# paolomandica/HALO

Measured on AMD Instinct MI355X. Metric: acquisition-scored images/sec (1024x2048, C=256, 19 cls), higher is better.
Workload: dtype f64

## Files before the change

### halo_amd/_lib.py

```python
import ctypes as C
import os
import threading

from . import _build

F32, F64 = 0, 1
I64, I32, U8 = 2, 3, 4
UNC = {"entropy": 0, "pixel_entropy": 1, "oracle_acc": 2}
UNC_ZEROS = 3
PUR = {"ripu": 0, "oracle_ripu": 1, "hyper": 2, "none": 3, "radius": 4, "euc_norm": 5}
E_UNSUPPORTED = -2
SELECT = {"auto": 0, "serial": 1, "binned": 2}
LOSS_CE, LOSS_NL = 1, 2
SWEEP_REASONS = ("done", "bad_values", "bin_overflow", "survivors", "exhausted", "not_run")
PAD = {"zeros": 0, "reflect": 1, "replicate": 2, "circular": 3}
FLAG_NORMALIZE = 1


def score_flags(normalize, padding_mode="zeros"):
    return (FLAG_NORMALIZE if normalize else 0) | (PAD[padding_mode] << 8)

_i64, _dbl, _int, _vp, _sz = C.c_int64, C.c_double, C.c_int, C.c_void_p, C.c_size_t

SIGNATURES = {
    "halo_version": (_int, []),
    "halo_last_error": (C.c_char_p, []),
    "halo_expmap0_project": (_int, [_vp, _int, _vp, _i64, _i64, _i64, _dbl, _vp]),
    "halo_logmap0_project": (_int, [_vp, _vp, _i64, _i64, _i64, _dbl, _vp]),
    "halo_dist0": (_int, [_vp, _int, _vp, _i64, _i64, _i64, _dbl, _vp]),
    "halo_pdist": (_int, [_vp, _vp, _vp, _i64, _i64, _dbl, _vp]),
    "halo_hypermlr_workspace_bytes": (_sz, [_i64, _i64]),
    "halo_hypermlr_logits": (_int, [_vp, _vp, _vp, _vp, _int, _i64, _i64, _i64, _i64, _dbl, _vp, _sz, _vp]),
    "halo_head_tail": (_int, [_vp, _vp, _vp, _vp, _vp, _int, _i64, _i64, _i64, _i64, _dbl, _vp, _sz, _vp]),
    "halo_expmap0_project_bwd": (_int, [_vp, _int, _vp, _vp, _i64, _i64, _i64, _dbl, _vp]),
    "halo_hypermlr_bwd_terms": (_int, [_vp, _vp, _vp, _vp, _i64, _i64, _i64, _i64, _dbl, _vp, _vp, _vp, _vp, _vp, _vp, _vp,
                                       _sz, _vp]),
    "halo_hypermlr_backward_workspace_bytes": (_sz, [_i64, _i64, _i64, _i64]),
    "halo_hypermlr_backward": (_int, [_vp, _vp, _vp, _vp, _int, _i64, _i64, _i64, _i64, _dbl, _vp, _vp, _vp, _vp, _sz, _vp]),
    "halo_bilinear_upsample": (_int, [_vp, _vp, _int, _i64, _i64, _i64, _i64, _i64, _vp]),
    "halo_bilinear_upsample_bwd": (_int, [_vp, _vp, _int, _i64, _i64, _i64, _i64, _i64, _vp]),
    "halo_score_workspace_bytes": (_sz, [_i64, _i64, _i64]),
    "halo_score_maps": (_int, [_vp, _i64, _vp, _int, _i64, _vp, _vp, _i64, _i64, _i64, _i64, _i64, _int, _int,
                               _int, _int, _int, _i64, _dbl, _vp, _vp, _vp, _vp, _sz, _vp]),
    "halo_score_maps_timed": (_int, [_vp, _i64, _vp, _int, _i64, _vp, _vp, _i64, _i64, _i64, _i64, _i64, _int, _int,
                                     _int, _int, _int, _i64, _dbl, _vp, _vp, _vp, _vp, _sz, _vp, _vp, _vp, _vp]),
    "halo_score_maps_split": (_int, [_vp, _i64, _vp, _int, _i64, _vp, _vp, _i64, _i64, _i64, _i64, _i64, _int, _int,
                                     _int, _int, _int, _i64, _dbl, _vp, _vp, _vp, _vp, _sz, _vp, _vp, _vp, _vp, _vp]),
    "halo_score_lr_workspace_bytes": (_sz, [_i64, _i64, _i64, _i64]),
    "halo_score_maps_lr": (_int, [_vp, _i64, _i64, _i64, _vp, _int, _i64, _i64, _i64, _vp, _vp, _i64, _i64, _i64, _i64, _i64,
                                  _int, _int, _int, _int, _int, _i64, _dbl, _vp, _vp, _vp, _vp, _sz, _vp]),
    "halo_score_lr_gram_workspace_bytes": (_sz, [_i64, _i64, _i64, _i64, _i64, _i64]),
    "halo_score_maps_lr_gram": (_int, [_vp, _i64, _i64, _i64, _vp, _int, _i64, _i64, _i64, _vp, _vp, _i64, _i64, _i64, _i64, _i64,
                                       _int, _int, _int, _int, _int, _i64, _dbl, _vp, _vp, _vp, _vp, _sz, _vp]),
    "halo_score_maps_lr_timed": (_int, [_vp, _i64, _i64, _i64, _vp, _int, _i64, _i64, _i64, _vp, _vp, _i64, _i64, _i64, _i64, _i64,
                                        _int, _int, _int, _int, _int, _i64, _dbl, _vp, _vp, _vp, _vp, _sz, _vp, _int, _vp, _vp, _vp, _vp, _vp, _vp, _vp]),
    "halo_region_uncertainty": (_int, [_vp, _i64, _int, _vp, _i64, _i64, _i64, _i64, _int, _int, _int, _vp, _vp, _sz, _vp]),
    "halo_region_impurity": (_int, [_vp, _i64, _i64, _i64, _int, _i64, _vp, _vp, _int, _vp]),
    "halo_quantize_radius": (_int, [_vp, _int, _i64, _i64, _i64, _i64, _i64, _i64, _dbl, _vp, _vp, _sz, _vp]),
    "halo_loss_workspace_bytes": (_sz, [_i64]),
    "halo_negative_learning_fwd": (_int, [_vp, _i64, _dbl, _vp, _vp, _sz, _vp]),
    "halo_negative_learning_bwd": (_int, [_vp, _i64, _dbl, _vp, _vp, _vp, _vp]),
    "halo_local_consistent_fwd": (_int, [_vp, _vp, _i64, _i64, _i64, _i64, _int, _vp, _vp, _vp, _vp, _vp, _vp, _sz, _vp]),
    "halo_local_consistent_bwd": (_int, [_vp, _vp, _vp, _vp, _i64, _i64, _i64, _i64, _vp, _vp, _vp, _vp]),
    "halo_eval_workspace_bytes": (_sz, [_i64, _i64, _i64, _i64]),
    "halo_eval_confusion": (_int, [_vp, _i64, _int, _i64, _i64, _i64, _vp, _int, _i64, _i64, _i64, _i64, _vp, _vp, _vp, _sz, _vp]),
    "halo_confusion_from_pred": (_int, [_vp, _int, _vp, _int, _i64, _i64, _i64, _i64, _i64, _vp, _vp, _sz, _vp]),
    "halo_upsampled_loss_workspace_bytes": (_sz, [_i64, _i64, _i64, _i64]),
    "halo_upsampled_loss_fwd": (_int, [_vp, _i64, _i64, _i64, _i64, _i64, _vp, _int, _i64, _i64, _i64, _dbl, _int, _vp, _vp, _sz, _vp]),
    "halo_upsampled_loss_bwd": (_int, [_vp, _i64, _i64, _i64, _i64, _i64, _vp, _int, _i64, _i64, _i64, _dbl, _int, _vp, _vp, _vp, _vp, _vp]),
    "halo_hfr_workspace_bytes": (_sz, [_i64, _i64, _i64]),
    "halo_hfr_fwd_stats": (_int, [_vp, _i64, _i64, _i64, _vp, _vp, _vp, _vp, _sz, _vp]),
    "halo_hfr_fwd_apply": (_int, [_vp, _i64, _i64, _i64, _vp, _vp, _vp, _vp, _vp, _dbl, _dbl, _vp, _vp, _vp, _vp, _vp, _vp, _sz, _vp]),
    "halo_hfr_bwd_reduce": (_int, [_vp, _i64, _i64, _i64, _vp, _vp, _vp, _vp, _vp, _vp, _vp, _vp, _sz, _vp]),
    "halo_hfr_bwd_apply": (_int, [_vp, _i64, _i64, _i64, _vp, _vp, _vp, _vp, _vp, _vp, _vp, _vp, _vp, _sz, _vp]),
    "halo_dwconv_workspace_bytes": (_sz, [_i64, _i64, _i64, _i64, _i64]),
    "halo_dwconv3x3_affine_relu_fwd": (_int, [_vp, _vp, _vp, _vp, _vp, _i64, _i64, _i64, _i64, _i64, _vp]),
    "halo_dwconv3x3_affine_relu_bwd_data": (_int, [_vp, _vp, _vp, _vp, _vp, _i64, _i64, _i64, _i64, _i64, _vp]),
    "halo_dwconv3x3_affine_relu_bwd_weight": (_int, [_vp, _vp, _vp, _vp, _vp, _i64, _i64, _i64, _i64, _i64, _vp, _sz, _vp]),
    "halo_event_create": (_vp, []),
    "halo_event_record": (_int, [_vp, _vp]),
    "halo_event_elapsed_ms": (_int, [_vp, _vp, C.POINTER(C.c_float)]),
    "halo_event_destroy": (_int, [_vp]),
    "halo_pack_pick_tables": (_int, [_vp, _vp, _i64, _i64, _vp, _i64, _vp]),
    "halo_reset_round_state": (_int, [_vp, _vp, _vp, _i64, _vp]),
    "halo_undo_picks": (_int, [_vp, _vp, _i64, _i64, _i64, _i64, _i64, _i64, _vp, _vp, _vp, _vp]),
    "halo_device_identity": (_int, [_int, C.c_char_p, _sz]),
    "halo_select_workspace_bytes": (_sz, [_i64, _i64, _i64, _i64, _i64]),
    "halo_score_range_bytes": (_sz, [_i64]),
    "halo_score_range": (_int, [_vp, _int, _i64, _i64, _i64, _vp, _vp]),
    "halo_greedy_select_ranged": (_int, [_vp, _int, _i64, _i64, _i64, _i64, _i64, _i64, _vp, _vp, _vp, _vp, _vp, _vp,
                                         _vp, _sz, _int, _vp, _vp]),
    "halo_greedy_select_ex": (_int, [_vp, _int, _i64, _i64, _i64, _i64, _i64, _i64, _vp, _vp, _vp, _vp, _vp, _vp,
                                     _vp, _sz, _int, _vp, _vp, _vp]),
    "halo_greedy_select": (_int, [_vp, _int, _i64, _i64, _i64, _i64, _i64, _i64, _vp, _vp, _vp, _vp, _vp, _vp,
                                  _vp, _sz, _int, _vp]),
}

ABI_VERSION = 10

_lock = threading.Lock()
_handle = None


class HaloHipError(RuntimeError):
    pass


class HaloUnsupported(HaloHipError):
    """The kernel declined this configuration (HALO_E_UNSUPPORTED); the caller may take another HIP route."""


def library_path():
    return _build.SO


def _preload_torch_hip_runtime():
    import torch
    libdir = os.path.join(os.path.dirname(torch.__file__), "lib")
    for name in ("libamdhip64.so",):
        cand = os.path.join(libdir, name)
        if os.path.exists(cand):
            C.CDLL(cand, mode=C.RTLD_GLOBAL)


def hip_runtime():
    import torch
    cand = os.path.join(os.path.dirname(torch.__file__), "lib", "libamdhip64.so")
    return C.CDLL(cand if os.path.exists(cand) else "libamdhip64.so", mode=C.RTLD_GLOBAL)


def lib():
    global _handle
    if _handle is not None:
        return _handle
    with _lock:
        if _handle is not None:
            return _handle
        try:
            path = os.environ.get("HALO_LIB_PATH") or _build.build()
        except Exception as exc:
            if not os.path.exists(_build.SO):
                raise HaloHipError("libhalo_hip.so is missing and could not be built: %s" % exc) from exc
            if _build.is_stale() and not os.environ.get("HALO_ALLOW_STALE_LIB"):
                raise HaloHipError("libhalo_hip.so is older than its sources and could not be rebuilt (%s); "
                                   "set HALO_ALLOW_STALE_LIB=1 to load it anyway" % exc) from exc
            path = _build.SO
        _preload_torch_hip_runtime()
        h = C.CDLL(path)
        ns = _Library()
        for name, (res, args) in SIGNATURES.items():
            fn = getattr(h, name, None)
            if fn is None:
                raise HaloHipError("%s does not export %s" % (path, name))
            fn.restype = res
            fn.argtypes = args
            setattr(ns, name, _on_stream_device(fn) if res is _int and args and _vp in args else fn)
        got = h.halo_version()
        if got != ABI_VERSION:
            raise HaloHipError("%s has ABI version %d, this package binds version %d: rebuild it "
                               "(python -m halo_amd._build --force)" % (path, got, ABI_VERSION))
        ns._cdll = h
        _handle = ns
    return _handle


class _Library(object):
    """Typed entry points of libhalo_hip.so (attributes named like the C functions)."""


class StreamPtr(C.c_void_p):
    device_index = None


def _on_stream_device(fn):
    def call(*args):
        import torch
        for a in reversed(args):
            if isinstance(a, StreamPtr):
                idx = a.device_index
                if idx is not None and idx != torch.cuda.current_device():
                    with torch.cuda.device(idx):
                        return fn(*args)
                break
        return fn(*args)
    call.__name__ = getattr(fn, "__name__", "halo_call")
    return call


def check(rc, what=""):
    if rc == 0:
        return
    msg = lib().halo_last_error().decode("utf-8", "replace")
    if rc == E_UNSUPPORTED and "not implemented" in msg:
        raise NotImplementedError(msg)
    if rc == E_UNSUPPORTED:
        raise HaloUnsupported("%s: %s" % (what or "halo call", msg))
    raise HaloHipError("%s failed (%d): %s" % (what or "halo call", rc, msg))


def dtype_code(t):
    import torch
    if t.dtype == torch.float32:
        return F32
    if t.dtype == torch.float64:
        return F64
    raise TypeError("halo_amd: expected float32/float64 tensor, got %s" % t.dtype)


def int_code(t):
    import torch
    code = {torch.int64: I64, torch.int32: I32, torch.uint8: U8}.get(t.dtype)
    if code is None:
        raise HaloUnsupported("halo_amd: expected an int64/int32/uint8 map, got %s" % t.dtype)
    return code


def require_device(*tensors):
    dev = None
    for t in tensors:
        if t is None:
            continue
        if not t.is_cuda:
            raise HaloHipError(
                "halo_amd runs on ROCm devices only (got a %s tensor); there is no CPU fallback" % t.device)
        if dev is None:
            dev = t.device
        elif t.device != dev:
            raise HaloHipError("halo_amd: tensors on different devices (%s vs %s)" % (dev, t.device))
    return dev


def stream_ptr(device=None):
    import torch
    st = torch.cuda.current_stream(device)
    p = StreamPtr(st.cuda_stream)
    p.device_index = st.device.index
    return p


def ptr(t):
    return C.c_void_p(0 if t is None else t.data_ptr())
```

### halo_amd/core/active/floating_region.py

```python
import os

import torch
import torch.nn as nn

from ... import _lib
from ..configs import cfg
from ..utils.hyperbolic import HyperMapper

_WS = {}


import threading as _threading

_ws_tls = _threading.local()


class private_workspaces(object):

    def __enter__(self):
        self.held = []
        self._prev = getattr(_ws_tls, "held", None)
        _ws_tls.held = self.held
        return self

    def __exit__(self, *exc):
        _ws_tls.held = self._prev
        return False


def _workspace(dev, nbytes, tag):
    held = getattr(_ws_tls, "held", None)
    if held is not None:
        buf = torch.empty(int(nbytes), dtype=torch.uint8, device=dev)
        held.append(buf)
        return buf
    key = (dev.index, torch.cuda.current_stream(dev).cuda_stream, tag)
    buf = _WS.get(key)
    if buf is None or buf.numel() < nbytes:
        buf = torch.empty(int(nbytes), dtype=torch.uint8, device=dev)
        _WS[key] = buf
    return buf


def score_workspace(B, H, W, dev):
    return torch.empty(int(_lib.lib().halo_score_workspace_bytes(int(B), int(H), int(W))), dtype=torch.uint8, device=dev)


def score_dtype(pur_type, decoder_out):
    if pur_type in ("radius", "euc_norm") and decoder_out is not None and decoder_out.dtype == torch.float64:
        return torch.float64
    return torch.float32


def new_score_range(B, dev):
    n = _lib.lib().halo_score_range_bytes(1)
    return torch.empty((int(B), int(n)), dtype=torch.uint8, device=dev)


def score_maps(logit, decoder_out=None, unc_type=None, pur_type=None, normalize=False, ground_truth=None,
               size=3, purity_size=None, K=100, c=1.0, active=None, want_maps=True, out=None, events=None, score_range=None,
               tail_stream=None, workspace=None, maps=None, padding_mode="zeros"):
    if pur_type not in _lib.PUR:
        raise NotImplementedError("Error: purity type '{}' not implemented".format(pur_type))
    if padding_mode not in _lib.PAD:
        raise ValueError("padding_mode must be one of %s, got %r" % (sorted(_lib.PAD), padding_mode))
    dev = _lib.require_device(logit, decoder_out, ground_truth, active)
    assert logit.dim() == 4, "logit must be (B,O,H,W)"
    if logit.dtype != torch.float32:
        logit = logit.float()
    B, O, H, W = logit.shape
    if logit.stride()[1:] != (H * W, W, 1):
        logit = logit.contiguous()
    need_feat = pur_type in ("hyper", "radius", "euc_norm")
    feat = None
    Cc, fdt, fbs = 0, _lib.F64, 0
    if need_feat:
        if decoder_out is None:
            raise ValueError("decoder_out is required for purity type '%s'" % pur_type)
        feat = decoder_out
        if feat.dtype not in (torch.float32, torch.float64):
            feat = feat.float()
        Cc = feat.shape[1]
        assert feat.shape[0] == B and feat.shape[2:] == (H, W), "decoder_out shape mismatch"
        if feat.stride()[1:] != (H * W, W, 1):
            feat = feat.contiguous()
        fdt, fbs = _lib.dtype_code(feat), feat.stride(0)
    need_gt = unc_type == "oracle_acc" or pur_type == "oracle_ripu"
    gt = None
    if need_gt:
        if ground_truth is None:
            raise ValueError("ground_truth is required for '%s'/'%s'" % (unc_type, pur_type))
        gt = ground_truth.reshape(B, H, W).to(torch.int64).contiguous()
    act = None
    if active is not None:
        act = active.reshape(B, H, W).contiguous()
        act = act.view(torch.uint8) if act.dtype == torch.bool else act.to(torch.uint8)
    odt = score_dtype(pur_type, feat)
    if B == 0 or H == 0 or W == 0:
        e = torch.empty((B, H, W), dtype=odt, device=dev)
        return (e, e.clone(), torch.empty((B, H, W), dtype=torch.float32, device=dev)) if want_maps else (e, None, None)
    if out is not None:
        assert out.shape == (B, H, W) and out.dtype == odt and out.is_contiguous() and out.device == dev
        score = out
    else:
        score = torch.empty((B, H, W), dtype=odt, device=dev)
    if maps is not None:
        imp, unc = maps
        assert imp.shape == (B, H, W) and imp.dtype == odt and imp.is_contiguous() and unc.shape == (B, H, W) and unc.dtype == torch.float32
    else:
        imp = torch.empty((B, H, W), dtype=odt, device=dev) if want_maps else None
        unc = torch.empty((B, H, W), dtype=torch.float32, device=dev) if want_maps else None
    L = _lib.lib()
    nws = L.halo_score_workspace_bytes(B, H, W)
    if workspace is not None:
        assert workspace.dtype == torch.uint8 and workspace.numel() >= nws and workspace.device == dev
        ws = workspace
    else:
        ws = _workspace(dev, nws, "score")
    psize = size if purity_size is None else purity_size
    ev0, ev1 = events if events is not None else (None, None)
    if score_range is not None:
        assert score_range.is_contiguous() and score_range.device == dev and score_range.numel() >= L.halo_score_range_bytes(B)
    if tail_stream is not None:
        assert events is not None and workspace is not None and (maps is not None or not want_maps), \
            "tail_stream needs events, a workspace of the call's own and preallocated maps"
        rc = L.halo_score_maps_split(_lib.ptr(logit), logit.stride(0), _lib.ptr(feat), fdt, fbs, _lib.ptr(gt),
                                     _lib.ptr(act), B, O, Cc, H, W, _lib.UNC.get(unc_type, _lib.UNC_ZEROS),
                                     _lib.PUR[pur_type], _lib.score_flags(normalize, padding_mode), int(size), int(psize), int(K), float(c),
                                     _lib.ptr(score), _lib.ptr(imp), _lib.ptr(unc), _lib.ptr(ws), ws.numel(),
                                     _lib.stream_ptr(dev), _lib.C.c_void_p(tail_stream.cuda_stream), ev0, ev1, _lib.ptr(score_range))
        _lib.check(rc, "halo_score_maps_split")
        return score, imp, unc
    rc = L.halo_score_maps_timed(_lib.ptr(logit), logit.stride(0), _lib.ptr(feat), fdt, fbs, _lib.ptr(gt),
                                 _lib.ptr(act), B, O, Cc, H, W, _lib.UNC.get(unc_type, _lib.UNC_ZEROS),
                                 _lib.PUR[pur_type], _lib.score_flags(normalize, padding_mode), int(size), int(psize), int(K), float(c),
                                 _lib.ptr(score), _lib.ptr(imp), _lib.ptr(unc), _lib.ptr(ws), ws.numel(),
                                 _lib.stream_ptr(dev), ev0, ev1, _lib.ptr(score_range))
    _lib.check(rc, "halo_score_maps")
    return score, imp, unc


LOWRES_MODES = ("exact", "gram")


def lowres_mode(mode=None):
    mode = os.environ.get("HALO_LOWRES", "exact") if mode is None else mode
    if mode not in LOWRES_MODES:
        raise ValueError("low-res mode must be one of %s, got %r" % (LOWRES_MODES, mode))
    return mode


def score_maps_lowres(logit_lr, decoder_lr, size, unc_type=None, pur_type=None, normalize=False, ground_truth=None,
                      ksize=3, purity_size=None, K=100, c=1.0, active=None, want_maps=True, mode=None, events=None,
                      score_range=None, padding_mode="zeros"):
    if pur_type not in _lib.PUR:
        raise NotImplementedError("Error: purity type '{}' not implemented".format(pur_type))
    mode = lowres_mode(mode)
    dev = _lib.require_device(logit_lr, decoder_lr, ground_truth, active)
    H, W = int(size[0]), int(size[1])
    logit_lr = logit_lr.float().contiguous()
    B, O, hl, wl = logit_lr.shape
    need_feat = pur_type in ("hyper", "radius", "euc_norm")
    feat, Cc, fdt, fbs, hf, wf = None, 0, _lib.F64, 0, 0, 0
    if need_feat:
        if decoder_lr is None:
            raise ValueError("decoder_out is required for purity type '%s'" % pur_type)
        feat = decoder_lr if decoder_lr.dtype in (torch.float32, torch.float64) else decoder_lr.float()
        feat = feat.contiguous()
        assert feat.shape[0] == B
        Cc, hf, wf = feat.shape[1:]
        fdt, fbs = _lib.dtype_code(feat), feat.stride(0)
    need_gt = unc_type == "oracle_acc" or pur_type == "oracle_ripu"
    if need_gt and ground_truth is None:
        raise ValueError("ground_truth is required for '%s'/'%s'" % (unc_type, pur_type))
    gt = ground_truth.reshape(B, H, W).to(torch.int64).contiguous() if need_gt else None
    act = None
    if active is not None:
        act = active.reshape(B, H, W).contiguous()
        act = act.view(torch.uint8) if act.dtype == torch.bool else act.to(torch.uint8)
    odt = score_dtype(pur_type, feat)
    score = torch.empty((B, H, W), dtype=odt, device=dev)
    imp = torch.empty((B, H, W), dtype=odt, device=dev) if want_maps else None
    unc = torch.empty((B, H, W), dtype=torch.float32, device=dev) if want_maps else None
    L = _lib.lib()
    gram = mode == "gram" and need_feat and fdt == _lib.F64
    nws = L.halo_score_lr_gram_workspace_bytes(B, O, H, W, hf, wf) if gram else L.halo_score_lr_workspace_bytes(B, O, H, W)
    ws = _workspace(dev, nws, "score")
    psize = ksize if purity_size is None else purity_size
    fn, name = (L.halo_score_maps_lr_gram, "halo_score_maps_lr_gram") if gram else (L.halo_score_maps_lr, "halo_score_maps_lr")
    args = (_lib.ptr(logit_lr), logit_lr.stride(0), hl, wl, _lib.ptr(feat), fdt, fbs, hf, wf,
            _lib.ptr(gt), _lib.ptr(act), B, O, Cc, H, W, _lib.UNC.get(unc_type, _lib.UNC_ZEROS),
            _lib.PUR[pur_type], _lib.score_flags(normalize, padding_mode), int(ksize), int(psize), int(K), float(c),
            _lib.ptr(score), _lib.ptr(imp), _lib.ptr(unc), _lib.ptr(ws), ws.numel(),
            _lib.stream_ptr(dev))
    if events is not None or score_range is not None:
        if score_range is not None:
            assert score_range.is_contiguous() and score_range.device == dev and score_range.numel() >= L.halo_score_range_bytes(B)
        name = "halo_score_maps_lr_timed"
        ev = tuple(events or ()) + (None,) * 6
        rc = L.halo_score_maps_lr_timed(*(args + (1 if gram else 0,) + ev[:4] + (_lib.ptr(score_range),) + ev[4:6]))
    else:
        rc = fn(*args)
    _lib.check(rc, name)
    return score, imp, unc


class FloatingRegionScore(nn.Module):
    def __init__(self, in_channels=19, padding_mode="zeros", size=33, purity_type=None, K=100):
        super(FloatingRegionScore, self).__init__()
        self.in_channels = in_channels
        assert size % 2 == 1, "error size"
        if padding_mode not in _lib.PAD:
            raise ValueError("padding_mode must be one of ['zeros', 'reflect', 'replicate', 'circular'], but got padding_mode='{}'"
                             .format(padding_mode))
        self.padding_mode = padding_mode
        if purity_type is None:
            purity_type = cfg.ACTIVE.PURITY
        self.size = size
        self.purity_size = size
        self.purity_channels = in_channels
        if purity_type == "hyper":
            self.K, self.purity_size, self.purity_channels = K, 3, K
        self.mapper = HyperMapper(c=cfg.MODEL.CURVATURE)

    def _check_purity_channels(self, pur_type):
        if pur_type in ("ripu", "oracle_ripu") and self.purity_channels != self.in_channels:
            raise RuntimeError("purity window was built for %d bins ('hyper'), got a %d-class prediction"
                               % (self.purity_channels, self.in_channels))
        if pur_type == "hyper" and not hasattr(self, "K"):
            raise AttributeError("'FloatingRegionScore' object has no attribute 'K'")
        if pur_type == "hyper" and self.purity_channels != self.K:
            raise RuntimeError("purity window channel mismatch")

    def _uncertainty(self, x, is_prob, unc_type, ground_truth, do_box):
        dev = _lib.require_device(x, ground_truth)
        x = x.float().contiguous()
        O, H, W = x.shape
        out = torch.empty((1, 1, H, W), dtype=torch.float32, device=dev)
        gt = None if ground_truth is None else ground_truth.to(torch.int64).contiguous()
        ws = _workspace(dev, H * W * 4 + 256, "unc")
        rc = _lib.lib().halo_region_uncertainty(_lib.ptr(x), x.numel(), 1 if is_prob else 0, _lib.ptr(gt), 1, O, H, W,
                                                _lib.UNC.get(unc_type, _lib.UNC_ZEROS), int(self.size),
                                                (1 if do_box else 0) | (_lib.PAD[self.padding_mode] << 8), _lib.ptr(out), _lib.ptr(ws), ws.numel(),
                                                _lib.stream_ptr(dev))
        _lib.check(rc, "halo_region_uncertainty")
        return out

    def compute_region_uncertainty(self, unc_type, logit, p, ground_truth=None):
        return self._uncertainty(p, True, unc_type, ground_truth, do_box=(unc_type != "none"))

    def compute_pixel_entropy(self, p):
        return self._uncertainty(p, True, "pixel_entropy", None, do_box=False)

    def quantize_uncert_map(self, decoder_out):
        dev = _lib.require_device(decoder_out)
        feat = decoder_out if decoder_out.dtype in (torch.float32, torch.float64) else decoder_out.float()
        feat = feat.contiguous()
        B, Cc, H, W = feat.shape
        assert B == 1
        pred = torch.empty((H, W), dtype=torch.int64, device=dev)
        L = _lib.lib()
        nws = L.halo_score_workspace_bytes(1, H, W)
        ws = _workspace(dev, nws, "score")
        rc = L.halo_quantize_radius(_lib.ptr(feat), _lib.dtype_code(feat), feat.stride(0), 1, Cc, H, W, int(self.K),
                                    float(self.mapper.c), _lib.ptr(pred), _lib.ptr(ws), ws.numel(), _lib.stream_ptr(dev))
        _lib.check(rc, "halo_quantize_radius")
        return pred

    def compute_region_impurity(self, predict, K):
        dev = _lib.require_device(predict)
        if K != self.purity_channels:
            raise RuntimeError("purity window was built for %d channels, got K=%d" % (self.purity_channels, K))
        pred = predict.to(torch.int64).contiguous()
        H, W = pred.shape
        imp = torch.empty((1, 1, H, W), dtype=torch.float32, device=dev)
        cnt = torch.empty((1, 1, H, W), dtype=torch.float32, device=dev)
        rc = _lib.lib().halo_region_impurity(_lib.ptr(pred), 1, H, W, int(self.purity_size), int(K), _lib.ptr(imp),
                                             _lib.ptr(cnt), _lib.PAD[self.padding_mode], _lib.stream_ptr(dev))
        _lib.check(rc, "halo_region_impurity")
        return imp, cnt

    def forward(self, logit: torch.Tensor, decoder_out: torch.Tensor = None, unc_type: str = None,
                pur_type: str = None, normalize: bool = False, ground_truth=None):
        if pur_type not in _lib.PUR:
            raise NotImplementedError("Error: purity type '{}' not implemented".format(pur_type))
        self._check_purity_channels(pur_type)
        if logit.dim() == 3:
            logit = logit.unsqueeze(0)
        if logit.shape[0] != 1:
            raise ValueError("FloatingRegionScore.forward scores one image (as the reference); "
                             "use score_maps() for a batch")
        if decoder_out is not None and decoder_out.dim() == 3:
            decoder_out = decoder_out.unsqueeze(0)
        gt = None if ground_truth is None else ground_truth.unsqueeze(0)
        score, imp, unc = score_maps(logit, decoder_out, unc_type, pur_type, normalize, gt, size=self.size,
                                     purity_size=self.purity_size, K=getattr(self, "K", 100), c=self.mapper.c,
                                     padding_mode=self.padding_mode)
        return score[0], imp[0], unc[0]
```

### halo_amd/csrc/halo_score.hip

```cpp
#include "halo_common.hpp"
#include "halo_devmath.hpp"
#include "halo_select_plan.hpp"
#include "halo_softmax.hpp"
#include <stdlib.h>

namespace halo {

constexpr int TPB = 256;
#ifndef HALO_FTPB
#define HALO_FTPB 128
#endif
#ifndef HALO_FEAT_WAVES
#define HALO_FEAT_WAVES 4
#endif
#ifndef HALO_FEAT_UNROLL
#define HALO_FEAT_UNROLL 8
#endif
constexpr int FTPB = HALO_FTPB;

__device__ __forceinline__ double nan_min(double a, double b) { return (a != a) ? a : ((b != b) ? b : (b < a ? b : a)); }
__device__ __forceinline__ double nan_max(double a, double b) { return (a != a) ? a : ((b != b) ? b : (b > a ? b : a)); }

template <int NT = TPB>
__device__ __forceinline__ void block_minmax(double mn, double mx, double *out2)
{
    __shared__ double smn[NT / 64], smx[NT / 64];
#pragma unroll
    for (int off = 32; off > 0; off >>= 1) {
        mn = nan_min(mn, __shfl_xor(mn, off));
        mx = nan_max(mx, __shfl_xor(mx, off));
    }
    const int wave = threadIdx.x >> 6;
    if ((threadIdx.x & 63) == 0) { smn[wave] = mn; smx[wave] = mx; }
    __syncthreads();
    if (threadIdx.x == 0) {
#pragma unroll
        for (int i = 1; i < NT / 64; ++i) { mn = nan_min(mn, smn[i]); mx = nan_max(mx, smx[i]); }
        out2[0] = mn;
        out2[1] = mx;
    }
}

__global__ void __launch_bounds__(TPB) k_minmax_finalize(const double *__restrict__ partials, int nblk,
                                                          double *__restrict__ stats, int slot)
{
    const int b = blockIdx.x;
    const double *p = partials + (size_t)b * nblk * 2;
    double mn = p[0], mx = p[1];
    for (int i = threadIdx.x; i < nblk; i += TPB) { mn = nan_min(mn, p[2 * i]); mx = nan_max(mx, p[2 * i + 1]); }
    block_minmax<TPB>(mn, mx, stats + b * 4 + slot * 2);
}

constexpr int FIN_TPB = 1024;
__global__ void __launch_bounds__(FIN_TPB) k_minmax_finalize2(const double *__restrict__ part0, int nblk0, const double *__restrict__ part1,
                                                               int nblk1, double *__restrict__ stats)
{
    const int b = blockIdx.x, slot = blockIdx.y;
    const int nblk = slot ? nblk1 : nblk0;
    const double2 *p = reinterpret_cast<const double2 *>((slot ? part1 : part0) + (size_t)b * nblk * 2);
    const double2 p0 = p[0];
    double mn = p0.x, mx = p0.y;
    for (int i = threadIdx.x; i < nblk; i += FIN_TPB) { const double2 q = p[i]; mn = nan_min(mn, q.x); mx = nan_max(mx, q.y); }
    block_minmax<FIN_TPB>(mn, mx, stats + b * 4 + slot * 2);
}


#ifndef HALO_LOGF_LDS
#define HALO_LOGF_LDS 1
#endif

struct ClassSum {
    float a0 = 0.0f, a1 = 0.0f, a2 = 0.0f, a3 = 0.0f;
    int prev = 0;
    __device__ __forceinline__ void add(int c, float t)
    {
        const int x = c ^ prev;
        if (x >> 4) {
            a1 = a1 + a0; a0 = 0.0f;
            if (x >> 8) {
                a2 = a2 + a1; a1 = 0.0f;
                if (x >> 12) { a3 = a3 + a2; a2 = 0.0f; }
            }
        }
        a0 = a0 + t;
        prev = c;
    }
    __device__ __forceinline__ float result() const { return ((a0 + a1) + a2) + a3; }
};

__device__ __forceinline__ void px_general(const float *__restrict__ lp, int O, long long hw, int is_prob, int unc_type,
                                           int pur_type, long long g, float &ent, int &pred)
{
    float m = 0.0f, s = 1.0f;
    if (!is_prob) {
        m = lp[0];
#pragma unroll 1
        for (int c = 1; c < O; ++c) { float x = lp[(size_t)c * hw]; m = x > m ? x : m; }
        s = 0.0f;
#pragma unroll 1
        for (int c = 0; c < O; ++c) s = s + det_expf(lp[(size_t)c * hw] - m);
    }
    float best = 0.0f, pg = 0.0f;
    ClassSum acc;
    int am = 0;
#pragma unroll 1
    for (int c = 0; c < O; ++c) {
        const float p = is_prob ? lp[(size_t)c * hw] : det_expf(lp[(size_t)c * hw] - m) / s;
        if (c == 0 || p > best) { best = p; am = c; }
        if (c == (int)g) pg = p;
        acc.add(c, (-p) * det_logf(p + 1e-6f));
    }
    const float a = acc.result();
    if (unc_type == HALO_UNC_ENTROPY || unc_type == HALO_UNC_PIXEL_ENTROPY) ent = a / (float)2.9444389791664403;
    else if (unc_type == HALO_UNC_ORACLE_ACC) ent = 1.0f - (g == 255 ? best : pg);
    else ent = 0.0f;
    pred = pur_type == HALO_PUR_ORACLE_RIPU ? (g == 255 ? am : (int)g) : am;
}


template <int O_T, int NP, bool LEAN>
__device__ __forceinline__ void finish_px(float (&p)[NP][O_T], int unc_type, int pur_type, const long long (&g)[NP],
                                          float (&ent)[NP], int (&pred)[NP], bool want_pred = true, const double (*ltab)[2] = logf_tab_)
{
    int am[NP];
    float best[NP];
#pragma unroll
    for (int j = 0; j < NP; ++j) { am[j] = 0; best[j] = p[j][0]; }
    if (want_pred || unc_type == HALO_UNC_ORACLE_ACC) {
#pragma unroll
        for (int c = 1; c < O_T; ++c)
#pragma unroll
            for (int j = 0; j < NP; ++j) { const bool gtb = p[j][c] > best[j]; am[j] = gtb ? c : am[j]; best[j] = gtb ? p[j][c] : best[j]; }
    }
    if (unc_type == HALO_UNC_ENTROPY || unc_type == HALO_UNC_PIXEL_ENTROPY) {
        static_assert(O_T <= 256, "class count of the unrolled statement");
        float a0[NP], a1[NP];
#pragma unroll
        for (int j = 0; j < NP; ++j) a0[j] = a1[j] = 0.0f;
#pragma unroll
        for (int c = 0; c < O_T; ++c) {
#pragma unroll
            for (int j = 0; j < NP; ++j) {
                const float q = p[j][c] + 1e-6f;
                a0[j] = a0[j] + (-p[j][c]) * (LEAN ? det_logf_core(q, ltab) : det_logf(q));
            }
            if ((c & 15) == 15 && c + 1 < O_T) {
#pragma unroll
                for (int j = 0; j < NP; ++j) { a1[j] = a1[j] + a0[j]; a0[j] = 0.0f; }
            }
        }
#pragma unroll
        for (int j = 0; j < NP; ++j) ent[j] = (a0[j] + a1[j]) / (float)2.9444389791664403;
    } else if (unc_type == HALO_UNC_ORACLE_ACC) {
#pragma unroll
        for (int j = 0; j < NP; ++j) {
            const int gi = g[j] == 255 ? am[j] : (int)g[j];
            float pg = 0.0f;
#pragma unroll
            for (int c = 0; c < O_T; ++c) pg = c == gi ? p[j][c] : pg;
            ent[j] = 1.0f - pg;
        }
    } else {
#pragma unroll
        for (int j = 0; j < NP; ++j) ent[j] = 0.0f;
    }
#pragma unroll
    for (int j = 0; j < NP; ++j) pred[j] = pur_type == HALO_PUR_ORACLE_RIPU ? (g[j] == 255 ? am[j] : (int)g[j]) : am[j];
}

template <int O_T, int VEC>
__global__ void __launch_bounds__(TPB) k_logit_maps(const float *__restrict__ logit, long long bstride,
                                                    const long long *__restrict__ gt, long long hw,
                                                    int unc_type, int pur_type, float *__restrict__ ent,
                                                    short *__restrict__ pred)
{
    const int b = blockIdx.y;
    const long long i0 = ((long long)blockIdx.x * TPB + threadIdx.x) * VEC;
#if HALO_LOGF_LDS
    __shared__ double s_ltab[128][2];
    stage_logf_table<TPB>(s_ltab);
    const double (*ltab)[2] = s_ltab;
#else
    const double (*ltab)[2] = logf_tab_;
#endif
    if (i0 >= hw) return;
    const float *lp = logit + (size_t)b * bstride + i0;
    const bool need_gt = unc_type == HALO_UNC_ORACLE_ACC || pur_type == HALO_PUR_ORACLE_RIPU;
    float v[VEC][O_T];
    if constexpr (VEC == 4) {
#pragma unroll
        for (int c = 0; c < O_T; ++c) {
            const float4 q = *reinterpret_cast<const float4 *>(lp + (size_t)c * hw);
            v[0][c] = q.x; v[1][c] = q.y; v[2][c] = q.z; v[3][c] = q.w;
        }
    } else {
#pragma unroll
        for (int c = 0; c < O_T; ++c) v[0][c] = lp[(size_t)c * hw];
    }
    float e[VEC];
    int pr[VEC];
    long long g[VEC];
#pragma unroll
    for (int j = 0; j < VEC; ++j) g[j] = need_gt ? gt[(size_t)b * hw + i0 + j] : 0;
    if (softmax_lean<O_T, VEC>(v)) {
        finish_px<O_T, VEC, true>(v, unc_type, pur_type, g, e, pr, pred != nullptr, ltab);
    } else {
#pragma unroll 1
        for (int j = 0; j < VEC; ++j) px_general(lp + j, O_T, hw, 0, unc_type, pur_type, g[j], e[j], pr[j]);
    }
    float *ep = ent + (size_t)b * hw + i0;
    if constexpr (VEC == 4) {
        *reinterpret_cast<float4 *>(ep) = make_float4(e[0], e[1], e[2], e[3]);
    } else {
        ep[0] = e[0];
    }
    if (pred) {
#pragma unroll
        for (int j = 0; j < VEC; ++j) pred[(size_t)b * hw + i0 + j] = (short)pr[j];
    }
}

__global__ void __launch_bounds__(TPB) k_logit_maps_generic(const float *__restrict__ logit, long long bstride,
                                                            const long long *__restrict__ gt, int O, long long hw,
                                                            int unc_type, int pur_type, int is_prob,
                                                            float *__restrict__ ent, short *__restrict__ pred)
{
    const int b = blockIdx.y;
    const long long i = (long long)blockIdx.x * TPB + threadIdx.x;
    if (i >= hw) return;
    const bool need_gt = unc_type == HALO_UNC_ORACLE_ACC || pur_type == HALO_PUR_ORACLE_RIPU;
    const long long g = need_gt ? gt[(size_t)b * hw + i] : 0;
    float e;
    int pr;
    px_general(logit + (size_t)b * bstride + i, O, hw, is_prob, unc_type, pur_type, g, e, pr);
    ent[(size_t)b * hw + i] = e;
    if (pred) pred[(size_t)b * hw + i] = (short)pr;
}

__device__ __forceinline__ double fma_t(double a, double b, double c) { return __builtin_fma(a, b, c); }
__device__ __forceinline__ float fma_t(float a, float b, float c) { return __builtin_fmaf(a, b, c); }

template <typename T, int VEC> struct VecLoad;
typedef double d2_t __attribute__((ext_vector_type(2)));
typedef float f4_t __attribute__((ext_vector_type(4)));
template <> struct VecLoad<double, 2> {
    static __device__ __forceinline__ void ld(const double *p, double (&v)[2])
    {
        const d2_t q = __builtin_nontemporal_load(reinterpret_cast<const d2_t *>(p));
        v[0] = q.x; v[1] = q.y;
    }
};
template <> struct VecLoad<float, 4> {
    static __device__ __forceinline__ void ld(const float *p, float (&v)[4])
    {
        const f4_t q = __builtin_nontemporal_load(reinterpret_cast<const f4_t *>(p));
        v[0] = q.x; v[1] = q.y; v[2] = q.z; v[3] = q.w;
    }
};
template <typename T> struct VecLoad<T, 1> {
    static __device__ __forceinline__ void ld(const T *p, T (&v)[1]) { v[0] = *p; }
};

template <typename T, int VEC, int MODE, int UNROLL, int FO>
__global__ void __launch_bounds__(FTPB) __attribute__((amdgpu_waves_per_eu(1, HALO_FEAT_WAVES))) k_feat_reduce(const T *__restrict__ feat, long long bstride, int C,
                                                     long long hw, double ks, double rks, T *__restrict__ out,
                                                     double *__restrict__ partials, const float *__restrict__ logit,
                                                     long long lbstride, int unc_type, float *__restrict__ ent, unsigned xcd_g)
{
    const int b = blockIdx.y;
    unsigned bx = blockIdx.x;
    const unsigned xj = blockIdx.x >> 3;
    if (xcd_g != 0 && blockIdx.x < (gridDim.x / (8 * xcd_g)) * (8 * xcd_g))
        bx = (xj / xcd_g) * 8 * xcd_g + (blockIdx.x & 7) * xcd_g + xj % xcd_g;
    const long long blk0 = (long long)bx * (FTPB * VEC);
    const unsigned lane0 = threadIdx.x * VEC;
    const long long i0 = blk0 + lane0;
    const bool live = i0 < hw;
#if HALO_LOGF_LDS
    __shared__ double s_ltab[FO > 0 ? 128 : 1][2];
    if constexpr (FO > 0) stage_logf_table<FTPB>(s_ltab);
    const double (*ltab)[2] = s_ltab;
#else
    const double (*ltab)[2] = logf_tab_;
#endif
    T acc[VEC];
#pragma unroll
    for (int j = 0; j < VEC; ++j) acc[j] = (T)0;
    auto entropy_part = [&]() {
        if constexpr (FO > 0) {
            const float *lp = logit + (size_t)b * lbstride + blk0;
            float *eb = ent + (size_t)b * hw + blk0;
            constexpr int NP = VEC >= 2 ? 2 : 1;
#pragma unroll
            for (int part = 0; part < VEC / NP; ++part) {
                const unsigned off = part * (FTPB * NP) + threadIdx.x * NP;
                if (blk0 + off < hw) {
                    float lv[NP][FO];
                    const float *plane = lp;
#pragma unroll
                    for (int c2 = 0; c2 < FO; ++c2, plane += hw) {
                        if constexpr (NP == 2) {
                            const float2 q = *reinterpret_cast<const float2 *>(plane + off);
                            lv[0][c2] = q.x; lv[1][c2] = q.y;
                        } else {
                            lv[0][c2] = plane[off];
                        }
                    }
                    float e[NP];
                    int pr[NP];
                    long long gz[NP];
#pragma unroll
                    for (int j = 0; j < NP; ++j) gz[j] = 0;
                    if (softmax_lean<FO, NP>(lv)) {
                        finish_px<FO, NP, true>(lv, unc_type, HALO_PUR_NONE, gz, e, pr, false, ltab);
                    } else {
#pragma unroll 1
                        for (int j = 0; j < NP; ++j) px_general(lp + off + j, FO, hw, 0, unc_type, HALO_PUR_NONE, 0, e[j], pr[j]);
                    }
                    if constexpr (NP == 2) *reinterpret_cast<float2 *>(eb + off) = make_float2(e[0], e[1]);
                    else eb[off] = e[0];
                }
                __builtin_amdgcn_sched_barrier(0);
            }
        }
    };
    const bool ent_first = ((xcd_g != 0 ? xj / xcd_g : blockIdx.x) & 1) != 0;
    double mn = 0.0, mx = 0.0;
    const T *p = feat + (size_t)b * bstride + blk0;
    auto walk_to = [&](int c, const int c_end) {
        for (; c + UNROLL <= c_end; c += UNROLL) {
            T v[UNROLL][VEC];
#pragma unroll
            for (int u = 0; u < UNROLL; ++u, p += hw) VecLoad<T, VEC>::ld(p + lane0, v[u]);
#pragma unroll
            for (int u = 0; u < UNROLL; ++u)
#pragma unroll
                for (int j = 0; j < VEC; ++j) acc[j] = fma_t(v[u][j], v[u][j], acc[j]);
        }
        for (; c < c_end; ++c, p += hw) {
            T v[VEC];
            VecLoad<T, VEC>::ld(p + lane0, v);
#pragma unroll
            for (int j = 0; j < VEC; ++j) acc[j] = fma_t(v[j], v[j], acc[j]);
        }
    };
    auto finish = [&]() {
        T r[VEC];
#pragma unroll
        for (int j = 0; j < VEC; ++j) {
            if constexpr (MODE == 0) r[j] = dist0_from_ssq(acc[j], ks, rks);
            else if constexpr (sizeof(T) == 8) r[j] = __builtin_sqrt(acc[j]);
            else r[j] = __builtin_sqrtf(acc[j]);
        }
        T *op = (out + (size_t)b * hw + blk0) + lane0;
        if constexpr (VEC == 2) *reinterpret_cast<double2 *>(op) = make_double2(r[0], r[1]);
        else if constexpr (VEC == 4) *reinterpret_cast<float4 *>(op) = make_float4(r[0], r[1], r[2], r[3]);
        else op[0] = r[0];
        mn = mx = (double)r[0];
#pragma unroll
        for (int j = 1; j < VEC; ++j) { mn = nan_min(mn, (double)r[j]); mx = nan_max(mx, (double)r[j]); }
    };
    if constexpr (FO > 0) {
        if (live && !ent_first) { walk_to(0, C); finish(); }
        entropy_part();
        if (live && ent_first) { walk_to(0, C); finish(); }
    } else {
        if (live) { walk_to(0, C); finish(); }
    }
    __shared__ double seed[2];
    if (threadIdx.x == 0) { seed[0] = mn; seed[1] = mx; }
    __syncthreads();
    if (!live) { mn = seed[0]; mx = seed[1]; }
    block_minmax<FTPB>(mn, mx, partials + ((size_t)b * gridDim.x + bx) * 2);
}

template <typename T, typename TO>
__global__ void __launch_bounds__(TPB) k_quantize(const T *__restrict__ r, const double *__restrict__ stats,
                                                  long long hw, int K, TO *__restrict__ pred)
{
    const int b = blockIdx.y;
    const long long i = (long long)blockIdx.x * TPB + threadIdx.x;
    if (i >= hw) return;
    const T mn = (T)stats[b * 4 + 0], mx = (T)stats[b * 4 + 1];
    T x;
    if constexpr (sizeof(T) == 8) {
        x = (r[(size_t)b * hw + i] - mn) / (mx - mn);
        x = 1.0 - x;
        double p = x * (double)K - 0.5;
        const double lo = -0.5 + 1e-5, hi = (double)K - 0.5 - 1e-5;
        p = p < lo ? lo : p;
        p = p > hi ? hi : p;
        pred[(size_t)b * hw + i] = (TO)__builtin_rint(p);
    } else {
        const float den = (float)((double)mx - (double)mn);
        x = (r[(size_t)b * hw + i] - mn) / den;
        x = 1.0f - x;
        float p = x * (float)K - 0.5f;
        const float lo = (float)(-0.5 + 1e-5), hi = (float)((double)K - 0.5 - 1e-5);
        p = p < lo ? lo : p;
        p = p > hi ? hi : p;
        const float q = __builtin_rintf(p);
        pred[(size_t)b * hw + i] = (TO)(q > (float)(K - 1) ? (float)(K - 1) : q);
    }
}

__device__ __forceinline__ int pad_index(int t, int n, int mode)
{
    if (t >= 0 && t < n) return t;
    if (mode == HALO_PAD_ZEROS) return -1;
    if (mode == HALO_PAD_REPLICATE) return t < 0 ? 0 : n - 1;
    if (mode == HALO_PAD_REFLECT) return t < 0 ? -t : 2 * (n - 1) - t;
    return t < 0 ? t + n : t - n;
}

template <typename TL>
__global__ void __launch_bounds__(TPB) k_region_impurity(const TL *__restrict__ pred, int H, int W, int k,
                                                         float logK, float *__restrict__ imp, float *__restrict__ count, int pad)
{
    const int b = blockIdx.y;
    const long long hw = (long long)H * W;
    const long long i = (long long)blockIdx.x * TPB + threadIdx.x;
    if (i >= hw) return;
    const int y = (int)(i / W), x = (int)(i % W), r = k / 2;
    const int y0 = pad ? y - r : (y - r < 0 ? 0 : y - r), y1 = pad ? y + r : (y + r >= H ? H - 1 : y + r);
    const int x0 = pad ? x - r : (x - r < 0 ? 0 : x - r), x1 = pad ? x + r : (x + r >= W ? W - 1 : x + r);
    const TL *pp = pred + (size_t)b * hw;
    const float cnt = (float)((y1 - y0 + 1) * (x1 - x0 + 1));
    ClassSum acc;
    int cur = -1;
    while (true) {
        int nxt = 0x7fffffff, n = 0;
        for (int yy = y0; yy <= y1; ++yy)
            for (int xx = x0; xx <= x1; ++xx) {
                const int v = (int)pp[(size_t)pad_index(yy, H, pad) * W + pad_index(xx, W, pad)];
                if (v > cur) {
                    if (v < nxt) { nxt = v; n = 1; }
                    else if (v == nxt) ++n;
                }
            }
        if (n == 0) break;
        const float d = (float)n / cnt;
        acc.add(nxt, (-d) * det_logf(d + 1e-6f));
        cur = nxt;
    }
    imp[(size_t)b * hw + i] = acc.result() / logK;
    if (count) count[(size_t)b * hw + i] = cnt;
}

constexpr int RI_TW = 64, RI_TH = 16;

template <typename TL>
__global__ void __launch_bounds__(TPB) k_region_impurity3(const TL *__restrict__ pred, int H, int W, float logK,
                                                          float *__restrict__ imp, float *__restrict__ count,
                                                          double *__restrict__ partials)
{
    __shared__ int lab[RI_TH + 2][RI_TW + 2 + 2];
    __shared__ float term[10][10];
    const int b = blockIdx.z, tid = threadIdx.x;
    if (tid < 100) {
        const int c = tid / 10, n = tid % 10;
        float tv = 0.0f;
        if (c > 0 && n > 0 && n <= c) { const float d = (float)n / (float)c; tv = (-d) * det_logf(d + 1e-6f); }
        term[c][n] = tv;
    }
    const int X0 = blockIdx.x * RI_TW, Y0 = blockIdx.y * RI_TH;
    const long long hw = (long long)H * W;
    const TL *pp = pred + (size_t)b * hw;
    for (int e = tid; e < (RI_TH + 2) * (RI_TW + 2); e += TPB) {
        const int ty = e / (RI_TW + 2), tx = e % (RI_TW + 2);
        const int y = Y0 + ty - 1, x = X0 + tx - 1;
        lab[ty][tx] = (y >= 0 && y < H && x >= 0 && x < W) ? (int)pp[(size_t)y * W + x] : -1;
    }
    __syncthreads();
    const int ly = tid >> 4, lx = (tid & 15) * 4;
    const int y = Y0 + ly, xb = X0 + lx;
    const bool live = y < H && xb < W;
    double mn = 0.0, mx = 0.0;
    int v[3][6];
#pragma unroll
    for (int dy = 0; dy < 3; ++dy)
#pragma unroll
        for (int dx = 0; dx < 6; ++dx) v[dy][dx] = lab[ly + dy][lx + dx];
    const int ny = (y > 0 ? 1 : 0) + 1 + (y < H - 1 ? 1 : 0);
#pragma unroll
    for (int j = 0; j < 4; ++j) {
        const int x = xb + j;
        if (!live || x >= W) break;
        const int cnti = ny * ((x > 0 ? 1 : 0) + 1 + (x < W - 1 ? 1 : 0));
        const float cnt = (float)cnti;
        const float *tc = term[cnti];
        ClassSum acc;
        int cur = -1;
        while (true) {
            int nxt = 0x7fffffff;
#pragma unroll
            for (int dy = 0; dy < 3; ++dy)
#pragma unroll
                for (int dx = 0; dx < 3; ++dx) { const int q = v[dy][j + dx]; nxt = (q > cur && q < nxt) ? q : nxt; }
            if (nxt == 0x7fffffff) break;
            int n = 0;
#pragma unroll
            for (int dy = 0; dy < 3; ++dy)
#pragma unroll
                for (int dx = 0; dx < 3; ++dx) n += v[dy][j + dx] == nxt ? 1 : 0;
            acc.add(nxt, tc[n]);
            cur = nxt;
        }
        const float res = acc.result() / logK;
        imp[(size_t)b * hw + (size_t)y * W + x] = res;
        if (count) count[(size_t)b * hw + (size_t)y * W + x] = cnt;
        if (j == 0) mn = mx = (double)res;
        else { mn = nan_min(mn, (double)res); mx = nan_max(mx, (double)res); }
    }
    if (!partials) return;
    __shared__ double seed[2];
    if (tid == 0) { seed[0] = mn; seed[1] = mx; }
    __syncthreads();
    if (!live) { mn = seed[0]; mx = seed[1]; }
    block_minmax<TPB>(mn, mx, partials + (((size_t)b * gridDim.y + blockIdx.y) * gridDim.x + blockIdx.x) * 2);
}

template <typename TL>
static int launch_region_impurity(const TL *pred, int64_t B, int64_t H, int64_t W, int k, float logK, float *imp, float *count,
                                  hipStream_t st, double *partials = nullptr, int pad = HALO_PAD_ZEROS)
{
    if (pad == HALO_PAD_ZEROS && k == 3 && cdiv(H, RI_TH) <= 65535 && B <= 65535) {
        const dim3 grid((unsigned)cdiv(W, RI_TW), (unsigned)cdiv(H, RI_TH), (unsigned)B);
        hipLaunchKernelGGL((k_region_impurity3<TL>), grid, dim3(TPB), 0, st, pred, (int)H, (int)W, logK, imp, count, partials);
        return partials ? (int)(grid.x * grid.y) : 0;
    }
    hipLaunchKernelGGL((k_region_impurity<TL>), dim3((unsigned)cdiv(H * W, TPB), (unsigned)B), dim3(TPB), 0, st, pred, (int)H, (int)W, k,
                       logK, imp, count, pad);
    return 0;
}

__global__ void __launch_bounds__(TPB) k_box_unc(const float *__restrict__ ent, int H, int W, int k, int do_box,
                                                 int pk, float *__restrict__ unc, double *__restrict__ partials, int pad)
{
    const int b = blockIdx.y;
    const long long hw = (long long)H * W;
    const long long i = (long long)blockIdx.x * TPB + threadIdx.x;
    const bool live = i < hw;
    double mn = 0.0, mx = 0.0;
    if (live) {
        const int y = (int)(i / W), x = (int)(i % W);
        const float *ep = ent + (size_t)b * hw;
        float a;
        if (do_box) {
            const int r = k / 2;
            a = 0.0f;
            for (int dy = -r; dy <= r; ++dy)
                for (int dx = -r; dx <= r; ++dx) {
                    const int yy = pad_index(y + dy, H, pad), xx = pad_index(x + dx, W, pad);
                    const float v = (yy >= 0 && xx >= 0) ? ep[(size_t)yy * W + xx] : 0.0f;
                    a = a + v;
                }
        } else {
            a = ep[i];
        }
        float cnt = 1.0f;
        if (pk > 0 && pad) {
            cnt = (float)(pk * pk);
        } else if (pk > 0) {
            const int r = pk / 2;
            const int y0 = y - r < 0 ? 0 : y - r, y1 = y + r >= H ? H - 1 : y + r;
            const int x0 = x - r < 0 ? 0 : x - r, x1 = x + r >= W ? W - 1 : x + r;
            cnt = (float)((y1 - y0 + 1) * (x1 - x0 + 1));
        }
        a = a / cnt;
        unc[(size_t)b * hw + i] = a;
        mn = mx = (double)a;
    }
    if (!partials) return;
    __shared__ double seed[2];
    if (threadIdx.x == 0) { seed[0] = mn; seed[1] = mx; }
    __syncthreads();
    if (!live) { mn = seed[0]; mx = seed[1]; }
    block_minmax<TPB>(mn, mx, partials + ((size_t)b * gridDim.x + blockIdx.x) * 2);
}

__device__ __forceinline__ float lane_prev(float v)
{
    return __int_as_float(__builtin_amdgcn_update_dpp(0, __float_as_int(v), 0x138 , 0xf, 0xf, false));
}
__device__ __forceinline__ float lane_next(float v)
{
    return __int_as_float(__builtin_amdgcn_update_dpp(0, __float_as_int(v), 0x130 , 0xf, 0xf, false));
}

__device__ __forceinline__ float box3_over_count(float a, int H, int W, int y, int xx, int pk)
{
    if (pk <= 0) return a;
    const int rr = pk / 2;
    const int y0 = y - rr < 0 ? 0 : y - rr, y1 = y + rr >= H ? H - 1 : y + rr;
    const int x0 = xx - rr < 0 ? 0 : xx - rr, x1 = xx + rr >= W ? W - 1 : xx + rr;
    return a / (float)((y1 - y0 + 1) * (x1 - x0 + 1));
}

__device__ __forceinline__ void box3_row4(const float *__restrict__ ep, int H, int W, int y, int x, bool live, int pk, float (&o)[4])
{
    const int lane = threadIdx.x & 63;
    float r[3][6];
#pragma unroll
    for (int dy = 0; dy < 3; ++dy) {
        const int yy = y + dy - 1;
        const bool in = live && yy >= 0 && yy < H;
        const float *row = ep + (size_t)(in ? yy : 0) * W;
        float4 q = make_float4(0.0f, 0.0f, 0.0f, 0.0f);
        if (in) q = *reinterpret_cast<const float4 *>(row + x);
        float left = lane_prev(q.w), right = lane_next(q.x);
        if (lane == 0) left = (in && x > 0) ? row[x - 1] : 0.0f;
        if (lane == 63) right = (in && x + 4 < W) ? row[x + 4] : 0.0f;
        r[dy][0] = (in && x > 0) ? left : 0.0f;
        r[dy][1] = q.x; r[dy][2] = q.y; r[dy][3] = q.z; r[dy][4] = q.w;
        r[dy][5] = (in && x + 4 < W) ? right : 0.0f;
    }
#pragma unroll
    for (int j = 0; j < 4; ++j) {
        float a = 0.0f;
#pragma unroll
        for (int dy = 0; dy < 3; ++dy)
#pragma unroll
            for (int dx = 0; dx < 3; ++dx) a = a + r[dy][j + dx];
        o[j] = box3_over_count(a, H, W, y, x + j, pk);
    }
}

__global__ void __launch_bounds__(TPB) k_box3_unc(const float *__restrict__ ent, int H, int W, int pk,
                                                  float *__restrict__ unc, double *__restrict__ partials)
{
    const int b = blockIdx.y;
    const long long hw = (long long)H * W;
    const long long i0 = ((long long)blockIdx.x * TPB + threadIdx.x) * 4;
    const bool live = i0 < hw;
    double mn = 0.0, mx = 0.0;
    const int y = live ? (int)(i0 / W) : 0, x = live ? (int)(i0 % W) : 0;
    float o[4];
    box3_row4(ent + (size_t)b * hw, H, W, y, x, live, pk, o);
    if (live) {
        if (unc) *reinterpret_cast<float4 *>(unc + (size_t)b * hw + i0) = make_float4(o[0], o[1], o[2], o[3]);
        mn = mx = (double)o[0];
#pragma unroll
        for (int j = 1; j < 4; ++j) { mn = nan_min(mn, (double)o[j]); mx = nan_max(mx, (double)o[j]); }
    }
    if (!partials) return;
    __shared__ double seed[2];
    if (threadIdx.x == 0) { seed[0] = mn; seed[1] = mx; }
    __syncthreads();
    if (!live) { mn = seed[0]; mx = seed[1]; }
    block_minmax<TPB>(mn, mx, partials + ((size_t)b * gridDim.x + blockIdx.x) * 2);
}

constexpr int BM_RPT = 4, BM_TW = 256, BM_TH = BM_RPT * (TPB / 64);

__device__ __forceinline__ float nan_minf(float a, float b) { return (a != a) ? a : ((b != b) ? b : (b < a ? b : a)); }
__device__ __forceinline__ float nan_maxf(float a, float b) { return (a != a) ? a : ((b != b) ? b : (b > a ? b : a)); }

__global__ void __launch_bounds__(TPB) k_box3_minmax(const float *__restrict__ ent, int H, int W, int pk, double *__restrict__ partials,
                                                     unsigned *__restrict__ hist_zero)
{
    const int b = blockIdx.z, lane = threadIdx.x & 63, wv = threadIdx.x >> 6;
    if (hist_zero) {
        const unsigned nb = gridDim.x * gridDim.y;
        for (unsigned l = blockIdx.y * gridDim.x + blockIdx.x; l < NB1 / TPB; l += nb) hist_zero[(size_t)b * NB1 + l * TPB + threadIdx.x] = 0u;
    }
    const int x = blockIdx.x * BM_TW + lane * 4, y0 = blockIdx.y * BM_TH + wv * BM_RPT;
    const float *ep = ent + (size_t)b * H * W;
    const bool xin = x < W;
    auto load_row = [&](int yy, float (&r)[6]) {
        const bool in = xin && yy >= 0 && yy < H;
        const float *row = ep + (size_t)(in ? yy : 0) * W;
        float4 q = make_float4(0.0f, 0.0f, 0.0f, 0.0f);
        if (in) q = *reinterpret_cast<const float4 *>(row + x);
        float left = lane_prev(q.w), right = lane_next(q.x);
        if (lane == 0) left = (in && x > 0) ? row[x - 1] : 0.0f;
        if (lane == 63) right = (in && x + 4 < W) ? row[x + 4] : 0.0f;
        r[0] = (in && x > 0) ? left : 0.0f;
        r[1] = q.x; r[2] = q.y; r[3] = q.z; r[4] = q.w;
        r[5] = (in && x + 4 < W) ? right : 0.0f;
    };
    float r0[6], r1[6], r2[6];
    load_row(y0 - 1, r0);
    load_row(y0, r1);
    float mn = 0.0f, mx = 0.0f;
    bool have = false;
#pragma unroll
    for (int k = 0; k < BM_RPT; ++k) {
        const int y = y0 + k;
        load_row(y + 1, r2);
        if (xin && y < H) {
#pragma unroll
            for (int j = 0; j < 4; ++j) {
                float a = 0.0f;
#pragma unroll
                for (int dx = 0; dx < 3; ++dx) a = a + r0[j + dx];
#pragma unroll
                for (int dx = 0; dx < 3; ++dx) a = a + r1[j + dx];
#pragma unroll
                for (int dx = 0; dx < 3; ++dx) a = a + r2[j + dx];
                const float o = box3_over_count(a, H, W, y, x + j, pk);
                if (!have) { mn = mx = o; have = true; }
                else { mn = nan_minf(mn, o); mx = nan_maxf(mx, o); }
            }
        }
#pragma unroll
        for (int q = 0; q < 6; ++q) { r0[q] = r1[q]; r1[q] = r2[q]; }
    }
    __shared__ float seedf[2];
    __shared__ float smn[TPB / 64], smx[TPB / 64];
    if (threadIdx.x == 0) { seedf[0] = mn; seedf[1] = mx; }
    __syncthreads();
    if (!have) { mn = seedf[0]; mx = seedf[1]; }
#pragma unroll
    for (int off = 32; off > 0; off >>= 1) {
        mn = nan_minf(mn, __shfl_xor(mn, off));
        mx = nan_maxf(mx, __shfl_xor(mx, off));
    }
    if (lane == 0) { smn[wv] = mn; smx[wv] = mx; }
    __syncthreads();
    if (threadIdx.x == 0) {
#pragma unroll
        for (int i = 1; i < TPB / 64; ++i) { mn = nan_minf(mn, smn[i]); mx = nan_maxf(mx, smx[i]); }
        double *out2 = partials + (((size_t)b * gridDim.y + blockIdx.y) * gridDim.x + blockIdx.x) * 2;
        out2[0] = (double)mn;
        out2[1] = (double)mx;
    }
}

__global__ void __launch_bounds__(TPB) k_minmax_f32(const float *__restrict__ x, long long hw,
                                                    double *__restrict__ partials)
{
    const int b = blockIdx.y;
    const long long i = (long long)blockIdx.x * TPB + threadIdx.x;
    const bool live = i < hw;
    double mn = 0.0, mx = 0.0;
    if (live) mn = mx = (double)x[(size_t)b * hw + i];
    __shared__ double seed[2];
    if (threadIdx.x == 0) { seed[0] = mn; seed[1] = mx; }
    __syncthreads();
    if (!live) { mn = seed[0]; mx = seed[1]; }
    block_minmax<TPB>(mn, mx, partials + ((size_t)b * gridDim.x + blockIdx.x) * 2);
}

__global__ void __launch_bounds__(TPB) k_fill_f32(float *__restrict__ x, long long n, float v)
{
    const long long i = (long long)blockIdx.x * TPB + threadIdx.x;
    if (i < n) x[i] = v;
}

template <typename TI>
__global__ void __launch_bounds__(TPB) k_combine(const TI *__restrict__ imp_raw, const float *__restrict__ unc_raw,
                                                 const double *__restrict__ stats, const unsigned char *__restrict__ active,
                                                 long long hw, int normalize, TI *__restrict__ score,
                                                 TI *__restrict__ imp_out, float *__restrict__ unc_out)
{
    const int b = blockIdx.y;
    const long long i = (long long)blockIdx.x * TPB + threadIdx.x;
    if (i >= hw) return;
    const size_t o = (size_t)b * hw + i;
    TI im = imp_raw[o];
    float un = unc_raw[o];
    if (normalize) {
        const float umn = (float)stats[b * 4 + 2], umx = (float)stats[b * 4 + 3];
        un = (un - umn) / (float)((double)umx - (double)umn);
        const TI imn = (TI)stats[b * 4 + 0], imx = (TI)stats[b * 4 + 1];
        if constexpr (sizeof(TI) == 8) im = (im - imn) / (imx - imn);
        else im = (im - imn) / (float)((double)imx - (double)imn);
    }
    TI s = im * (TI)un;
    if (active && active[o]) {
        if constexpr (sizeof(TI) == 8) s = __longlong_as_double(0xfff0000000000000ll);
        else s = __uint_as_float(0xff800000u);
    }
    score[o] = s;
    if (imp_out) imp_out[o] = im;
    if (unc_out) unc_out[o] = un;
}


constexpr int CB_ROWS = 16;

template <typename TI>
__global__ void __launch_bounds__(TPB) k_combine_box3(const TI *__restrict__ imp_raw, const float *__restrict__ ent,
                                                      const double *__restrict__ stats, const unsigned char *__restrict__ active,
                                                      int H, int W, int pk, int normalize, TI *__restrict__ score,
                                                      TI *__restrict__ imp_out, float *__restrict__ unc_out, SelHdr *__restrict__ rng,
                                                      unsigned *__restrict__ hist, int rows)
{
    __shared__ unsigned hl[NB1];
    const int b = blockIdx.z;
    const long long hw = (long long)H * W;
    const int x = (blockIdx.x * TPB + threadIdx.x) * 4;
    const bool live = x < W;
    float umn = 0.0f, uden = 1.0f;
    TI imn = (TI)0, iden = (TI)1;
    bool fin = false;
    if (normalize) {
        umn = (float)stats[b * 4 + 2];
        const float umx = (float)stats[b * 4 + 3];
        uden = (float)((double)umx - (double)umn);
        imn = (TI)stats[b * 4 + 0];
        const TI imx = (TI)stats[b * 4 + 1];
        if constexpr (sizeof(TI) == 8) iden = imx - imn;
        else iden = (float)((double)imx - (double)imn);
        fin = uden > 0.0f && uden < __builtin_inff() && iden > (TI)0 && iden < (TI)__builtin_inf();
        if (rng && blockIdx.x == 0 && blockIdx.y == 0 && threadIdx.x == 0) {
            SelHdr h;
            memset(&h, 0, sizeof(h));
            h.kmin_inv = ~order_key(0.0);
            h.kmax = order_key(1.0);
            h.nvalid = 1u;
            h.flags = fin ? (hist ? (unsigned)SEL_F_HIST : 0u) : (unsigned)SEL_F_BAD;
            rng[b] = h;
        }
    }
    const bool count = hist != nullptr && fin;
    if (count) {
        for (int j = threadIdx.x; j < NB1; j += TPB) hl[j] = 0u;
        __syncthreads();
    }
    ValRange vr;
    vr.lo = 0.0; vr.scale = (double)NB1; vr.ok = true;
    const int ybeg = blockIdx.y * rows, yend = ybeg + rows < H ? ybeg + rows : H;
    const float *ep = ent + (size_t)b * hw;
    const int lane = threadIdx.x & 63;
    struct RowRaw { float4 q; float el, er; bool in; };
    auto row_issue = [&](int yy) {
        RowRaw t;
        t.in = live && yy >= 0 && yy < H;
        const float *row = ep + (size_t)(t.in ? yy : 0) * W;
        t.q = make_float4(0.0f, 0.0f, 0.0f, 0.0f);
        t.el = 0.0f; t.er = 0.0f;
        if (t.in) t.q = *reinterpret_cast<const float4 *>(row + x);
        if (lane == 0 && t.in && x > 0) t.el = row[x - 1];
        if (lane == 63 && t.in && x + 4 < W) t.er = row[x + 4];
        return t;
    };
    auto row_finish = [&](const RowRaw &t, float (&r)[6]) {
        float left = lane_prev(t.q.w), right = lane_next(t.q.x);
        if (lane == 0) left = t.el;
        if (lane == 63) right = t.er;
        r[0] = (t.in && x > 0) ? left : 0.0f;
        r[1] = t.q.x; r[2] = t.q.y; r[3] = t.q.z; r[4] = t.q.w;
        r[5] = (t.in && x + 4 < W) ? right : 0.0f;
    };
    typedef double cb_d2 __attribute__((ext_vector_type(2)));
    typedef float cb_f4 __attribute__((ext_vector_type(4)));
    struct PixRaw { cb_d2 d0, d1; cb_f4 f; unsigned am; };
    auto pix_issue = [&](int yy) {
        PixRaw t;
        t.d0 = (cb_d2){0.0, 0.0}; t.d1 = t.d0; t.f = (cb_f4){0.f, 0.f, 0.f, 0.f}; t.am = 0u;
        if (!live || yy >= yend) return t;
        const size_t o = (size_t)b * hw + (size_t)yy * W + x;
        if constexpr (sizeof(TI) == 8) {
            t.d0 = *reinterpret_cast<const cb_d2 *>(imp_raw + o);
            t.d1 = *reinterpret_cast<const cb_d2 *>(imp_raw + o + 2);
        } else {
            t.f = *reinterpret_cast<const cb_f4 *>(imp_raw + o);
        }
        if (active) t.am = *reinterpret_cast<const unsigned *>(active + o);
        return t;
    };
    float r0[6], r1[6], r2[6];
    {
        const RowRaw a0 = row_issue(ybeg - 1), a1 = row_issue(ybeg);
        row_finish(a0, r0);
        row_finish(a1, r1);
    }
    RowRaw nrow = row_issue(ybeg + 1);
    PixRaw npix = pix_issue(ybeg);
    for (int y = ybeg; y < yend; ++y) {
        row_finish(nrow, r2);
        const PixRaw cpix = npix;
        nrow = row_issue(y + 2);
        npix = pix_issue(y + 1);
        float un[4];
#pragma unroll
        for (int j = 0; j < 4; ++j) {
            float a = 0.0f;
#pragma unroll
            for (int dx = 0; dx < 3; ++dx) a = a + r0[j + dx];
#pragma unroll
            for (int dx = 0; dx < 3; ++dx) a = a + r1[j + dx];
#pragma unroll
            for (int dx = 0; dx < 3; ++dx) a = a + r2[j + dx];
            un[j] = box3_over_count(a, H, W, y, x + j, pk);
        }
#pragma unroll
        for (int q = 0; q < 6; ++q) { r0[q] = r1[q]; r1[q] = r2[q]; }
        if (!live) continue;
        const size_t o = (size_t)b * hw + (size_t)y * W + x;
        TI im[4];
        if constexpr (sizeof(TI) == 8) { im[0] = cpix.d0.x; im[1] = cpix.d0.y; im[2] = cpix.d1.x; im[3] = cpix.d1.y; }
        else { im[0] = cpix.f.x; im[1] = cpix.f.y; im[2] = cpix.f.z; im[3] = cpix.f.w; }
        if (normalize) {
#pragma unroll
            for (int j = 0; j < 4; ++j) { un[j] = (un[j] - umn) / uden; im[j] = (im[j] - imn) / iden; }
        }
        const unsigned am = cpix.am;
        TI sc[4];
#pragma unroll
        for (int j = 0; j < 4; ++j) {
            sc[j] = im[j] * (TI)un[j];
            if ((am >> (8 * j)) & 0xffu) {
                if constexpr (sizeof(TI) == 8) sc[j] = __longlong_as_double(0xfff0000000000000ll);
                else sc[j] = __uint_as_float(0xff800000u);
            }
        }
        if (count) {
#pragma unroll
            for (int j = 0; j < 4; ++j) {
                const double v = (double)sc[j];
                const unsigned long long k = order_key(v);
                if (k < KEY_POS_INF && k != KEY_NEG_INF) {
                    double t;
                    atomicAdd(&hl[coarse_bin(v, vr, t)], 1u);
                }
            }
        }
        if constexpr (sizeof(TI) == 8) {
            *reinterpret_cast<double2 *>(score + o) = make_double2(sc[0], sc[1]);
            *reinterpret_cast<double2 *>(score + o + 2) = make_double2(sc[2], sc[3]);
            if (imp_out) {
                *reinterpret_cast<double2 *>(imp_out + o) = make_double2(im[0], im[1]);
                *reinterpret_cast<double2 *>(imp_out + o + 2) = make_double2(im[2], im[3]);
            }
        } else {
            *reinterpret_cast<float4 *>(score + o) = make_float4(sc[0], sc[1], sc[2], sc[3]);
            if (imp_out) *reinterpret_cast<float4 *>(imp_out + o) = make_float4(im[0], im[1], im[2], im[3]);
        }
        if (unc_out) *reinterpret_cast<float4 *>(unc_out + o) = make_float4(un[0], un[1], un[2], un[3]);
    }
    if (count) {
        __syncthreads();
        unsigned *g = hist + (size_t)b * NB1;
        for (int j = threadIdx.x; j < NB1; j += TPB)
            if (hl[j]) atomicAdd(&g[j], hl[j]);
    }
}



constexpr int LR_STAGE_IT = 3, LR_STAGE_G = 4;
constexpr int LR_TW = 64, LR_TH = 16, LR_PPT = 4;

template <typename T, int NPX = LR_PPT> struct LrW { T lx0, lx1, ly0[NPX], ly1[NPX]; };


template <typename T, int PAT> struct LrRows {
    T v[3][2];
    __device__ __forceinline__ void load(const T *__restrict__ tp, int stride)
    {
        if constexpr (sizeof(T) == 8) {
            typedef __attribute__((address_space(3))) const T *lds_ptr;
            const unsigned a0 = (unsigned)(uintptr_t)(lds_ptr)tp, a1 = a0 + (unsigned)stride * 8u;
            if constexpr (PAT != 0) {
                const unsigned a2 = a1 + (unsigned)stride * 8u;
                asm volatile("ds_read_b64 %0, %6\n\tds_read_b64 %1, %6 offset:8\n\tds_read_b64 %2, %7\n\tds_read_b64 %3, %7 offset:8\n\t"
                             "ds_read_b64 %4, %8\n\tds_read_b64 %5, %8 offset:8\n\ts_waitcnt lgkmcnt(0)"
                             : "=&v"(v[0][0]), "=&v"(v[0][1]), "=&v"(v[1][0]), "=&v"(v[1][1]), "=&v"(v[2][0]), "=&v"(v[2][1])
                             : "v"(a0), "v"(a1), "v"(a2)
                             : "memory");
            } else {
                asm volatile("ds_read_b64 %0, %4\n\tds_read_b64 %1, %4 offset:8\n\tds_read_b64 %2, %5\n\tds_read_b64 %3, %5 offset:8\n\t"
                             "s_waitcnt lgkmcnt(0)"
                             : "=&v"(v[0][0]), "=&v"(v[0][1]), "=&v"(v[1][0]), "=&v"(v[1][1])
                             : "v"(a0), "v"(a1)
                             : "memory");
            }
        } else {
            v[0][0] = tp[0]; v[0][1] = tp[1];
            v[1][0] = tp[stride]; v[1][1] = tp[stride + 1];
            if constexpr (PAT != 0) { v[2][0] = tp[2 * stride]; v[2][1] = tp[2 * stride + 1]; }
        }
    }
    __device__ __forceinline__ void accumulate(const LrW<T> &wt, T (&acc)[LR_PPT]) const
    {
        T t[3];
        t[0] = col_lerp(wt.lx0, wt.lx1, v[0][0], v[0][1]);
        t[1] = col_lerp(wt.lx0, wt.lx1, v[1][0], v[1][1]);
        if constexpr (PAT != 0) t[2] = col_lerp(wt.lx0, wt.lx1, v[2][0], v[2][1]);
#pragma unroll
        for (int j = 0; j < LR_PPT; ++j) {
            const int a = j == 0 ? 0 : (PAT >> (j - 1)) & 1;
            const T x = col_lerp(wt.ly0[j], wt.ly1[j], t[a], t[a + 1]);
            acc[j] = fma_t(x, x, acc[j]);
        }
    }
};
template <typename T, int PAT>
__device__ __forceinline__ void lr_rows_chunk(const T *__restrict__ tp, int cc, int plane, int stride, const LrW<T> &wt, T (&acc)[LR_PPT])
{
#pragma unroll 1
    for (int ch = 0; ch < cc; ++ch, tp += plane) {
        LrRows<T, PAT> A;
        A.load(tp, stride);
        A.accumulate(wt, acc);
    }
}

template <typename T, int MODE>
__global__ void __launch_bounds__(TPB) k_feat_reduce_lr(const T *__restrict__ feat, long long bstride, int C, int h, int w,
                                                        int H, int W, T sh, T sw, int max_rows, int max_cols, int CC,
                                                        double ks, double rks, T *__restrict__ out,
                                                        double *__restrict__ partials)
{
    extern __shared__ __attribute__((aligned(16))) unsigned char lr_smem[];
    T *tile = reinterpret_cast<T *>(lr_smem);
    const unsigned ntx = gridDim.x, nty = gridDim.y, ntiles = ntx * nty * gridDim.z;
    const unsigned lin = blockIdx.x + ntx * (blockIdx.y + nty * blockIdx.z);
    const unsigned xq = ntiles / 8, xr = ntiles % 8, xk = lin % 8;
    const unsigned tile_id = (xk < xr ? xk * (xq + 1) : xr * (xq + 1) + (xk - xr) * xq) + lin / 8;
    const int bx = (int)(tile_id % ntx), by = (int)((tile_id / ntx) % nty);
    const int b = (int)(tile_id / (ntx * nty));
    const int X0 = bx * LR_TW, Y0 = by * LR_TH;
    const int lx = threadIdx.x & (LR_TW - 1), ly = threadIdx.x / LR_TW;
    const int x = X0 + lx;
    const int ylast = (Y0 + LR_TH - 1 < H ? Y0 + LR_TH - 1 : H - 1), xlast = (X0 + LR_TW - 1 < W ? X0 + LR_TW - 1 : W - 1);
    const int ty_lo = make_taps<T>(Y0, sh, h).i0, ty_hi = make_taps<T>(ylast, sh, h).i1;
    const int tx_lo = make_taps<T>(X0, sw, w).i0, tx_hi = make_taps<T>(xlast, sw, w).i1;
    const int rows = ty_hi - ty_lo + 2, cols = tx_hi - tx_lo + 2;
    const bool xin = x < W;
    const Taps<T> tx = make_taps<T>(xin ? x : W - 1, sw, w);
    T acc[LR_PPT];
    LrW<T> wt;
    wt.lx0 = tx.l0; wt.lx1 = tx.l1;
    int o00[LR_PPT], o10[LR_PPT];
    bool live[LR_PPT];
    int a0 = 0, pat = 0;
    bool regular = true;
#pragma unroll
    for (int j = 0; j < LR_PPT; ++j) {
        const int y = Y0 + ly * LR_PPT + j;
        live[j] = xin && y < H;
        const Taps<T> ty = make_taps<T>(y < H ? y : H - 1, sh, h);
        wt.ly0[j] = ty.l0; wt.ly1[j] = ty.l1;
        o00[j] = (ty.i0 - ty_lo) * max_cols + (tx.i0 - tx_lo);
        o10[j] = (ty.i1 - ty_lo) * max_cols + (tx.i0 - tx_lo);
        acc[j] = (T)0;
        if (j == 0) a0 = ty.i0;
        const int d = ty.i0 - a0;
        regular = regular && (d == 0 || d == 1);
        if (j > 0) pat |= (d & 1) << (j - 1);
    }
    const int dx1 = tx.i1 - tx.i0;
    const T *fb = feat + (size_t)b * bstride;
    const int plane = max_rows * max_cols;
    int st_src[LR_STAGE_IT], st_dst[LR_STAGE_IT];
    bool st_ok[LR_STAGE_IT];
#pragma unroll
    for (int it = 0; it < LR_STAGE_IT; ++it) {
        const int e = (threadIdx.x & 63) + 64 * it;
        const int r = e / cols, q = e % cols;
        const int sr = ty_lo + r < h - 1 ? ty_lo + r : h - 1, sq = tx_lo + q < w - 1 ? tx_lo + q : w - 1;
        st_ok[it] = e < rows * cols;
        st_src[it] = sr * w + sq;
        st_dst[it] = r * max_cols + q;
    }
    const int upat = __builtin_amdgcn_readfirstlane(regular ? pat : -1);
    const int wv = threadIdx.x >> 6;
    for (int c0 = 0; c0 < C; c0 += CC) {
        const int cc = C - c0 < CC ? C - c0 : CC;
        __syncthreads();
        {
            T pre[LR_STAGE_G][LR_STAGE_IT];
#pragma unroll
            for (int gI = 0; gI < LR_STAGE_G; ++gI) {
                const int ch = wv + gI * (TPB / 64);
                const T *src = fb + (size_t)(c0 + (ch < cc ? ch : 0)) * h * w;
#pragma unroll
                for (int it = 0; it < LR_STAGE_IT; ++it) pre[gI][it] = (st_ok[it] && ch < cc) ? src[st_src[it]] : (T)0;
            }
#pragma unroll
            for (int gI = 0; gI < LR_STAGE_G; ++gI) {
                const int ch = wv + gI * (TPB / 64);
                if (ch < cc) {
                    T *dst = tile + ch * plane;
#pragma unroll
                    for (int it = 0; it < LR_STAGE_IT; ++it)
                        if (st_ok[it]) dst[st_dst[it]] = pre[gI][it];
                    for (int e = (threadIdx.x & 63) + 64 * LR_STAGE_IT; e < rows * cols; e += 64) {
                        const int r = e / cols, q = e % cols;
                        const int sr = ty_lo + r < h - 1 ? ty_lo + r : h - 1, sq = tx_lo + q < w - 1 ? tx_lo + q : w - 1;
                        dst[r * max_cols + q] = fb[(size_t)(c0 + ch) * h * w + (size_t)sr * w + sq];
                    }
                }
            }
        }
        __syncthreads();
        const T *t0 = tile + o00[0];
        if (upat == 0) lr_rows_chunk<T, 0>(t0, cc, plane, max_cols, wt, acc);
        else if (upat == 4) lr_rows_chunk<T, 4>(t0, cc, plane, max_cols, wt, acc);
        else if (upat == 6) lr_rows_chunk<T, 6>(t0, cc, plane, max_cols, wt, acc);
        else if (upat == 7) lr_rows_chunk<T, 7>(t0, cc, plane, max_cols, wt, acc);
        else {
#pragma unroll 1
            for (int ch = 0; ch < cc; ++ch) {
                const T *tp = tile + ch * plane;
#pragma unroll
                for (int j = 0; j < LR_PPT; ++j) {
                    const T v = bilerp<T>(tp[o00[j]], tp[o00[j] + dx1], tp[o10[j]], tp[o10[j] + dx1], wt.lx0, wt.lx1, wt.ly0[j], wt.ly1[j]);
                    acc[j] = fma_t(v, v, acc[j]);
                }
            }
        }
    }
    double mn = 0.0, mx = 0.0;
    bool have = false;
#pragma unroll
    for (int j = 0; j < LR_PPT; ++j) {
        if (!live[j]) continue;
        const int y = Y0 + ly * LR_PPT + j;
        T r;
        if constexpr (MODE == 0) r = dist0_from_ssq(acc[j], ks, rks);
        else if constexpr (sizeof(T) == 8) r = __builtin_sqrt(acc[j]);
        else r = __builtin_sqrtf(acc[j]);
        out[(size_t)b * H * W + (size_t)y * W + x] = r;
        if (!have) { mn = mx = (double)r; have = true; }
        else { mn = nan_min(mn, (double)r); mx = nan_max(mx, (double)r); }
    }
    __shared__ double seed[2];
    if (threadIdx.x == 0) { seed[0] = mn; seed[1] = mx; }
    __syncthreads();
    if (!have) { mn = seed[0]; mx = seed[1]; }
    block_minmax<TPB>(mn, mx, partials + (size_t)tile_id * 2);
}

constexpr int DMA_PER_WAVE = 4, DMA_UNITS = DMA_PER_WAVE * TPB;

__device__ __forceinline__ void glds16(const void *gsrc, unsigned lds_dst)
{
    unsigned keep;
    asm volatile("s_mov_b32 %0, m0\n\ts_mov_b32 m0, %2\n\ts_nop 0\n\tglobal_load_lds_dwordx4 %1, off\n\ts_mov_b32 m0, %0"
                 : "=&s"(keep) : "v"(gsrc), "s"(lds_dst) : "memory");
}

template <int MODE>
__global__ void __launch_bounds__(TPB) k_feat_reduce_lr_dma(const double *__restrict__ feat, long long bstride, int C, int h, int w,
                                                            int H, int W, double sh, double sw, int CC, double ks, double rks,
                                                            double *__restrict__ out, double *__restrict__ partials)
{
    typedef double T;
    extern __shared__ __attribute__((aligned(16))) unsigned char lr_smem[];
    T *img = reinterpret_cast<T *>(lr_smem);
    typedef __attribute__((address_space(3))) unsigned char *lds_bytes;
    const unsigned lds0 = (unsigned)(uintptr_t)(lds_bytes)lr_smem;
    const unsigned ntx = gridDim.x, nty = gridDim.y, ntiles = ntx * nty * gridDim.z;
    const unsigned lin = blockIdx.x + ntx * (blockIdx.y + nty * blockIdx.z);
    const unsigned xq = ntiles / 8, xr = ntiles % 8, xk = lin % 8;
    const unsigned tile_id = (xk < xr ? xk * (xq + 1) : xr * (xq + 1) + (xk - xr) * xq) + lin / 8;
    const int bx = (int)(tile_id % ntx), by = (int)((tile_id / ntx) % nty);
    const int b = (int)(tile_id / (ntx * nty));
    const int X0 = bx * LR_TW, Y0 = by * LR_TH;
    const int lx = threadIdx.x & (LR_TW - 1), ly = threadIdx.x / LR_TW;
    const int lane = threadIdx.x & 63, wv = threadIdx.x >> 6;
    const int x = X0 + lx;
    const int ylast = (Y0 + LR_TH - 1 < H ? Y0 + LR_TH - 1 : H - 1), xlast = (X0 + LR_TW - 1 < W ? X0 + LR_TW - 1 : W - 1);
    const int ty_lo = make_taps<T>(Y0, sh, h).i0, ty_hi = make_taps<T>(ylast, sh, h).i1;
    const int tx_lo = make_taps<T>(X0, sw, w).i0 & ~1, tx_hi = make_taps<T>(xlast, sw, w).i1;
    const int rows = ty_hi - ty_lo + 2;
    const int U = (tx_hi - tx_lo + 2 + 1) >> 1;
    const int per = rows * U, stride = 2 * U, plane = 2 * per;
    const bool xin = x < W;
    const Taps<T> tx = make_taps<T>(xin ? x : W - 1, sw, w);
    T acc[LR_PPT];
    LrW<T> wt;
    wt.lx0 = tx.l0; wt.lx1 = tx.l1;
    int o00[LR_PPT], o10[LR_PPT];
    bool live[LR_PPT];
    int a0 = 0, pat = 0;
    bool regular = true;
#pragma unroll
    for (int j = 0; j < LR_PPT; ++j) {
        const int y = Y0 + ly * LR_PPT + j;
        live[j] = xin && y < H;
        const Taps<T> ty = make_taps<T>(y < H ? y : H - 1, sh, h);
        wt.ly0[j] = ty.l0; wt.ly1[j] = ty.l1;
        o00[j] = (ty.i0 - ty_lo) * stride + (tx.i0 - tx_lo);
        o10[j] = (ty.i1 - ty_lo) * stride + (tx.i0 - tx_lo);
        acc[j] = (T)0;
        if (j == 0) a0 = ty.i0;
        const int d = ty.i0 - a0;
        regular = regular && (d == 0 || d == 1);
        if (j > 0) pat |= (d & 1) << (j - 1);
    }
    const int dx1 = tx.i1 - tx.i0;
    const int upat = __builtin_amdgcn_readfirstlane(regular ? pat : -1);
    const long long hwl = (long long)h * w;
    unsigned soff[DMA_PER_WAVE], sch[DMA_PER_WAVE];
#pragma unroll
    for (int i = 0; i < DMA_PER_WAVE; ++i) {
        const int u = (i * (TPB / 64) + wv) * 64 + lane;
        const int ch = u / per, rem = u - ch * per, r = rem / U, pp = rem - r * U;
        const int sr = ty_lo + r < h - 1 ? ty_lo + r : h - 1;
        int q0 = tx_lo + 2 * pp;
        q0 = q0 + 1 > w - 1 ? w - 2 : q0;
        sch[i] = (unsigned)ch;
        soff[i] = (unsigned)(sr * w + q0);
    }
    const T *fb = feat + (size_t)b * bstride;
    auto issue = [&](int c0, int buf) {
        const int cc = C - c0 < CC ? C - c0 : CC;
#pragma unroll
        for (int i = 0; i < DMA_PER_WAVE; ++i) {
            const unsigned ch = sch[i] < (unsigned)cc ? sch[i] : (unsigned)(cc - 1);
            const T *src = fb + (size_t)(c0 + ch) * hwl + soff[i];
            const unsigned dst = lds0 + (unsigned)buf * (DMA_UNITS * 16) + (unsigned)((i * (TPB / 64) + wv) * 64) * 16u;
            glds16(src, (unsigned)__builtin_amdgcn_readfirstlane((int)dst));
        }
    };
    const bool patch = tx_lo + 2 * U > w;
    const int nchunks = (C + CC - 1) / CC;
    issue(0, 0);
    for (int n = 0; n < nchunks; ++n) {
        const int c0 = n * CC, cc = C - c0 < CC ? C - c0 : CC;
        if (n + 1 < nchunks) {
            issue(c0 + CC, (n + 1) & 1);
            asm volatile("s_waitcnt vmcnt(%0)" ::"n"(DMA_PER_WAVE) : "memory");
        } else {
            asm volatile("s_waitcnt vmcnt(0)" ::: "memory");
        }
        __builtin_amdgcn_s_barrier();
        T *tile = img + (size_t)(n & 1) * (DMA_UNITS * 2);
        if (patch) {
            const int pu = (w - tx_lo) >> 1;
            for (int e = threadIdx.x; e < cc * rows; e += TPB) {
                T *q = tile + (size_t)(e / rows) * plane + (size_t)(e % rows) * stride + 2 * pu;
                q[0] = q[1];
            }
            asm volatile("s_waitcnt lgkmcnt(0)" ::: "memory");
            __builtin_amdgcn_s_barrier();
        }
        const T *t0 = tile + o00[0];
        if (upat == 0) lr_rows_chunk<T, 0>(t0, cc, plane, stride, wt, acc);
        else if (upat == 4) lr_rows_chunk<T, 4>(t0, cc, plane, stride, wt, acc);
        else if (upat == 6) lr_rows_chunk<T, 6>(t0, cc, plane, stride, wt, acc);
        else if (upat == 7) lr_rows_chunk<T, 7>(t0, cc, plane, stride, wt, acc);
        else {
#pragma unroll 1
            for (int ch = 0; ch < cc; ++ch) {
                const T *tp = tile + (size_t)ch * plane;
#pragma unroll
                for (int j = 0; j < LR_PPT; ++j) {
                    const T v = bilerp<T>(tp[o00[j]], tp[o00[j] + dx1], tp[o10[j]], tp[o10[j] + dx1], wt.lx0, wt.lx1, wt.ly0[j], wt.ly1[j]);
                    acc[j] = fma_t(v, v, acc[j]);
                }
            }
        }
        asm volatile("s_waitcnt lgkmcnt(0)" ::: "memory");
        __builtin_amdgcn_s_barrier();
    }
    double mn = 0.0, mx = 0.0;
    bool have = false;
#pragma unroll
    for (int j = 0; j < LR_PPT; ++j) {
        if (!live[j]) continue;
        const int y = Y0 + ly * LR_PPT + j;
        T r;
        if constexpr (MODE == 0) r = dist0_from_ssq(acc[j], ks, rks);
        else r = __builtin_sqrt(acc[j]);
        out[(size_t)b * H * W + (size_t)y * W + x] = r;
        if (!have) { mn = mx = (double)r; have = true; }
        else { mn = nan_min(mn, (double)r); mx = nan_max(mx, (double)r); }
    }
    __shared__ double seed[2];
    if (threadIdx.x == 0) { seed[0] = mn; seed[1] = mx; }
    __syncthreads();
    if (!have) { mn = seed[0]; mx = seed[1]; }
    block_minmax<TPB>(mn, mx, partials + (size_t)tile_id * 2);
}

template <int PAT, int OFF, int STRIDE_B> struct LrRowsImm {
    double v[3][2];
    __device__ __forceinline__ void issue(unsigned base)
    {
        if constexpr (PAT != 0) {
            asm volatile("ds_read_b64 %0, %6 offset:%7\n\tds_read_b64 %1, %6 offset:%8\n\tds_read_b64 %2, %6 offset:%9\n\t"
                         "ds_read_b64 %3, %6 offset:%10\n\tds_read_b64 %4, %6 offset:%11\n\tds_read_b64 %5, %6 offset:%12"
                         : "=&v"(v[0][0]), "=&v"(v[0][1]), "=&v"(v[1][0]), "=&v"(v[1][1]), "=&v"(v[2][0]), "=&v"(v[2][1])
                         : "v"(base), "n"(OFF), "n"(OFF + 8), "n"(OFF + STRIDE_B), "n"(OFF + STRIDE_B + 8), "n"(OFF + 2 * STRIDE_B),
                           "n"(OFF + 2 * STRIDE_B + 8)
                         : "memory");
        } else {
            asm volatile("ds_read_b64 %0, %4 offset:%5\n\tds_read_b64 %1, %4 offset:%6\n\tds_read_b64 %2, %4 offset:%7\n\t"
                         "ds_read_b64 %3, %4 offset:%8"
                         : "=&v"(v[0][0]), "=&v"(v[0][1]), "=&v"(v[1][0]), "=&v"(v[1][1])
                         : "v"(base), "n"(OFF), "n"(OFF + 8), "n"(OFF + STRIDE_B), "n"(OFF + STRIDE_B + 8)
                         : "memory");
        }
    }
    template <int N> __device__ __forceinline__ void wait()
    {
        if constexpr (PAT != 0)
            asm volatile("s_waitcnt lgkmcnt(%6)" : "+v"(v[0][0]), "+v"(v[0][1]), "+v"(v[1][0]), "+v"(v[1][1]), "+v"(v[2][0]), "+v"(v[2][1]) : "n"(N) : "memory");
        else
            asm volatile("s_waitcnt lgkmcnt(%4)" : "+v"(v[0][0]), "+v"(v[0][1]), "+v"(v[1][0]), "+v"(v[1][1]) : "n"(N) : "memory");
    }
    __device__ __forceinline__ void accumulate(const LrW<double> &wt, double (&acc)[LR_PPT]) const
    {
        double t[3];
        t[0] = col_lerp(wt.lx0, wt.lx1, v[0][0], v[0][1]);
        t[1] = col_lerp(wt.lx0, wt.lx1, v[1][0], v[1][1]);
        if constexpr (PAT != 0) t[2] = col_lerp(wt.lx0, wt.lx1, v[2][0], v[2][1]);
#pragma unroll
        for (int j = 0; j < LR_PPT; ++j) {
            const int a = j == 0 ? 0 : (PAT >> (j - 1)) & 1;
            const double x = col_lerp(wt.ly0[j], wt.ly1[j], t[a], t[a + 1]);
            acc[j] = fma_t(x, x, acc[j]);
        }
    }
};

template <int PAT, int ROWS, int UU, int CH, int CCF, bool FULL>
__device__ __forceinline__ void lr_imm_steps(unsigned base, int cc, LrRowsImm<PAT, (CH % CCF) * ROWS * UU * 16, UU * 16> &cur,
                                             const LrW<double> &wt, double (&acc)[LR_PPT])
{
    constexpr int NREAD = PAT != 0 ? 6 : 4;
    if constexpr (CH + 1 < CCF) {
        LrRowsImm<PAT, ((CH + 1) % CCF) * ROWS * UU * 16, UU * 16> nxt;
        nxt.issue(base);
        cur.template wait<NREAD>();
        if (FULL || CH < cc) cur.accumulate(wt, acc);
        lr_imm_steps<PAT, ROWS, UU, CH + 1, CCF, FULL>(base, cc, nxt, wt, acc);
    } else {
        cur.template wait<0>();
        if (FULL || CH < cc) cur.accumulate(wt, acc);
    }
}

template <int PAT, int ROWS, int UU, int CCF>
__device__ __forceinline__ void lr_imm_chunk(unsigned base, int cc, const LrW<double> &wt, double (&acc)[LR_PPT])
{
    if (cc == CCF) {
        LrRowsImm<PAT, 0, UU * 16> first;
        first.issue(base);
        lr_imm_steps<PAT, ROWS, UU, 0, CCF, true>(base, cc, first, wt, acc);
    } else {
        LrRowsImm<PAT, 0, UU * 16> first;
        first.issue(base);
        lr_imm_steps<PAT, ROWS, UU, 0, CCF, false>(base, cc, first, wt, acc);
    }
}

template <int NPX, unsigned CODE, int OFF, int STRIDE_B> struct LrRowsImmN {
    static constexpr int row(int j) { return (int)((CODE >> (2 * j)) & 3u); }
    static constexpr int NR = row(NPX - 1) + 2;
    double v[NR][2];
    template <int R> __device__ __forceinline__ void issue_rows(unsigned base)
    {
        if constexpr (R < NR) {
            asm volatile("ds_read_b64 %0, %2 offset:%3\n\tds_read_b64 %1, %2 offset:%4"
                         : "=&v"(v[R][0]), "=&v"(v[R][1]) : "v"(base), "n"(OFF + R * STRIDE_B), "n"(OFF + R * STRIDE_B + 8) : "memory");
            issue_rows<R + 1>(base);
        }
    }
    __device__ __forceinline__ void issue(unsigned base) { issue_rows<0>(base); }
    template <int N> __device__ __forceinline__ void wait()
    {
        asm volatile("s_waitcnt lgkmcnt(%0)" ::"n"(N) : "memory");
#pragma unroll
        for (int r = 0; r < NR; ++r) { asm volatile("" : "+v"(v[r][0])); asm volatile("" : "+v"(v[r][1])); }
    }
    __device__ __forceinline__ void accumulate(const LrW<double, NPX> &wt, double (&acc)[NPX]) const
    {
        double t[NR];
#pragma unroll
        for (int r = 0; r < NR; ++r) t[r] = col_lerp(wt.lx0, wt.lx1, v[r][0], v[r][1]);
#pragma unroll
        for (int j = 0; j < NPX; ++j) {
            const int a = row(j);
            const double x = col_lerp(wt.ly0[j], wt.ly1[j], t[a], t[a + 1]);
            acc[j] = fma_t(x, x, acc[j]);
        }
    }
};

template <int NPX, unsigned CODE, int ROWS, int UU, int CH, int CCF, bool FULL>
__device__ __forceinline__ void lr_immn_steps(unsigned base, int cc, LrRowsImmN<NPX, CODE, (CH % CCF) * ROWS * UU * 16, UU * 16> &cur,
                                              const LrW<double, NPX> &wt, double (&acc)[NPX])
{
    constexpr int NREAD = 2 * LrRowsImmN<NPX, CODE, 0, UU * 16>::NR;
    if constexpr (CH + 1 < CCF) {
        LrRowsImmN<NPX, CODE, ((CH + 1) % CCF) * ROWS * UU * 16, UU * 16> nxt;
        nxt.issue(base);
        cur.template wait<NREAD>();
        if (FULL || CH < cc) cur.accumulate(wt, acc);
        lr_immn_steps<NPX, CODE, ROWS, UU, CH + 1, CCF, FULL>(base, cc, nxt, wt, acc);
    } else {
        cur.template wait<0>();
        if (FULL || CH < cc) cur.accumulate(wt, acc);
    }
}
template <int NPX, unsigned CODE, int ROWS, int UU, int CCF>
__device__ __forceinline__ void lr_immn_chunk(unsigned base, int cc, const LrW<double, NPX> &wt, double (&acc)[NPX])
{
    if (cc == CCF) {
        LrRowsImmN<NPX, CODE, 0, UU * 16> first;
        first.issue(base);
        lr_immn_steps<NPX, CODE, ROWS, UU, 0, CCF, true>(base, cc, first, wt, acc);
    } else {
        LrRowsImmN<NPX, CODE, 0, UU * 16> first;
        first.issue(base);
        lr_immn_steps<NPX, CODE, ROWS, UU, 0, CCF, false>(base, cc, first, wt, acc);
    }
}

#ifndef HALO_LR8_WAVES
#define HALO_LR8_WAVES 3
#endif
#define HALO_LR_CODES8(X) \
    X(0x0000u) \
    X(0x5554u) X(0x5550u) X(0x5540u) X(0x5500u) X(0x5400u) X(0x5000u) X(0x4000u) \
    X(0xa954u) X(0xa554u) X(0x9554u) X(0xa550u) X(0x9550u) X(0x9540u) \
    X(0xaa54u) X(0xa950u) X(0xa540u) X(0x9500u)

template <int MODE, int ROWS, int UU, int PPT = LR_PPT>
__global__ void __launch_bounds__(TPB, (PPT > LR_PPT ? HALO_LR8_WAVES : 1)) k_feat_reduce_lr_dmaf(const double *__restrict__ feat, long long bstride, int C, int h, int w,
                                                             int H, int W, double sh, double sw, double ks, double rks,
                                                             double *__restrict__ out, double *__restrict__ partials)
{
    typedef double T;
    constexpr int PER = ROWS * UU, CCF = DMA_UNITS / PER, STRIDE = 2 * UU, PLANE = 2 * PER;
    constexpr int TH = PPT * (TPB / 64);
    extern __shared__ __attribute__((aligned(16))) unsigned char lr_smem[];
    T *img = reinterpret_cast<T *>(lr_smem);
    typedef __attribute__((address_space(3))) unsigned char *lds_bytes;
    const unsigned lds0 = (unsigned)(uintptr_t)(lds_bytes)lr_smem;
    const unsigned ntx = gridDim.x, nty = gridDim.y, ntiles = ntx * nty * gridDim.z;
    const unsigned lin = blockIdx.x + ntx * (blockIdx.y + nty * blockIdx.z);
    const unsigned xq = ntiles / 8, xr = ntiles % 8, xk = lin % 8;
    const unsigned tile_id = (xk < xr ? xk * (xq + 1) : xr * (xq + 1) + (xk - xr) * xq) + lin / 8;
    const int bx = (int)(tile_id % ntx), by = (int)((tile_id / ntx) % nty);
    const int b = (int)(tile_id / (ntx * nty));
    const int X0 = bx * LR_TW, Y0 = by * TH;
    const int lx = threadIdx.x & (LR_TW - 1), ly = threadIdx.x / LR_TW;
    const int lane = threadIdx.x & 63, wv = threadIdx.x >> 6;
    const int x = X0 + lx;
    const int xlast = (X0 + LR_TW - 1 < W ? X0 + LR_TW - 1 : W - 1);
    const int ty_lo = make_taps<T>(Y0, sh, h).i0;
    const int tx_lo = make_taps<T>(X0, sw, w).i0 & ~1, tx_hi = make_taps<T>(xlast, sw, w).i1;
    const bool xin = x < W;
    const Taps<T> tx = make_taps<T>(xin ? x : W - 1, sw, w);
    T acc[PPT];
    LrW<T, PPT> wt;
    wt.lx0 = tx.l0; wt.lx1 = tx.l1;
    int o00[PPT], o10[PPT];
    bool live[PPT];
    int a0 = 0, pat = 0;
    bool regular = true;
#pragma unroll
    for (int j = 0; j < PPT; ++j) {
        const int y = Y0 + ly * PPT + j;
        live[j] = xin && y < H;
        const Taps<T> ty = make_taps<T>(y < H ? y : H - 1, sh, h);
        wt.ly0[j] = ty.l0; wt.ly1[j] = ty.l1;
        o00[j] = (ty.i0 - ty_lo) * STRIDE + (tx.i0 - tx_lo);
        o10[j] = (ty.i1 - ty_lo) * STRIDE + (tx.i0 - tx_lo);
        acc[j] = (T)0;
        if (j == 0) a0 = ty.i0;
        const int d = ty.i0 - a0;
        if constexpr (PPT == LR_PPT) {
            regular = regular && (d == 0 || d == 1);
            if (j > 0) pat |= (d & 1) << (j - 1);
        } else {
            regular = regular && d >= 0 && d <= 3;
            pat |= (d & 3) << (2 * j);
        }
    }
    const int dx1 = tx.i1 - tx.i0;
    const int upat = __builtin_amdgcn_readfirstlane(regular ? pat : -1);
    const long long hwl = (long long)h * w;
    unsigned soff[DMA_PER_WAVE], sch[DMA_PER_WAVE];
#pragma unroll
    for (int i = 0; i < DMA_PER_WAVE; ++i) {
        const int u = (i * (TPB / 64) + wv) * 64 + lane;
        const int ch = u / PER, rem = u - ch * PER, r = rem / UU, pp = rem - r * UU;
        const int sr = ty_lo + r < h - 1 ? ty_lo + r : h - 1;
        int q0 = tx_lo + 2 * pp;
        q0 = q0 + 1 > w - 1 ? w - 2 : q0;
        sch[i] = (unsigned)(ch < CCF ? ch : CCF - 1);
        soff[i] = (unsigned)(sr * w + q0);
    }
    const T *fb = feat + (size_t)b * bstride;
    const T *sp[DMA_PER_WAVE];
#pragma unroll
    for (int i = 0; i < DMA_PER_WAVE; ++i) sp[i] = fb + (size_t)sch[i] * hwl + soff[i];
    const unsigned dst0 = (unsigned)__builtin_amdgcn_readfirstlane((int)(lds0 + (unsigned)(wv * 64) * 16u));
    auto issue = [&](int c0, int buf) {
        const int cc = C - c0 < CCF ? C - c0 : CCF;
        long long back[DMA_PER_WAVE];
#pragma unroll
        for (int i = 0; i < DMA_PER_WAVE; ++i) back[i] = 0;
        if (cc != CCF) {
#pragma unroll
            for (int i = 0; i < DMA_PER_WAVE; ++i) {
                const int ex = (int)sch[i] - (cc - 1);
                back[i] = ex > 0 ? (long long)ex * hwl : 0ll;
            }
        }
#pragma unroll
        for (int i = 0; i < DMA_PER_WAVE; ++i) {
            glds16(sp[i] - back[i], dst0 + (unsigned)buf * (DMA_UNITS * 16) + (unsigned)(i * (TPB / 64) * 64) * 16u);
            sp[i] += (size_t)CCF * hwl;
        }
    };
    const int pu = (w - tx_lo) >> 1;
    const bool patch = tx_hi + 1 >= w && pu < UU;
    const int nchunks = (C + CCF - 1) / CCF;
    issue(0, 0);
    for (int n = 0; n < nchunks; ++n) {
        const int c0 = n * CCF, cc = C - c0 < CCF ? C - c0 : CCF;
        if (n + 1 < nchunks) {
            issue(c0 + CCF, (n + 1) & 1);
            asm volatile("s_waitcnt vmcnt(%0)" ::"n"(DMA_PER_WAVE) : "memory");
        } else {
            asm volatile("s_waitcnt vmcnt(0)" ::: "memory");
        }
        __builtin_amdgcn_s_barrier();
        T *tile = img + (size_t)(n & 1) * (DMA_UNITS * 2);
        if (patch) {
            for (int e = threadIdx.x; e < cc * ROWS; e += TPB) {
                T *q = tile + (size_t)(e / ROWS) * PLANE + (size_t)(e % ROWS) * STRIDE + 2 * pu;
                q[0] = q[1];
            }
            asm volatile("s_waitcnt lgkmcnt(0)" ::: "memory");
            __builtin_amdgcn_s_barrier();
        }
        const unsigned base = lds0 + (unsigned)(n & 1) * (DMA_UNITS * 16) + (unsigned)o00[0] * 8u;
        bool done = false;
        if constexpr (PPT == LR_PPT) {
            done = true;
            if (upat == 0) lr_imm_chunk<0, ROWS, UU, CCF>(base, cc, wt, acc);
            else if (upat == 4) lr_imm_chunk<4, ROWS, UU, CCF>(base, cc, wt, acc);
            else if (upat == 6) lr_imm_chunk<6, ROWS, UU, CCF>(base, cc, wt, acc);
            else if (upat == 7) lr_imm_chunk<7, ROWS, UU, CCF>(base, cc, wt, acc);
            else done = false;
        } else {
            switch (upat) {
#define HALO_LR_CASE(CODE_) case (int)CODE_: lr_immn_chunk<PPT, CODE_, ROWS, UU, CCF>(base, cc, wt, acc); done = true; break;
                HALO_LR_CODES8(HALO_LR_CASE)
#undef HALO_LR_CASE
                default: break;
            }
        }
        if (!done) {
#pragma unroll 1
            for (int ch = 0; ch < cc; ++ch) {
                const T *tp = tile + (size_t)ch * PLANE;
#pragma unroll
                for (int j = 0; j < PPT; ++j) {
                    const T v = bilerp<T>(tp[o00[j]], tp[o00[j] + dx1], tp[o10[j]], tp[o10[j] + dx1], wt.lx0, wt.lx1, wt.ly0[j], wt.ly1[j]);
                    acc[j] = fma_t(v, v, acc[j]);
                }
            }
        }
        asm volatile("s_waitcnt lgkmcnt(0)" ::: "memory");
        __builtin_amdgcn_s_barrier();
    }
    double mn = 0.0, mx = 0.0;
    bool have = false;
#pragma unroll
    for (int j = 0; j < PPT; ++j) {
        if (!live[j]) continue;
        const int y = Y0 + ly * PPT + j;
        T r;
        if constexpr (MODE == 0) r = dist0_from_ssq(acc[j], ks, rks);
        else r = __builtin_sqrt(acc[j]);
        out[(size_t)b * H * W + (size_t)y * W + x] = r;
        if (!have) { mn = mx = (double)r; have = true; }
        else { mn = nan_min(mn, (double)r); mx = nan_max(mx, (double)r); }
    }
    __shared__ double seed[2];
    if (threadIdx.x == 0) { seed[0] = mn; seed[1] = mx; }
    __syncthreads();
    if (!have) { mn = seed[0]; mx = seed[1]; }
    block_minmax<TPB>(mn, mx, partials + (size_t)tile_id * 2);
}

constexpr int GRAM_MAPS = 5;
constexpr int GRAM_COLS = 63;

__device__ __forceinline__ double next_lane(double v)
{
    const long long u = __double_as_longlong(v);
    const int lo = __builtin_amdgcn_update_dpp(0, (int)(u & 0xffffffffll), 0x130 , 0xf, 0xf, false);
    const int hi = __builtin_amdgcn_update_dpp(0, (int)(u >> 32), 0x130, 0xf, 0xf, false);
    return __longlong_as_double(((long long)hi << 32) | (unsigned)lo);
}

__global__ void __launch_bounds__(TPB) k_gram_lr(const double *__restrict__ feat, long long bstride, int C, int h, int w,
                                                 double *__restrict__ gram)
{
    const int b = blockIdx.y, lane = threadIdx.x & 63;
    const unsigned per = gridDim.x / 8;
    const unsigned wid = ((blockIdx.x % 8) * per + blockIdx.x / 8) * (TPB / 64) + (threadIdx.x >> 6);
    const unsigned nwx = (unsigned)((w + GRAM_COLS - 1) / GRAM_COLS);
    const int y = 2 * (int)(wid / nwx);
    if (y >= h) return;
    const int xu = (int)(wid % nwx) * GRAM_COLS + lane, x = xu < w - 1 ? xu : w - 1;
    const int y1 = y + 1 < h - 1 ? y + 1 : h - 1, y2 = y + 2 < h - 1 ? y + 2 : h - 1;
    const unsigned a0 = (unsigned)(y * w + x), a1 = (unsigned)(y1 * w + x), a2 = (unsigned)(y2 * w + x);
    const int hwl = h * w;
    const double *p = feat + (size_t)b * bstride;
    double g0[GRAM_MAPS], g1[GRAM_MAPS];
#pragma unroll
    for (int k = 0; k < GRAM_MAPS; ++k) g0[k] = g1[k] = 0.0;
    auto accumulate = [&](double v0, double v1, double v2) {
        const double r0 = next_lane(v0), r1 = next_lane(v1), r2 = next_lane(v2);
        g0[0] = __builtin_fma(v0, v0, g0[0]); g0[1] = __builtin_fma(v0, r0, g0[1]); g0[2] = __builtin_fma(v0, v1, g0[2]);
        g0[3] = __builtin_fma(v0, r1, g0[3]); g0[4] = __builtin_fma(r0, v1, g0[4]);
        g1[0] = __builtin_fma(v1, v1, g1[0]); g1[1] = __builtin_fma(v1, r1, g1[1]); g1[2] = __builtin_fma(v1, v2, g1[2]);
        g1[3] = __builtin_fma(v1, r2, g1[3]); g1[4] = __builtin_fma(r1, v2, g1[4]);
    };
    int c = 0;
    for (; c + 4 <= C; c += 4) {
        double v[4][3];
#pragma unroll
        for (int u = 0; u < 4; ++u, p += hwl) { v[u][0] = p[a0]; v[u][1] = p[a1]; v[u][2] = p[a2]; }
#pragma unroll
        for (int u = 0; u < 4; ++u) accumulate(v[u][0], v[u][1], v[u][2]);
    }
    for (; c < C; ++c, p += hwl) accumulate(p[a0], p[a1], p[a2]);
    if (lane < GRAM_COLS && xu < w) {
        double *gb = gram + (size_t)b * GRAM_MAPS * hwl;
#pragma unroll
        for (int k = 0; k < GRAM_MAPS; ++k) gb[(size_t)k * hwl + a0] = g0[k];
        if (y + 1 < h) {
#pragma unroll
            for (int k = 0; k < GRAM_MAPS; ++k) gb[(size_t)k * hwl + a1] = g1[k];
        }
    }
}

template <int UCH, int R>
__global__ void __launch_bounds__(TPB) k_gram_lr2(const double *__restrict__ feat, long long bstride, int C, int h, int w,
                                                  double *__restrict__ gram)
{
    const int b = blockIdx.y, lane = threadIdx.x & 63;
    const unsigned per = gridDim.x / 8;
    const unsigned wid = ((blockIdx.x % 8) * per + blockIdx.x / 8) * (TPB / 64) + (threadIdx.x >> 6);
    const unsigned nwx = (unsigned)((w + 127) / 128);
    const int y = R * (int)(wid / nwx);
    if (y >= h) return;
    const int xu = (int)(wid % nwx) * 128 + 2 * lane;
    const int x = xu < w - 2 ? xu : w - 2;
    const int xr = xu + 2 < w - 1 ? xu + 2 : w - 1;
    unsigned a[R + 1], e[R + 1];
#pragma unroll
    for (int r = 0; r <= R; ++r) {
        const int yr = y + r < h - 1 ? y + r : h - 1;
        a[r] = (unsigned)(yr * w + x);
        e[r] = (unsigned)(yr * w + xr);
    }
    const int hwl = h * w;
    const double *p = feat + (size_t)b * bstride;
    double g[R][2][GRAM_MAPS];
#pragma unroll
    for (int r = 0; r < R; ++r)
#pragma unroll
        for (int q = 0; q < 2; ++q)
#pragma unroll
            for (int k = 0; k < GRAM_MAPS; ++k) g[r][q][k] = 0.0;
    const bool last = lane == 63, edge = xu + 2 >= w;
    auto accumulate = [&](const d2_t (&v)[R + 1], const double (&xx)[R + 1]) {
        double cc[R + 1][2], rr[R + 1][2];
#pragma unroll
        for (int r = 0; r <= R; ++r) {
            const double sh = next_lane(v[r].x);
            const double nb = edge ? v[r].y : (last ? xx[r] : sh);
            cc[r][0] = v[r].x; cc[r][1] = v[r].y; rr[r][0] = v[r].y; rr[r][1] = nb;
        }
#pragma unroll
        for (int r = 0; r < R; ++r)
#pragma unroll
            for (int q = 0; q < 2; ++q) {
                g[r][q][0] = __builtin_fma(cc[r][q], cc[r][q], g[r][q][0]); g[r][q][1] = __builtin_fma(cc[r][q], rr[r][q], g[r][q][1]);
                g[r][q][2] = __builtin_fma(cc[r][q], cc[r + 1][q], g[r][q][2]); g[r][q][3] = __builtin_fma(cc[r][q], rr[r + 1][q], g[r][q][3]);
                g[r][q][4] = __builtin_fma(rr[r][q], cc[r + 1][q], g[r][q][4]);
            }
    };
    auto ld2 = [](const double *q) -> d2_t { return *reinterpret_cast<const d2_t *>(q); };
    int c = 0;
    for (; c + UCH <= C; c += UCH) {
        d2_t v[UCH][R + 1];
        double xe[UCH][R + 1];
#pragma unroll
        for (int u = 0; u < UCH; ++u, p += hwl) {
#pragma unroll
            for (int r = 0; r <= R; ++r) { v[u][r] = ld2(p + a[r]); xe[u][r] = 0.0; }
            if (last) {
#pragma unroll
                for (int r = 0; r <= R; ++r) xe[u][r] = p[e[r]];
            }
        }
#pragma unroll
        for (int u = 0; u < UCH; ++u) accumulate(v[u], xe[u]);
    }
    for (; c < C; ++c, p += hwl) {
        d2_t v[R + 1];
        double xx[R + 1];
#pragma unroll
        for (int r = 0; r <= R; ++r) { v[r] = *reinterpret_cast<const d2_t *>(p + a[r]); xx[r] = last ? p[e[r]] : 0.0; }
        accumulate(v, xx);
    }
    if (xu < w) {
        double *gb = gram + (size_t)b * GRAM_MAPS * hwl;
#pragma unroll
        for (int r = 0; r < R; ++r)
            if (y + r < h) {
#pragma unroll
                for (int k = 0; k < GRAM_MAPS; ++k) *reinterpret_cast<d2_t *>(gb + (size_t)k * hwl + a[r]) = (d2_t){g[r][0][k], g[r][1][k]};
            }
    }
}

constexpr double GRAM_GUARD = 0x1p-10;

template <int MODE>
__global__ void __launch_bounds__(TPB) k_radius_gram(const double *__restrict__ gram, const double *__restrict__ feat, long long bstride,
                                                     int C, int h, int w, int H, int W, double sh, double sw,
                                                     double ks, double rks, double *__restrict__ out, double *__restrict__ partials)
{
    const int b = blockIdx.y;
    const long long hw = (long long)H * W;
    const long long i = (long long)blockIdx.x * TPB + threadIdx.x;
    const bool live = i < hw;
    double mn = 0.0, mx = 0.0;
    if (live) {
        int y, x;
        if (hw <= 0x7fffffffll) { const unsigned iu = (unsigned)i; y = (int)(iu / (unsigned)W); x = (int)(iu - (unsigned)y * (unsigned)W); }
        else { y = (int)(i / W); x = (int)(i % W); }
        const Taps<double> ty = make_taps<double>(y, sh, h), tx = make_taps<double>(x, sw, w);
        const double wt[4] = {ty.l0 * tx.l0, ty.l0 * tx.l1, ty.l1 * tx.l0, ty.l1 * tx.l1};
        const size_t hwl = (size_t)h * w;
        const double *S = gram + (size_t)b * GRAM_MAPS * hwl, *Hh = S + hwl, *Vv = Hh + hwl, *D1 = Vv + hwl, *D2 = D1 + hwl;
        const unsigned c00 = (unsigned)(ty.i0 * w + tx.i0), c01 = (unsigned)(ty.i0 * w + tx.i1), c10 = (unsigned)(ty.i1 * w + tx.i0),
                       c11 = (unsigned)(ty.i1 * w + tx.i1);
        const double G[10] = {S[c00], Hh[c00], Vv[c00], D1[c00], S[c01], D2[c00], Vv[c01], S[c10], Hh[c10], S[c11]};
        double s = 0.0, t = 0.0;
        int k = 0;
#pragma unroll
        for (int a = 0; a < 4; ++a)
#pragma unroll
            for (int c2 = a; c2 < 4; ++c2, ++k) {
                double coef = wt[a] * wt[c2];
                if (c2 != a) coef = coef + coef;
                s = __builtin_fma(coef, G[k], s);
                t = __builtin_fma(coef, __builtin_fabs(G[k]), t);
            }
        if (s < t * GRAM_GUARD) {
            const double *pl = feat + (size_t)b * bstride;
            double acc = 0.0;
            for (int ch = 0; ch < C; ++ch, pl += hwl) {
                const double v = bilerp<double>(pl[c00], pl[c01], pl[c10], pl[c11], tx.l0, tx.l1, ty.l0, ty.l1);
                acc = __builtin_fma(v, v, acc);
            }
            s = acc;
        }
        double r;
        if constexpr (MODE == 0) r = dist0_from_ssq(s, ks, rks);
        else r = __builtin_sqrt(s);
        out[(size_t)b * hw + i] = r;
        mn = mx = r;
    }
    __shared__ double seed[2];
    if (threadIdx.x == 0) { seed[0] = mn; seed[1] = mx; }
    __syncthreads();
    if (!live) { mn = seed[0]; mx = seed[1]; }
    block_minmax<TPB>(mn, mx, partials + ((size_t)b * gridDim.x + blockIdx.x) * 2);
}

template <int O_T>
__global__ void __launch_bounds__(TPB) k_logit_maps_lr(const float *__restrict__ logit, long long bstride, int h, int w, int H, int W,
                                                       float sh, float sw, const long long *__restrict__ gt, int unc_type,
                                                       int pur_type, float *__restrict__ ent, short *__restrict__ pred)
{
    const int b = blockIdx.y;
    const long long hw = (long long)H * W;
    const long long i = (long long)blockIdx.x * TPB + threadIdx.x;
#if HALO_LOGF_LDS
    __shared__ double s_ltab[128][2];
    stage_logf_table<TPB>(s_ltab);
    const double (*ltab)[2] = s_ltab;
#else
    const double (*ltab)[2] = logf_tab_;
#endif
    if (i >= hw) return;
    const int y = (int)(i / W), x = (int)(i % W);
    const Taps<float> ty = make_taps<float>(y, sh, h), tx = make_taps<float>(x, sw, w);
    const char *pl = reinterpret_cast<const char *>(logit + (size_t)b * bstride);
    const unsigned a00 = (unsigned)(ty.i0 * w + tx.i0) * 4u, a01 = (unsigned)(ty.i0 * w + tx.i1) * 4u,
                   a10 = (unsigned)(ty.i1 * w + tx.i0) * 4u, a11 = (unsigned)(ty.i1 * w + tx.i1) * 4u;
    const size_t plane_bytes = (size_t)h * w * 4;
    auto at = [](const char *base, unsigned off) { return *reinterpret_cast<const float *>(base + off); };
    float p[1][O_T];
#pragma unroll
    for (int c = 0; c < O_T; ++c, pl += plane_bytes)
        p[0][c] = bilerp<float>(at(pl, a00), at(pl, a01), at(pl, a10), at(pl, a11), tx.l0, tx.l1, ty.l0, ty.l1);
    const bool need_gt = unc_type == HALO_UNC_ORACLE_ACC || pur_type == HALO_PUR_ORACLE_RIPU;
    const long long g[1] = {need_gt ? gt[(size_t)b * hw + i] : 0};
    float e[1];
    int pr[1];
    if (softmax_lean<O_T, 1>(p)) {
        finish_px<O_T, 1, true>(p, unc_type, pur_type, g, e, pr, pred != nullptr, ltab);
    } else {
        softmax_general<O_T, 1>(p);
        finish_px<O_T, 1, false>(p, unc_type, pur_type, g, e, pr, pred != nullptr);
    }
    ent[(size_t)b * hw + i] = e[0];
    if (pred) pred[(size_t)b * hw + i] = (short)pr[0];
}

__global__ void __launch_bounds__(TPB) k_logit_interp_lr(const float *__restrict__ logit, long long bstride, int O, int h, int w, int H,
                                                         int W, float sh, float sw, float *__restrict__ dst)
{
    const int b = blockIdx.y;
    const long long hw = (long long)H * W;
    const long long i = (long long)blockIdx.x * TPB + threadIdx.x;
    if (i >= hw) return;
    const int y = (int)(i / W), x = (int)(i % W);
    const Taps<float> ty = make_taps<float>(y, sh, h), tx = make_taps<float>(x, sw, w);
    const float *lb = logit + (size_t)b * bstride;
    for (int c = 0; c < O; ++c) {
        const float *pl = lb + (size_t)c * h * w;
        dst[((size_t)b * O + c) * hw + i] = bilerp<float>(pl[(size_t)ty.i0 * w + tx.i0], pl[(size_t)ty.i0 * w + tx.i1],
                                                          pl[(size_t)ty.i1 * w + tx.i0], pl[(size_t)ty.i1 * w + tx.i1], tx.l0, tx.l1, ty.l0, ty.l1);
    }
}

static inline bool aligned16(const void *p) { return ((uintptr_t)p & 15) == 0; }

struct FusedLogit { const float *logit; long long bstride; int O; int unc_type; float *ent; };

template <typename T, int VEC>
static void launch_feat(const T *feat, long long bstride, int C, long long hw, int B, int mode, double ks, double rks,
                        T *out, double *partials, int nblk, hipStream_t st, const FusedLogit *fl = nullptr)
{
    dim3 grid(nblk, B), block(FTPB);
    constexpr int UNROLL = HALO_FEAT_UNROLL;
    unsigned xcd_g = 256;
    while (xcd_g > 1 && 8 * xcd_g > (unsigned)nblk) xcd_g >>= 1;
    if (8 * xcd_g > (unsigned)nblk) xcd_g = 0;
#define HALO_FEAT(M, FO_)                                                                                               \
    hipLaunchKernelGGL((k_feat_reduce<T, VEC, M, UNROLL, FO_>), grid, block, 0, st, feat, bstride, C, hw, ks, rks, out, \
                       partials, fl ? fl->logit : nullptr, fl ? fl->bstride : 0ll, fl ? fl->unc_type : 0, fl ? fl->ent : nullptr, \
                       xcd_g)
    const int fo = fl ? fl->O : 0;
    if (mode == 0) {
        if (fo == 19) HALO_FEAT(0, 19); else if (fo == 16) HALO_FEAT(0, 16); else HALO_FEAT(0, 0);
    } else {
        if (fo == 19) HALO_FEAT(1, 19); else if (fo == 16) HALO_FEAT(1, 16); else HALO_FEAT(1, 0);
    }
#undef HALO_FEAT
}

}

using namespace halo;

static_assert(RI_TW == LR_TW && RI_TH == LR_TH, "k_region_impurity3 writes one min/max partial per tile of the same shape");
static size_t partial_slots(int64_t H, int64_t W)
{
    const size_t a = (size_t)cdiv(H * W, FTPB), b = (size_t)(cdiv(W, LR_TW) * cdiv(H, LR_TH));
    return a > b ? a : b;
}

extern "C" size_t halo_score_workspace_bytes(int64_t B, int64_t H, int64_t W)
{
    if (B <= 0 || H <= 0 || W <= 0) return 0;
    const size_t n = (size_t)B * H * W;
    const size_t nblk = partial_slots(H, W);
    size_t s = 0;
    s += align_up(n * 4, 256);
    s += align_up(n * 4, 256);
    s += align_up(n * 8, 256);
    s += align_up(n * 2, 256);
    s += 2 * align_up((size_t)B * nblk * 2 * 8, 256);
    s += align_up((size_t)B * 4 * 8, 256);
    return s + 1024;
}

extern "C" int halo_score_maps(const float *logit, int64_t logit_bstride, const void *feat, int feat_dtype,
                               int64_t feat_bstride, const int64_t *gt, const uint8_t *active, int64_t B, int64_t O,
                               int64_t C, int64_t H, int64_t W, int unc_type, int pur_type, int normalize, int ksize,
                               int pksize, int64_t K, double c, void *score, void *impurity, float *uncertainty,
                               void *workspace, size_t workspace_bytes, void *stream)
{
    return halo_score_maps_timed(logit, logit_bstride, feat, feat_dtype, feat_bstride, gt, active, B, O, C, H, W, unc_type,
                                 pur_type, normalize, ksize, pksize, K, c, score, impurity, uncertainty, workspace,
                                 workspace_bytes, stream, nullptr, nullptr, nullptr);
}

extern "C" size_t halo_score_lr_workspace_bytes(int64_t B, int64_t O, int64_t H, int64_t W)
{
    const size_t base = halo_score_workspace_bytes(B, H, W);
    if (base == 0 || O <= 0) return 0;
    return base + ((O == 19 || O == 16) ? 0 : (size_t)B * O * H * W * 4 + 512);
}

extern "C" size_t halo_score_lr_gram_workspace_bytes(int64_t B, int64_t O, int64_t H, int64_t W, int64_t hf, int64_t wf)
{
    const size_t base = halo_score_lr_workspace_bytes(B, O, H, W);
    if (base == 0 || hf <= 0 || wf <= 0) return 0;
    return base + (size_t)B * 5 * hf * wf * 8 + 512;
}

struct LrDims { int hl, wl, hf, wf; bool gram; };

template <typename T>
static void lr_window(int out_size, int in_size, int tile, int &max_span)
{
    const T sc = out_size > 1 ? (T)(in_size - 1) / (T)(out_size - 1) : (T)0;
    max_span = 1;
    for (int o0 = 0; o0 < out_size; o0 += tile) {
        const int ol = o0 + tile - 1 < out_size ? o0 + tile - 1 : out_size - 1;
        T f = sc * (T)o0; int lo = (int)f; lo = lo > in_size - 1 ? in_size - 1 : lo;
        f = sc * (T)ol; int hi = (int)f; hi = hi > in_size - 1 ? in_size - 1 : hi; hi = hi + (hi < in_size - 1 ? 1 : 0);
        if (hi - lo + 1 > max_span) max_span = hi - lo + 1;
    }
}

template <typename T>
static int launch_feat_lr(const T *feat, long long bstride, int C, const LrDims &lr, int H, int W, int B, int mode, double ks,
                          double rks, T *out, double *partials, int &nblk, hipStream_t st)
{
    int max_rows, max_cols;
    lr_window<T>(H, lr.hf, LR_TH, max_rows);
    lr_window<T>(W, lr.wf, LR_TW, max_cols);
    ++max_rows; ++max_cols;
    const T sh = H > 1 ? (T)(lr.hf - 1) / (T)(H - 1) : (T)0, sw = W > 1 ? (T)(lr.wf - 1) / (T)(W - 1) : (T)0;
    dim3 grid((unsigned)cdiv(W, LR_TW), (unsigned)cdiv(H, LR_TH), (unsigned)B), block(TPB);
    nblk = (int)(grid.x * grid.y);
    if constexpr (sizeof(T) == 8) {
        const int units_per_ch = max_rows * ((max_cols + 2) / 2 + 1);
        int CCd = DMA_UNITS / units_per_ch;
        CCd = CCd > C ? C : CCd;
        const bool dma_ok = lr.wf >= 2 && lr.wf % 2 == 0 && bstride % 2 == 0 && aligned16(feat) && CCd >= 4;
        if (dma_ok) {
            const size_t lds = 2 * (size_t)DMA_UNITS * 16;
            const int need_rows = max_rows, need_u = (max_cols + 2) / 2;
            if ((double)sh <= 1.0 / 3.0 && H >= 2 * LR_TH) {
                int max_rows8;
                lr_window<T>(H, lr.hf, 2 * LR_TH, max_rows8);
                ++max_rows8;
                dim3 grid8((unsigned)cdiv(W, LR_TW), (unsigned)cdiv(H, 2 * LR_TH), (unsigned)B);
#define HALO_LR_FIXED8(R_, U_)                                                                                                             \
                if (max_rows8 <= R_ && need_u <= U_) {                                                                                     \
                    nblk = (int)(grid8.x * grid8.y);                                                                                       \
                    if (mode == 0) hipLaunchKernelGGL((k_feat_reduce_lr_dmaf<0, R_, U_, 2 * LR_PPT>), grid8, block, lds, st, (const double *)feat, bstride, C, lr.hf, lr.wf, H, W, (double)sh, (double)sw, ks, rks, (double *)out, partials); \
                    else hipLaunchKernelGGL((k_feat_reduce_lr_dmaf<1, R_, U_, 2 * LR_PPT>), grid8, block, lds, st, (const double *)feat, bstride, C, lr.hf, lr.wf, H, W, (double)sh, (double)sw, ks, rks, (double *)out, partials);           \
                    return HALO_OK;                                                                                                        \
                }
                HALO_LR_FIXED8(8, 8)
                HALO_LR_FIXED8(11, 10)
#undef HALO_LR_FIXED8
            }
#define HALO_LR_FIXED(R_, U_)                                                                                                              \
            if (need_rows <= R_ && need_u <= U_) {                                                                                         \
                if (mode == 0) hipLaunchKernelGGL((k_feat_reduce_lr_dmaf<0, R_, U_>), grid, block, lds, st, (const double *)feat, bstride, C, lr.hf, lr.wf, H, W, (double)sh, (double)sw, ks, rks, (double *)out, partials); \
                else hipLaunchKernelGGL((k_feat_reduce_lr_dmaf<1, R_, U_>), grid, block, lds, st, (const double *)feat, bstride, C, lr.hf, lr.wf, H, W, (double)sh, (double)sw, ks, rks, (double *)out, partials);           \
                return HALO_OK;                                                                                                            \
            }
            HALO_LR_FIXED(6, 8)
            HALO_LR_FIXED(7, 10)
            HALO_LR_FIXED(8, 12)
#undef HALO_LR_FIXED
            if (mode == 0) hipLaunchKernelGGL((k_feat_reduce_lr_dma<0>), grid, block, lds, st, (const double *)feat, bstride, C, lr.hf, lr.wf, H, W, (double)sh, (double)sw, CCd, ks, rks, (double *)out, partials);
            else hipLaunchKernelGGL((k_feat_reduce_lr_dma<1>), grid, block, lds, st, (const double *)feat, bstride, C, lr.hf, lr.wf, H, W, (double)sh, (double)sw, CCd, ks, rks, (double *)out, partials);
            return HALO_OK;
        }
    }
    const size_t plane_bytes = (size_t)max_rows * max_cols * sizeof(T);
    if (plane_bytes > 48 * 1024) return fail(HALO_E_UNSUPPORTED, "halo_score_maps_lr: source window too large for LDS (downsampling?)");
    int CC = (int)((48 * 1024) / plane_bytes);
    CC = CC > (TPB / 64) * LR_STAGE_G ? (TPB / 64) * LR_STAGE_G : CC;
    CC = CC > C ? C : CC;
    const size_t lds = (size_t)CC * plane_bytes;
    if (mode == 0) hipLaunchKernelGGL((k_feat_reduce_lr<T, 0>), grid, block, lds, st, feat, bstride, C, lr.hf, lr.wf, H, W, sh, sw, max_rows, max_cols, CC, ks, rks, out, partials);
    else hipLaunchKernelGGL((k_feat_reduce_lr<T, 1>), grid, block, lds, st, feat, bstride, C, lr.hf, lr.wf, H, W, sh, sw, max_rows, max_cols, CC, ks, rks, out, partials);
    return HALO_OK;
}

static int check_padding(int pad, int k, int64_t H, int64_t W, const char *who)
{
    if (pad < HALO_PAD_ZEROS || pad > HALO_PAD_CIRCULAR) return fail(HALO_E_ARG, "%s: bad padding mode %d", who, pad);
    const int64_t r = k / 2, m = H < W ? H : W;
    if (pad == HALO_PAD_REFLECT && r >= m)
        return fail(HALO_E_ARG, "%s: padding_mode='reflect' needs the padding (%lld) to be smaller than the map (%lld x %lld)", who, (long long)r, (long long)H, (long long)W);
    if (pad == HALO_PAD_CIRCULAR && r > m)
        return fail(HALO_E_ARG, "%s: padding_mode='circular' needs the padding (%lld) to be at most the map size (%lld x %lld)", who, (long long)r, (long long)H, (long long)W);
    return HALO_OK;
}

static int score_impl(const float *logit, int64_t logit_bstride, const void *feat, int feat_dtype,
                      int64_t feat_bstride, const int64_t *gt, const uint8_t *active, int64_t B, int64_t O,
                      int64_t C, int64_t H, int64_t W, int unc_type, int pur_type, int normalize, int ksize,
                      int pksize, int64_t K, double c, void *score, void *impurity, float *uncertainty,
                      void *workspace, size_t workspace_bytes, void *stream, void *ev_feat_start,
                      void *ev_feat_stop, const LrDims *lr, void *ev_logit_start = nullptr, void *ev_logit_stop = nullptr,
                      void *score_range = nullptr, void *tail_stream = nullptr, void *ev_feat_mid = nullptr, void *ev_tail_stop = nullptr)
{
    hipStream_t st = (hipStream_t)stream;
    const int pad = (normalize >> 8) & 3;
    if (normalize & ~(HALO_FLAG_NORMALIZE | (3 << 8))) return fail(HALO_E_ARG, "halo_score_maps: unknown flag bits 0x%x", normalize);
    normalize &= HALO_FLAG_NORMALIZE;
    if (!logit || !score || B <= 0 || O <= 0 || H <= 0 || W <= 0) return fail(HALO_E_ARG, "halo_score_maps: null/empty argument");
    if (unc_type < 0 || unc_type > HALO_UNC_ZEROS) return fail(HALO_E_ARG, "halo_score_maps: bad unc_type %d", unc_type);
    if (pur_type < 0 || pur_type > HALO_PUR_EUC_NORM) return fail(HALO_E_UNSUPPORTED, "Error: purity type '%d' not implemented", pur_type);
    if (ksize < 1 || !(ksize & 1) || pksize < 1 || !(pksize & 1)) return fail(HALO_E_ARG, "halo_score_maps: window sizes must be odd");
    {
        const int rc = check_padding(pad, ksize > pksize ? ksize : pksize, H, W, "halo_score_maps");
        if (rc != HALO_OK) return rc;
    }
    const bool need_feat = pur_type == HALO_PUR_HYPER || pur_type == HALO_PUR_RADIUS || pur_type == HALO_PUR_EUC_NORM;
    if (need_feat && (!feat || C <= 0)) return fail(HALO_E_ARG, "halo_score_maps: decoder_out required for this purity type");
    if (need_feat && feat_dtype != HALO_F32 && feat_dtype != HALO_F64) return fail(HALO_E_ARG, "halo_score_maps: bad feat dtype");
    const bool need_gt = unc_type == HALO_UNC_ORACLE_ACC || pur_type == HALO_PUR_ORACLE_RIPU;
    if (need_gt && !gt) return fail(HALO_E_ARG, "halo_score_maps: ground_truth required");
    if (pur_type == HALO_PUR_HYPER && (K < 1 || K > 32767)) return fail(HALO_E_UNSUPPORTED, "halo_score_maps: K out of range");
    if (O > 32767) return fail(HALO_E_UNSUPPORTED, "halo_score_maps: too many classes");
    if (workspace_bytes < halo_score_workspace_bytes(B, H, W) || !workspace) return fail(HALO_E_WORKSPACE, "halo_score_maps: workspace too small");
    const bool lr_generic_O = lr && !(O == 19 || O == 16);
    if (lr_generic_O && workspace_bytes < halo_score_workspace_bytes(B, H, W) + (size_t)B * O * H * W * 4 + 256)
        return fail(HALO_E_WORKSPACE, "halo_score_maps_lr: workspace too small for %d classes", (int)O);

    const long long hw = (long long)H * W;
    const int nblk1 = (int)cdiv(hw, TPB);
    Arena ar(workspace, workspace_bytes);
    float *ent = ar.take<float>((size_t)B * hw);
    float *unc_raw = ar.take<float>((size_t)B * hw);
    double *imp_raw = ar.take<double>((size_t)B * hw);
    short *pred = ar.take<short>((size_t)B * hw);
    double *part_imp = ar.take<double>((size_t)B * partial_slots(H, W) * 2);
    double *part_unc = ar.take<double>((size_t)B * partial_slots(H, W) * 2);
    double *stats = ar.take<double>((size_t)B * 4);
    float *lr_logit_full = lr_generic_O ? ar.take<float>((size_t)B * O * hw) : nullptr;
    const bool gram_mode = lr && lr->gram && need_feat;
    if (gram_mode && feat_dtype != HALO_F64) return fail(HALO_E_UNSUPPORTED, "halo_score_maps_lr_gram: float64 embeddings only");
    double *gram = gram_mode ? ar.take<double>((size_t)B * GRAM_MAPS * lr->hf * lr->wf) : nullptr;
    if (!ar.ok()) return fail(HALO_E_WORKSPACE, "halo_score_maps: workspace too small");

    const bool f64out = (pur_type == HALO_PUR_RADIUS || pur_type == HALO_PUR_EUC_NORM) && feat_dtype == HALO_F64;
    const bool hist = pur_type == HALO_PUR_RIPU || pur_type == HALO_PUR_ORACLE_RIPU || pur_type == HALO_PUR_HYPER;
    const double ks = sqrt(fabs(-c) + 1e-15), rks = 1.0 / ks;
    dim3 block(TPB);

    const bool ent_only = (unc_type == HALO_UNC_ENTROPY || unc_type == HALO_UNC_PIXEL_ENTROPY) &&
                          pur_type != HALO_PUR_RIPU && pur_type != HALO_PUR_ORACLE_RIPU;
    const int fvec = !need_feat ? 0 : (feat_dtype == HALO_F64
        ? (((hw % 2 == 0) && (feat_bstride % 2 == 0) && aligned16(feat) && aligned16(imp_raw)) ? 2 : 1)
        : (((hw % 4 == 0) && (feat_bstride % 4 == 0) && aligned16(feat) && aligned16(imp_raw)) ? 4 : 1));
    const bool fuse = !lr && need_feat && ent_only && (O == 19 || O == 16) && fvec > 1 && (logit_bstride % fvec == 0) &&
                      (((uintptr_t)logit) % (4 * fvec) == 0);
    FusedLogit fl{logit, (long long)logit_bstride, (int)O, unc_type, ent};
    const FusedLogit *flp = fuse ? &fl : nullptr;
    const bool need_logit_pass = !fuse && ( unc_type != HALO_UNC_ZEROS || pur_type == HALO_PUR_RIPU || pur_type == HALO_PUR_ORACLE_RIPU);
    short *pred_from_logits = (pur_type == HALO_PUR_RIPU || pur_type == HALO_PUR_ORACLE_RIPU) ? pred : nullptr;
    if (ev_logit_start) (void)hipEventRecord((hipEvent_t)ev_logit_start, st);
    if (need_logit_pass && lr) {
        const float shl = H > 1 ? (float)(lr->hl - 1) / (float)(H - 1) : 0.0f, swl = W > 1 ? (float)(lr->wl - 1) / (float)(W - 1) : 0.0f;
        dim3 grid((unsigned)nblk1, (unsigned)B);
        if (O == 19)
            hipLaunchKernelGGL((k_logit_maps_lr<19>), grid, block, 0, st, logit, (long long)logit_bstride, lr->hl, lr->wl, (int)H, (int)W, shl, swl, (const long long *)gt, unc_type, pur_type, ent, pred_from_logits);
        else if (O == 16)
            hipLaunchKernelGGL((k_logit_maps_lr<16>), grid, block, 0, st, logit, (long long)logit_bstride, lr->hl, lr->wl, (int)H, (int)W, shl, swl, (const long long *)gt, unc_type, pur_type, ent, pred_from_logits);
        else {
            hipLaunchKernelGGL(k_logit_interp_lr, grid, block, 0, st, logit, (long long)logit_bstride, (int)O, lr->hl, lr->wl, (int)H, (int)W, shl, swl, lr_logit_full);
            hipLaunchKernelGGL(k_logit_maps_generic, grid, block, 0, st, (const float *)lr_logit_full, (long long)(O * hw), (const long long *)gt, (int)O, hw, unc_type, pur_type, 0, ent, pred_from_logits);
        }
    } else if (need_logit_pass) {
        const bool vec4 = (hw % 4 == 0) && (logit_bstride % 4 == 0) && aligned16(logit) && aligned16(ent);
        if (O == 19 && vec4) {
            dim3 grid((unsigned)cdiv(hw, TPB * 4), (unsigned)B);
            hipLaunchKernelGGL((k_logit_maps<19, 4>), grid, block, 0, st, logit, (long long)logit_bstride, (const long long *)gt, hw, unc_type, pur_type, ent, pred_from_logits);
        } else if (O == 16 && vec4) {
            dim3 grid((unsigned)cdiv(hw, TPB * 4), (unsigned)B);
            hipLaunchKernelGGL((k_logit_maps<16, 4>), grid, block, 0, st, logit, (long long)logit_bstride, (const long long *)gt, hw, unc_type, pur_type, ent, pred_from_logits);
        } else {
            dim3 grid((unsigned)nblk1, (unsigned)B);
            hipLaunchKernelGGL(k_logit_maps_generic, grid, block, 0, st, logit, (long long)logit_bstride, (const long long *)gt, (int)O, hw, unc_type, pur_type, 0, ent, pred_from_logits);
        }
    } else if (!fuse) {
        hipLaunchKernelGGL(k_fill_f32, dim3((unsigned)cdiv(B * hw, TPB)), block, 0, st, ent, (long long)(B * hw), 0.0f);
    }

    if (ev_logit_stop) (void)hipEventRecord((hipEvent_t)ev_logit_stop, st);

    int nblk_imp = nblk1;
    if (need_feat) {
        if (ev_feat_start) (void)hipEventRecord((hipEvent_t)ev_feat_start, st);
        const int mode = pur_type == HALO_PUR_EUC_NORM ? 1 : 0;
        if (gram_mode) {
            const bool wide = lr->wf >= 2 && lr->wf % 2 == 0 && feat_bstride % 2 == 0 && aligned16(feat) && aligned16(gram);
            if (wide) {
                const long long nwx = cdiv(lr->wf, 128);
                int rows = 2;
                for (int cand = 8; cand > 2; cand >>= 1)
                    if (B * nwx * cdiv(lr->hf, cand) >= 1024) { rows = cand; break; }
                const long long nwaves = nwx * cdiv(lr->hf, rows);
                const dim3 gg((unsigned)(cdiv(cdiv(nwaves, TPB / 64), 8) * 8), (unsigned)B);
#define HALO_GRAM2(U_, R_) hipLaunchKernelGGL((k_gram_lr2<U_, R_>), gg, block, 0, st, (const double *)feat, (long long)feat_bstride, (int)C, lr->hf, lr->wf, gram)
                if (rows == 8) HALO_GRAM2(1, 8);
                else if (rows == 4) HALO_GRAM2(2, 4);
                else HALO_GRAM2(2, 2);
#undef HALO_GRAM2
            } else {
                const long long nwaves = cdiv(lr->wf, GRAM_COLS) * cdiv(lr->hf, 2);
                hipLaunchKernelGGL(k_gram_lr, dim3((unsigned)(cdiv(cdiv(nwaves, TPB / 64), 8) * 8), (unsigned)B), block, 0, st, (const double *)feat,
                                   (long long)feat_bstride, (int)C, lr->hf, lr->wf, gram);
            }
            if (ev_feat_mid) (void)hipEventRecord((hipEvent_t)ev_feat_mid, st);
            const double shd = H > 1 ? (double)(lr->hf - 1) / (double)(H - 1) : 0.0, swd = W > 1 ? (double)(lr->wf - 1) / (double)(W - 1) : 0.0;
            nblk_imp = nblk1;
            if (mode == 0) hipLaunchKernelGGL(k_radius_gram<0>, dim3((unsigned)nblk1, (unsigned)B), block, 0, st, gram, (const double *)feat, (long long)feat_bstride, (int)C, lr->hf, lr->wf, (int)H, (int)W, shd, swd, ks, rks, imp_raw, part_imp);
            else hipLaunchKernelGGL(k_radius_gram<1>, dim3((unsigned)nblk1, (unsigned)B), block, 0, st, gram, (const double *)feat, (long long)feat_bstride, (int)C, lr->hf, lr->wf, (int)H, (int)W, shd, swd, ks, rks, imp_raw, part_imp);
        } else if (lr) {
            const int rc = feat_dtype == HALO_F64
                ? launch_feat_lr<double>((const double *)feat, feat_bstride, (int)C, *lr, (int)H, (int)W, (int)B, mode, ks, rks, imp_raw, part_imp, nblk_imp, st)
                : launch_feat_lr<float>((const float *)feat, feat_bstride, (int)C, *lr, (int)H, (int)W, (int)B, mode, ks, rks, (float *)imp_raw, part_imp, nblk_imp, st);
            if (rc != HALO_OK) return rc;
        } else if (feat_dtype == HALO_F64) {
            const bool v2 = (hw % 2 == 0) && (feat_bstride % 2 == 0) && aligned16(feat) && aligned16(imp_raw);
            if (v2) { nblk_imp = (int)cdiv(hw, FTPB * 2); launch_feat<double, 2>((const double *)feat, feat_bstride, (int)C, hw, (int)B, mode, ks, rks, imp_raw, part_imp, nblk_imp, st, flp); }
            else { nblk_imp = (int)cdiv(hw, FTPB); launch_feat<double, 1>((const double *)feat, feat_bstride, (int)C, hw, (int)B, mode, ks, rks, imp_raw, part_imp, nblk_imp, st); }
        } else {
            const bool v4 = (hw % 4 == 0) && (feat_bstride % 4 == 0) && aligned16(feat) && aligned16(imp_raw);
            if (v4) { nblk_imp = (int)cdiv(hw, FTPB * 4); launch_feat<float, 4>((const float *)feat, feat_bstride, (int)C, hw, (int)B, mode, ks, rks, (float *)imp_raw, part_imp, nblk_imp, st, flp); }
            else { nblk_imp = (int)cdiv(hw, FTPB); launch_feat<float, 1>((const float *)feat, feat_bstride, (int)C, hw, (int)B, mode, ks, rks, (float *)imp_raw, part_imp, nblk_imp, st); }
        }
        if (ev_feat_stop) (void)hipEventRecord((hipEvent_t)ev_feat_stop, st);
    }
    if (tail_stream && (hipStream_t)tail_stream != st) {
        if (!need_feat || !ev_feat_stop) return fail(HALO_E_ARG, "halo_score_maps_split: a purity type that reads decoder_out and ev_feat_stop are required with a tail stream");
        if (hipStreamWaitEvent((hipStream_t)tail_stream, (hipEvent_t)ev_feat_stop, 0) != hipSuccess)
            return fail(HALO_E_LAUNCH, "halo_score_maps_split: hipStreamWaitEvent: %s", hipGetErrorString(hipGetLastError()));
        st = (hipStream_t)tail_stream;
    }
    dim3 grid1((unsigned)nblk1, (unsigned)B);
    if (pur_type == HALO_PUR_HYPER) {
        hipLaunchKernelGGL(k_minmax_finalize, dim3((unsigned)B), block, 0, st, part_imp, nblk_imp, stats, 0);
        if (feat_dtype == HALO_F64) hipLaunchKernelGGL((k_quantize<double, short>), grid1, block, 0, st, (const double *)imp_raw, stats, hw, (int)K, pred);
        else hipLaunchKernelGGL((k_quantize<float, short>), grid1, block, 0, st, (const float *)imp_raw, stats, hw, (int)K, pred);
    }
    if (hist) {
        const float logK = (float)log((double)(pur_type == HALO_PUR_HYPER ? K : O));
        const int np = launch_region_impurity<short>((const short *)pred, B, H, W, pksize, logK, (float *)imp_raw, (float *)nullptr, st,
                                                     normalize ? part_imp : nullptr, pad);
        nblk_imp = np ? np : nblk1;
        if (normalize && !np) hipLaunchKernelGGL(k_minmax_f32, grid1, block, 0, st, (const float *)imp_raw, hw, part_imp);
    } else if (pur_type == HALO_PUR_NONE) {
        hipLaunchKernelGGL(k_fill_f32, dim3((unsigned)cdiv(B * hw, TPB)), block, 0, st, (float *)imp_raw, (long long)(B * hw), 0.0f);
        if (normalize) hipLaunchKernelGGL(k_minmax_f32, grid1, block, 0, st, (const float *)imp_raw, hw, part_imp);
        nblk_imp = nblk1;
    }

    const int do_box = (unc_type == HALO_UNC_ENTROPY || unc_type == HALO_UNC_ORACLE_ACC) ? 1 : 0;
    int nblk_unc = nblk1;
    const bool box3 = do_box && pad == HALO_PAD_ZEROS && ksize == 3 && W % 4 == 0 && aligned16(ent) && aligned16(unc_raw);
    const bool fuse_tail = box3 && B <= 65535 && H <= 65535 && aligned16(imp_raw) && aligned16(score) && (!impurity || aligned16(impurity)) &&
                           (!uncertainty || aligned16(uncertainty)) && (!active || ((uintptr_t)active & 3) == 0);
    const int nblk_c3 = (int)cdiv(hw, TPB * 4);
    unsigned *rng_hist = (score_range && normalize && fuse_tail)
                             ? (unsigned *)((char *)score_range + range_hist_offset(B)) : nullptr;
    if (fuse_tail) {
        if (normalize) {
            const dim3 gridm((unsigned)cdiv(W, BM_TW), (unsigned)cdiv(H, BM_TH), (unsigned)B);
            nblk_unc = (int)(gridm.x * gridm.y);
            hipLaunchKernelGGL(k_box3_minmax, gridm, block, 0, st, (const float *)ent, (int)H, (int)W, hist ? pksize : 0, part_unc, rng_hist);
        }
    } else if (box3) {
        nblk_unc = nblk_c3;
        hipLaunchKernelGGL(k_box3_unc, dim3((unsigned)nblk_unc, (unsigned)B), block, 0, st, (const float *)ent, (int)H, (int)W,
                           hist ? pksize : 0, unc_raw, normalize ? part_unc : nullptr);
    } else {
        hipLaunchKernelGGL(k_box_unc, grid1, block, 0, st, ent, (int)H, (int)W, ksize, do_box, hist ? pksize : 0, unc_raw,
                           normalize ? part_unc : nullptr, pad);
    }

    SelHdr *rng_free = (score_range && normalize && fuse_tail) ? (SelHdr *)score_range : nullptr;
    if (normalize)
        hipLaunchKernelGGL(k_minmax_finalize2, dim3((unsigned)B, 2u), dim3(FIN_TPB), 0, st, (const double *)part_imp, nblk_imp,
                           (const double *)part_unc, nblk_unc, stats);
    if (fuse_tail) {
        int crows = CB_ROWS;
        while (crows > 1 && cdiv(W, TPB * 4) * cdiv(H, crows) * B < 1024) crows >>= 1;
        dim3 gridc((unsigned)cdiv(W, TPB * 4), (unsigned)cdiv(H, crows), (unsigned)B);
#define HALO_CB(T) hipLaunchKernelGGL((k_combine_box3<T>), gridc, block, 0, st, (const T *)imp_raw, (const float *)ent, stats, active, (int)H, (int)W, hist ? pksize : 0, normalize, (T *)score, (T *)impurity, uncertainty, rng_free, rng_hist, crows)
        if (f64out) HALO_CB(double);
        else HALO_CB(float);
#undef HALO_CB
    } else if (f64out) hipLaunchKernelGGL((k_combine<double>), grid1, block, 0, st, (const double *)imp_raw, unc_raw, stats, active, hw, normalize, (double *)score, (double *)impurity, uncertainty);
    else hipLaunchKernelGGL((k_combine<float>), grid1, block, 0, st, (const float *)imp_raw, unc_raw, stats, active, hw, normalize, (float *)score, (float *)impurity, uncertainty);
    if (score_range && !rng_free) {
        const int rc = score_range_exact(score, f64out ? HALO_F64 : HALO_F32, B, hw, score_range, st);
        if (rc != HALO_OK) return rc;
    }
    if (ev_tail_stop) (void)hipEventRecord((hipEvent_t)ev_tail_stop, st);
    return check_launch("halo_score_maps");
}

extern "C" int halo_region_uncertainty(const float *x, int64_t bstride, int is_prob, const int64_t *gt, int64_t B, int64_t O,
                                       int64_t H, int64_t W, int unc_type, int ksize, int do_box, float *out,
                                       void *workspace, size_t workspace_bytes, void *stream)
{
    hipStream_t st = (hipStream_t)stream;
    const int pad = (do_box >> 8) & 3;
    do_box &= 1;
    if (!x || !out || B <= 0 || O <= 0 || H <= 0 || W <= 0) return fail(HALO_E_ARG, "halo_region_uncertainty: null/empty argument");
    if (unc_type < 0 || unc_type > HALO_UNC_ZEROS) return fail(HALO_E_ARG, "halo_region_uncertainty: bad unc_type");
    if (unc_type == HALO_UNC_ORACLE_ACC && !gt) return fail(HALO_E_ARG, "halo_region_uncertainty: ground_truth required");
    if (ksize < 1 || !(ksize & 1)) return fail(HALO_E_ARG, "halo_region_uncertainty: window size must be odd");
    if (do_box) { const int rc = check_padding(pad, ksize, H, W, "halo_region_uncertainty"); if (rc != HALO_OK) return rc; }
    const long long hw = (long long)H * W;
    if (!workspace || workspace_bytes < (size_t)B * hw * 4 + 256) return fail(HALO_E_WORKSPACE, "halo_region_uncertainty: workspace too small");
    float *ent = (float *)(((uintptr_t)workspace + 255) & ~(uintptr_t)255);
    dim3 block(TPB), grid1((unsigned)cdiv(hw, TPB), (unsigned)B);
    float *dst = do_box ? ent : out;
    if (unc_type == HALO_UNC_ZEROS)
        hipLaunchKernelGGL(k_fill_f32, dim3((unsigned)cdiv(B * hw, TPB)), block, 0, st, dst, (long long)(B * hw), 0.0f);
    else
        hipLaunchKernelGGL(k_logit_maps_generic, grid1, block, 0, st, x, (long long)bstride, (const long long *)gt, (int)O, hw,
                           unc_type, HALO_PUR_NONE, is_prob, dst, (short *)nullptr);
    if (do_box)
        hipLaunchKernelGGL(k_box_unc, grid1, block, 0, st, (const float *)ent, (int)H, (int)W, ksize, 1, 0, out, (double *)nullptr, pad);
    return check_launch("halo_region_uncertainty");
}

extern "C" int halo_region_impurity(const int64_t *pred, int64_t B, int64_t H, int64_t W, int ksize, int64_t K, float *impurity,
                                    float *count, int pad_mode, void *stream)
{
    if (!pred || !impurity || B <= 0 || H <= 0 || W <= 0 || K < 1) return fail(HALO_E_ARG, "halo_region_impurity: null/empty argument");
    if (ksize < 1 || !(ksize & 1)) return fail(HALO_E_ARG, "halo_region_impurity: window size must be odd");
    { const int rc = check_padding(pad_mode, ksize, H, W, "halo_region_impurity"); if (rc != HALO_OK) return rc; }
    launch_region_impurity<long long>((const long long *)pred, B, H, W, ksize, (float)log((double)K), impurity, count, (hipStream_t)stream,
                                      nullptr, pad_mode);
    return check_launch("halo_region_impurity");
}

extern "C" int halo_quantize_radius(const void *feat, int feat_dtype, int64_t feat_bstride, int64_t B, int64_t C, int64_t H,
                                    int64_t W, int64_t K, double c, int64_t *pred, void *workspace, size_t workspace_bytes,
                                    void *stream)
{
    hipStream_t st = (hipStream_t)stream;
    if (!feat || !pred || B <= 0 || C <= 0 || H <= 0 || W <= 0 || K < 1) return fail(HALO_E_ARG, "halo_quantize_radius: null/empty argument");
    if (feat_dtype != HALO_F32 && feat_dtype != HALO_F64) return fail(HALO_E_ARG, "halo_quantize_radius: bad dtype");
    if (!workspace || workspace_bytes < halo_score_workspace_bytes(B, H, W)) return fail(HALO_E_WORKSPACE, "halo_quantize_radius: workspace too small");
    const long long hw = (long long)H * W;
    const int nblk1 = (int)cdiv(hw, TPB), nblkf = (int)cdiv(hw, FTPB);
    Arena ar(workspace, workspace_bytes);
    double *imp_raw = ar.take<double>((size_t)B * hw);
    double *part = ar.take<double>((size_t)B * nblkf * 2);
    double *stats = ar.take<double>((size_t)B * 4);
    if (!ar.ok()) return fail(HALO_E_WORKSPACE, "halo_quantize_radius: workspace too small");
    const double ks = sqrt(fabs(-c) + 1e-15), rks = 1.0 / ks;
    dim3 block(TPB), grid1((unsigned)nblk1, (unsigned)B);
    if (feat_dtype == HALO_F64) {
        launch_feat<double, 1>((const double *)feat, feat_bstride, (int)C, hw, (int)B, 0, ks, rks, imp_raw, part, nblkf, st);
        hipLaunchKernelGGL(k_minmax_finalize, dim3((unsigned)B), block, 0, st, (const double *)part, nblkf, stats, 0);
        hipLaunchKernelGGL((k_quantize<double, long long>), grid1, block, 0, st, (const double *)imp_raw, (const double *)stats, hw, (int)K, (long long *)pred);
    } else {
        launch_feat<float, 1>((const float *)feat, feat_bstride, (int)C, hw, (int)B, 0, ks, rks, (float *)imp_raw, part, nblkf, st);
        hipLaunchKernelGGL(k_minmax_finalize, dim3((unsigned)B), block, 0, st, (const double *)part, nblkf, stats, 0);
        hipLaunchKernelGGL((k_quantize<float, long long>), grid1, block, 0, st, (const float *)imp_raw, (const double *)stats, hw, (int)K, (long long *)pred);
    }
    return check_launch("halo_quantize_radius");
}

extern "C" int halo_score_maps_timed(const float *logit, int64_t logit_bstride, const void *feat, int feat_dtype,
                                     int64_t feat_bstride, const int64_t *gt, const uint8_t *active, int64_t B, int64_t O,
                                     int64_t C, int64_t H, int64_t W, int unc_type, int pur_type, int normalize, int ksize,
                                     int pksize, int64_t K, double c, void *score, void *impurity, float *uncertainty,
                                     void *workspace, size_t workspace_bytes, void *stream, void *ev_feat_start,
                                     void *ev_feat_stop, void *score_range)
{
    return score_impl(logit, logit_bstride, feat, feat_dtype, feat_bstride, gt, active, B, O, C, H, W, unc_type, pur_type,
                      normalize, ksize, pksize, K, c, score, impurity, uncertainty, workspace, workspace_bytes, stream,
                      ev_feat_start, ev_feat_stop, nullptr, nullptr, nullptr, score_range);
}

extern "C" int halo_score_maps_split(const float *logit, int64_t logit_bstride, const void *feat, int feat_dtype,
                                     int64_t feat_bstride, const int64_t *gt, const uint8_t *active, int64_t B, int64_t O,
                                     int64_t C, int64_t H, int64_t W, int unc_type, int pur_type, int normalize, int ksize,
                                     int pksize, int64_t K, double c, void *score, void *impurity, float *uncertainty,
                                     void *workspace, size_t workspace_bytes, void *stream, void *tail_stream, void *ev_feat_start,
                                     void *ev_feat_stop, void *score_range)
{
    return score_impl(logit, logit_bstride, feat, feat_dtype, feat_bstride, gt, active, B, O, C, H, W, unc_type, pur_type,
                      normalize, ksize, pksize, K, c, score, impurity, uncertainty, workspace, workspace_bytes, stream,
                      ev_feat_start, ev_feat_stop, nullptr, nullptr, nullptr, score_range, tail_stream);
}

extern "C" int halo_score_maps_lr(const float *logit_lr, int64_t logit_bstride, int64_t hl, int64_t wl, const void *feat_lr,
                                  int feat_dtype, int64_t feat_bstride, int64_t hf, int64_t wf, const int64_t *gt,
                                  const uint8_t *active, int64_t B, int64_t O, int64_t C, int64_t H, int64_t W, int unc_type,
                                  int pur_type, int normalize, int ksize, int pksize, int64_t K, double c, void *score,
                                  void *impurity, float *uncertainty, void *workspace, size_t workspace_bytes, void *stream)
{
    if (hl <= 0 || wl <= 0) return fail(HALO_E_ARG, "halo_score_maps_lr: bad low-res logit size");
    const bool need_feat = pur_type == HALO_PUR_HYPER || pur_type == HALO_PUR_RADIUS || pur_type == HALO_PUR_EUC_NORM;
    if (need_feat && (hf <= 0 || wf <= 0)) return fail(HALO_E_ARG, "halo_score_maps_lr: bad low-res embedding size");
    LrDims lr{(int)hl, (int)wl, (int)hf, (int)wf, false};
    return score_impl(logit_lr, logit_bstride, feat_lr, feat_dtype, feat_bstride, gt, active, B, O, C, H, W, unc_type, pur_type,
                      normalize, ksize, pksize, K, c, score, impurity, uncertainty, workspace, workspace_bytes, stream, nullptr,
                      nullptr, &lr);
}

extern "C" int halo_score_maps_lr_gram(const float *logit_lr, int64_t logit_bstride, int64_t hl, int64_t wl, const void *feat_lr,
                                       int feat_dtype, int64_t feat_bstride, int64_t hf, int64_t wf, const int64_t *gt,
                                       const uint8_t *active, int64_t B, int64_t O, int64_t C, int64_t H, int64_t W, int unc_type,
                                       int pur_type, int normalize, int ksize, int pksize, int64_t K, double c, void *score,
                                       void *impurity, float *uncertainty, void *workspace, size_t workspace_bytes, void *stream)
{
    if (hl <= 0 || wl <= 0) return fail(HALO_E_ARG, "halo_score_maps_lr_gram: bad low-res logit size");
    const bool need_feat = pur_type == HALO_PUR_HYPER || pur_type == HALO_PUR_RADIUS || pur_type == HALO_PUR_EUC_NORM;
    if (need_feat && (hf <= 0 || wf <= 0)) return fail(HALO_E_ARG, "halo_score_maps_lr_gram: bad low-res embedding size");
    if (need_feat && hf * wf > 0x7fffffffll) return fail(HALO_E_UNSUPPORTED, "halo_score_maps_lr_gram: low-res planes of more than 2^31 elements");
    if (need_feat && workspace_bytes < halo_score_lr_gram_workspace_bytes(B, O, H, W, hf, wf))
        return fail(HALO_E_WORKSPACE, "halo_score_maps_lr_gram: workspace too small");
    LrDims lr{(int)hl, (int)wl, (int)hf, (int)wf, true};
    return score_impl(logit_lr, logit_bstride, feat_lr, feat_dtype, feat_bstride, gt, active, B, O, C, H, W, unc_type, pur_type,
                      normalize, ksize, pksize, K, c, score, impurity, uncertainty, workspace, workspace_bytes, stream, nullptr,
                      nullptr, &lr);
}

extern "C" int halo_score_maps_lr_timed(const float *logit_lr, int64_t logit_bstride, int64_t hl, int64_t wl, const void *feat_lr,
                                        int feat_dtype, int64_t feat_bstride, int64_t hf, int64_t wf, const int64_t *gt,
                                        const uint8_t *active, int64_t B, int64_t O, int64_t C, int64_t H, int64_t W, int unc_type,
                                        int pur_type, int normalize, int ksize, int pksize, int64_t K, double c, void *score,
                                        void *impurity, float *uncertainty, void *workspace, size_t workspace_bytes, void *stream,
                                        int gram, void *ev_logit_start, void *ev_logit_stop, void *ev_feat_start, void *ev_feat_stop,
                                        void *score_range, void *ev_feat_mid, void *ev_tail_stop)
{
    if (hl <= 0 || wl <= 0) return fail(HALO_E_ARG, "halo_score_maps_lr_timed: bad low-res logit size");
    const bool need_feat = pur_type == HALO_PUR_HYPER || pur_type == HALO_PUR_RADIUS || pur_type == HALO_PUR_EUC_NORM;
    if (need_feat && (hf <= 0 || wf <= 0)) return fail(HALO_E_ARG, "halo_score_maps_lr_timed: bad low-res embedding size");
    if (gram && need_feat && workspace_bytes < halo_score_lr_gram_workspace_bytes(B, O, H, W, hf, wf))
        return fail(HALO_E_WORKSPACE, "halo_score_maps_lr_timed: workspace too small");
    LrDims lr{(int)hl, (int)wl, (int)hf, (int)wf, gram != 0};
    return score_impl(logit_lr, logit_bstride, feat_lr, feat_dtype, feat_bstride, gt, active, B, O, C, H, W, unc_type, pur_type,
                      normalize, ksize, pksize, K, c, score, impurity, uncertainty, workspace, workspace_bytes, stream, ev_feat_start,
                      ev_feat_stop, &lr, ev_logit_start, ev_logit_stop, score_range, nullptr, ev_feat_mid, ev_tail_stop);
}
```

### include/halo_hip.h

```cpp
#ifndef HALO_HIP_H
#define HALO_HIP_H

#include <stddef.h>
#include <stdint.h>

#ifdef __cplusplus
extern "C" {
#endif

#define HALO_ABI_VERSION 10

enum { HALO_F32 = 0, HALO_F64 = 1, HALO_I64 = 2, HALO_I32 = 3, HALO_U8 = 4 };

enum { HALO_OK = 0, HALO_E_ARG = -1, HALO_E_UNSUPPORTED = -2, HALO_E_WORKSPACE = -3, HALO_E_LAUNCH = -4 };

enum { HALO_UNC_ENTROPY = 0, HALO_UNC_PIXEL_ENTROPY = 1, HALO_UNC_ORACLE_ACC = 2, HALO_UNC_ZEROS = 3 };

enum { HALO_PAD_ZEROS = 0, HALO_PAD_REFLECT = 1, HALO_PAD_REPLICATE = 2, HALO_PAD_CIRCULAR = 3 };
enum { HALO_FLAG_NORMALIZE = 1 };
#define HALO_FLAG_PAD(mode) ((mode) << 8)

enum { HALO_PUR_RIPU = 0, HALO_PUR_ORACLE_RIPU = 1, HALO_PUR_HYPER = 2, HALO_PUR_NONE = 3,
       HALO_PUR_RADIUS = 4, HALO_PUR_EUC_NORM = 5 };

int halo_version(void);
const char *halo_last_error(void);


int halo_expmap0_project(const void *x, int x_dtype, double *y, int64_t outer, int64_t C, int64_t inner,
                         double c, void *stream);

int halo_logmap0_project(const double *x, double *y, int64_t outer, int64_t C, int64_t inner, double c,
                         void *stream);

int halo_dist0(const void *x, int dtype, void *out, int64_t outer, int64_t C, int64_t inner, double c,
               void *stream);

int halo_pdist(const double *x, const double *y, double *out, int64_t n, int64_t d, double c, void *stream);

size_t halo_hypermlr_workspace_bytes(int64_t O, int64_t C);
int halo_hypermlr_logits(const double *x, const double *P, const double *A, void *out, int out_dtype,
                         int64_t B, int64_t C, int64_t O, int64_t hw, double c, void *workspace,
                         size_t workspace_bytes, void *stream);

int halo_head_tail(const float *feat, const double *P, const double *A, double *embed, void *out, int out_dtype, int64_t B,
                   int64_t C, int64_t O, int64_t hw, double c, void *workspace, size_t workspace_bytes, void *stream);

int halo_expmap0_project_bwd(const void *x, int x_dtype, const double *gy, void *gx, int64_t outer, int64_t C,
                             int64_t inner, double c, void *stream);
int halo_hypermlr_bwd_terms(const double *x, const double *P, const double *A, const double *gout, int64_t B, int64_t C,
                            int64_t O, int64_t hw, double c, double *dpx, double *dxa, double *dxx, double *dpp,
                            double *dpa, double *dan, void *workspace, size_t workspace_bytes, void *stream);

size_t halo_hypermlr_backward_workspace_bytes(int64_t B, int64_t C, int64_t O, int64_t hw);
int halo_hypermlr_backward(const double *x, const double *P, const double *A, const void *gout, int gout_dtype, int64_t B, int64_t C,
                           int64_t O, int64_t hw, double c, double *gx, double *gP, double *gA, void *workspace,
                           size_t workspace_bytes, void *stream);

int halo_bilinear_upsample(const void *src, void *dst, int dtype, int64_t planes, int64_t h, int64_t w,
                           int64_t H, int64_t W, void *stream);

int halo_bilinear_upsample_bwd(const void *grad_out, void *grad_in, int dtype, int64_t planes, int64_t h, int64_t w,
                               int64_t H, int64_t W, void *stream);

size_t halo_score_workspace_bytes(int64_t B, int64_t H, int64_t W);
int halo_score_maps(const float *logit, int64_t logit_bstride, const void *feat, int feat_dtype,
                    int64_t feat_bstride, const int64_t *gt, const uint8_t *active, int64_t B, int64_t O,
                    int64_t C, int64_t H, int64_t W, int unc_type, int pur_type, int normalize, int ksize,
                    int pksize, int64_t K, double c, void *score, void *impurity, float *uncertainty,
                    void *workspace, size_t workspace_bytes, void *stream);

int halo_score_maps_timed(const float *logit, int64_t logit_bstride, const void *feat, int feat_dtype,
                          int64_t feat_bstride, const int64_t *gt, const uint8_t *active, int64_t B, int64_t O,
                          int64_t C, int64_t H, int64_t W, int unc_type, int pur_type, int normalize, int ksize,
                          int pksize, int64_t K, double c, void *score, void *impurity, float *uncertainty,
                          void *workspace, size_t workspace_bytes, void *stream, void *ev_feat_start,
                          void *ev_feat_stop, void *score_range);

int halo_score_maps_split(const float *logit, int64_t logit_bstride, const void *feat, int feat_dtype,
                          int64_t feat_bstride, const int64_t *gt, const uint8_t *active, int64_t B, int64_t O,
                          int64_t C, int64_t H, int64_t W, int unc_type, int pur_type, int normalize, int ksize,
                          int pksize, int64_t K, double c, void *score, void *impurity, float *uncertainty,
                          void *workspace, size_t workspace_bytes, void *stream, void *tail_stream, void *ev_feat_start,
                          void *ev_feat_stop, void *score_range);

size_t halo_score_lr_workspace_bytes(int64_t B, int64_t O, int64_t H, int64_t W);
int halo_score_maps_lr(const float *logit_lr, int64_t logit_bstride, int64_t hl, int64_t wl, const void *feat_lr,
                       int feat_dtype, int64_t feat_bstride, int64_t hf, int64_t wf, const int64_t *gt,
                       const uint8_t *active, int64_t B, int64_t O, int64_t C, int64_t H, int64_t W, int unc_type,
                       int pur_type, int normalize, int ksize, int pksize, int64_t K, double c, void *score,
                       void *impurity, float *uncertainty, void *workspace, size_t workspace_bytes, void *stream);

size_t halo_score_lr_gram_workspace_bytes(int64_t B, int64_t O, int64_t H, int64_t W, int64_t hf, int64_t wf);
int halo_score_maps_lr_gram(const float *logit_lr, int64_t logit_bstride, int64_t hl, int64_t wl, const void *feat_lr,
                            int feat_dtype, int64_t feat_bstride, int64_t hf, int64_t wf, const int64_t *gt,
                            const uint8_t *active, int64_t B, int64_t O, int64_t C, int64_t H, int64_t W, int unc_type,
                            int pur_type, int normalize, int ksize, int pksize, int64_t K, double c, void *score,
                            void *impurity, float *uncertainty, void *workspace, size_t workspace_bytes, void *stream);

int halo_score_maps_lr_timed(const float *logit_lr, int64_t logit_bstride, int64_t hl, int64_t wl, const void *feat_lr,
                             int feat_dtype, int64_t feat_bstride, int64_t hf, int64_t wf, const int64_t *gt,
                             const uint8_t *active, int64_t B, int64_t O, int64_t C, int64_t H, int64_t W, int unc_type,
                             int pur_type, int normalize, int ksize, int pksize, int64_t K, double c, void *score,
                             void *impurity, float *uncertainty, void *workspace, size_t workspace_bytes, void *stream,
                             int gram, void *ev_logit_start, void *ev_logit_stop, void *ev_feat_start, void *ev_feat_stop,
                             void *score_range, void *ev_feat_mid, void *ev_tail_stop);

int halo_region_uncertainty(const float *x, int64_t bstride, int is_prob, const int64_t *gt, int64_t B, int64_t O,
                            int64_t H, int64_t W, int unc_type, int ksize, int do_box, float *out, void *workspace,
                            size_t workspace_bytes, void *stream);
int halo_region_impurity(const int64_t *pred, int64_t B, int64_t H, int64_t W, int ksize, int64_t K, float *impurity,
                         float *count, int pad_mode, void *stream);
int halo_quantize_radius(const void *feat, int feat_dtype, int64_t feat_bstride, int64_t B, int64_t C, int64_t H,
                         int64_t W, int64_t K, double c, int64_t *pred, void *workspace, size_t workspace_bytes,
                         void *stream);

enum { HALO_SELECT_AUTO = 0, HALO_SELECT_SERIAL = 1, HALO_SELECT_BINNED = 2 };
size_t halo_select_workspace_bytes(int64_t B, int64_t H, int64_t W, int64_t n_regions, int64_t mask_radius);
int halo_greedy_select(void *score, int dtype, int64_t B, int64_t H, int64_t W, int64_t n_regions,
                       int64_t active_radius, int64_t mask_radius, uint8_t *active, uint8_t *selected,
                       int64_t *active_mask, const int64_t *gt, double *picks, int32_t *n_picked,
                       void *workspace, size_t workspace_bytes, int method, void *stream);

size_t halo_score_range_bytes(int64_t B);
int halo_score_range(const void *score, int dtype, int64_t B, int64_t H, int64_t W, void *score_range, void *stream);
int halo_greedy_select_ranged(void *score, int dtype, int64_t B, int64_t H, int64_t W, int64_t n_regions,
                              int64_t active_radius, int64_t mask_radius, uint8_t *active, uint8_t *selected,
                              int64_t *active_mask, const int64_t *gt, double *picks, int32_t *n_picked,
                              void *workspace, size_t workspace_bytes, int method, const void *score_range, void *stream);

enum { HALO_SWEEP_DONE = 0,
       HALO_SWEEP_BAD_VALUES = 1,
       HALO_SWEEP_BIN_OVERFLOW = 2,
       HALO_SWEEP_SURVIVORS = 3,
       HALO_SWEEP_EXHAUSTED = 4,
       HALO_SWEEP_NOT_RUN = 5 };
int halo_greedy_select_ex(void *score, int dtype, int64_t B, int64_t H, int64_t W, int64_t n_regions,
                          int64_t active_radius, int64_t mask_radius, uint8_t *active, uint8_t *selected,
                          int64_t *active_mask, const int64_t *gt, double *picks, int32_t *n_picked,
                          void *workspace, size_t workspace_bytes, int method, const void *score_range,
                          int32_t *handover, void *stream);

int halo_pack_pick_tables(const double *picks, const int32_t *n_picked, int64_t B, int64_t n_regions, int32_t *wire,
                          int64_t wire_row_stride, void *stream);
int halo_reset_round_state(uint8_t *active, uint8_t *selected, int64_t *active_mask, int64_t n_pixels, void *stream);
int halo_undo_picks(const double *picks, const int32_t *n_picked, int64_t B, int64_t H, int64_t W, int64_t n_regions,
                    int64_t active_radius, int64_t mask_radius, uint8_t *active, uint8_t *selected, int64_t *active_mask,
                    void *stream);
int halo_device_identity(int device, char *buf, size_t len);

size_t halo_loss_workspace_bytes(int64_t n);
int halo_negative_learning_fwd(const float *p, int64_t n, double threshold, double *sums, void *workspace,
                               size_t workspace_bytes, void *stream);
int halo_negative_learning_bwd(const float *p, int64_t n, double threshold, const double *sums, const float *gloss,
                               float *gp, void *stream);
int halo_local_consistent_fwd(const float *x, const int64_t *label, int64_t B, int64_t O, int64_t h, int64_t w, int kl,
                              float *p, double *sums, float *coef_a, float *coef_b, uint8_t *mask, void *workspace,
                              size_t workspace_bytes, void *stream);
int halo_local_consistent_bwd(const float *p, const float *coef_a, const float *coef_b, const uint8_t *mask, int64_t B, int64_t O,
                              int64_t h, int64_t w, const double *sums, const float *gloss, float *gx, void *stream);

size_t halo_eval_workspace_bytes(int64_t B, int64_t K, int64_t H, int64_t W);
int halo_eval_confusion(const float *logit, int64_t logit_bstride, int views, int64_t K, int64_t h, int64_t w, const void *label,
                        int label_dtype, int64_t H, int64_t W, int64_t B, int64_t ignore_index, int64_t *counts, int64_t *pred,
                        void *workspace, size_t workspace_bytes, void *stream);
int halo_confusion_from_pred(const void *pred, int pred_dtype, const void *label, int label_dtype, int64_t K, int64_t H, int64_t W,
                             int64_t B, int64_t ignore_index, int64_t *counts, void *workspace, size_t workspace_bytes, void *stream);

enum { HALO_LOSS_CE = 1, HALO_LOSS_NL = 2 };
size_t halo_upsampled_loss_workspace_bytes(int64_t B, int64_t K, int64_t H, int64_t W);
int halo_upsampled_loss_fwd(const float *logit, int64_t logit_bstride, int64_t B, int64_t K, int64_t h, int64_t w, const void *label,
                            int label_dtype, int64_t H, int64_t W, int64_t ignore_index, double threshold, int terms, double *sums,
                            void *workspace, size_t workspace_bytes, void *stream);
int halo_upsampled_loss_bwd(const float *logit, int64_t logit_bstride, int64_t B, int64_t K, int64_t h, int64_t w, const void *label,
                            int label_dtype, int64_t H, int64_t W, int64_t ignore_index, double threshold, int terms,
                            const double *sums, const float *g_ce, const float *g_nl, float *grad_logit, void *stream);

size_t halo_hfr_workspace_bytes(int64_t B, int64_t C, int64_t P);
int halo_hfr_fwd_stats(const float *x, int64_t B, int64_t C, int64_t P, const float *W1, const float *b1, double *stats, void *workspace,
                       size_t workspace_bytes, void *stream);
int halo_hfr_fwd_apply(const float *x, int64_t B, int64_t C, int64_t P, const float *W1, const float *b1, const double *stats,
                       float *running_mean, float *running_var, double momentum, double eps, const float *gamma, const float *beta,
                       const float *W2, const float *b2, float *y, void *workspace, size_t workspace_bytes, void *stream);
int halo_hfr_bwd_reduce(const float *x, int64_t B, int64_t C, int64_t P, const float *W2, const float *g, float *g_W2, float *g_b2,
                        float *g_gamma, float *g_beta, double *gsums, void *workspace, size_t workspace_bytes, void *stream);
int halo_hfr_bwd_apply(const float *x, int64_t B, int64_t C, int64_t P, const float *W1, const float *b1, const float *gamma,
                       const float *g, const double *gsums, float *g_x, float *g_W1, float *g_b1, void *workspace,
                       size_t workspace_bytes, void *stream);

size_t halo_dwconv_workspace_bytes(int64_t B, int64_t C, int64_t H, int64_t W, int64_t d);
int halo_dwconv3x3_affine_relu_fwd(const float *x, const float *w, const float *scale, const float *shift, float *y, int64_t B, int64_t C,
                                   int64_t H, int64_t W, int64_t d, void *stream);
int halo_dwconv3x3_affine_relu_bwd_data(const float *g, const float *y, const float *w, const float *scale, float *g_x, int64_t B,
                                        int64_t C, int64_t H, int64_t W, int64_t d, void *stream);
int halo_dwconv3x3_affine_relu_bwd_weight(const float *g, const float *y, const float *x, const float *scale, float *g_w, int64_t B,
                                          int64_t C, int64_t H, int64_t W, int64_t d, void *workspace, size_t workspace_bytes,
                                          void *stream);

void *halo_event_create(void);
int halo_event_record(void *event, void *stream);
int halo_event_elapsed_ms(void *start, void *stop, float *ms);
int halo_event_destroy(void *event);

#ifdef __cplusplus
}
#endif
#endif
```

Before: 1366.

## Fuse box3 min/max and stats finalize into feature-reduce kernel via atomic counters

Folds the separate box3 min/max pass and the min/max finalize kernel into the tail of the fused feature-reduce kernel. Per-band atomic counters detect when a band of entropy rows and its neighbours are complete, and the last block reduces the band; a final counter triggers the stats finalization and resets the counters. A workspace-ready flag lets the host skip the counter-clearing kernel when the Python side pre-zeroed the counter region, saving launches and a re-read of the entropy map. In exchange it adds agent-scope atomics and fences and a dependence on counters being left at zero between calls.

```diff
diff --git a/halo_amd/_lib.py b/halo_amd/_lib.py
--- a/halo_amd/_lib.py
+++ b/halo_amd/_lib.py
@@ -15,10 +15,12 @@
 SWEEP_REASONS = ("done", "bad_values", "bin_overflow", "survivors", "exhausted", "not_run")
 PAD = {"zeros": 0, "reflect": 1, "replicate": 2, "circular": 3}
 FLAG_NORMALIZE = 1
-
-
-def score_flags(normalize, padding_mode="zeros"):
-    return (FLAG_NORMALIZE if normalize else 0) | (PAD[padding_mode] << 8)
+FLAG_WORKSPACE_READY = 2
+WS_COUNTER_BYTES = 65536
+
+
+def score_flags(normalize, padding_mode="zeros", ws_ready=False):
+    return (FLAG_NORMALIZE if normalize else 0) | (FLAG_WORKSPACE_READY if ws_ready else 0) | (PAD[padding_mode] << 8)
 
 _i64, _dbl, _int, _vp, _sz = C.c_int64, C.c_double, C.c_int, C.c_void_p, C.c_size_t
 
@@ -40,6 +42,7 @@
     "halo_bilinear_upsample": (_int, [_vp, _vp, _int, _i64, _i64, _i64, _i64, _i64, _vp]),
     "halo_bilinear_upsample_bwd": (_int, [_vp, _vp, _int, _i64, _i64, _i64, _i64, _i64, _vp]),
     "halo_score_workspace_bytes": (_sz, [_i64, _i64, _i64]),
+    "halo_score_stats_offset": (_sz, [_i64, _i64, _i64]),
     "halo_score_maps": (_int, [_vp, _i64, _vp, _int, _i64, _vp, _vp, _i64, _i64, _i64, _i64, _i64, _int, _int,
                                _int, _int, _int, _i64, _dbl, _vp, _vp, _vp, _vp, _sz, _vp]),
     "halo_score_maps_timed": (_int, [_vp, _i64, _vp, _int, _i64, _vp, _vp, _i64, _i64, _i64, _i64, _i64, _int, _int,
diff --git a/halo_amd/core/active/floating_region.py b/halo_amd/core/active/floating_region.py
--- a/halo_amd/core/active/floating_region.py
+++ b/halo_amd/core/active/floating_region.py
@@ -28,22 +28,39 @@
         return False
 
 
+def _new_scratch(dev, nbytes, tag):
+    buf = torch.empty(int(nbytes), dtype=torch.uint8, device=dev)
+    if tag == "score" and nbytes >= _lib.WS_COUNTER_BYTES and not torch.cuda.is_current_stream_capturing():
+        buf[:_lib.WS_COUNTER_BYTES].zero_()
+        buf._halo_counters_zero = True
+    return buf
+
+
+def _ws_ready(ws):
+    return bool(getattr(ws, "_halo_counters_zero", False))
+
+
 def _workspace(dev, nbytes, tag):
     held = getattr(_ws_tls, "held", None)
     if held is not None:
-        buf = torch.empty(int(nbytes), dtype=torch.uint8, device=dev)
+        buf = _new_scratch(dev, nbytes, tag)
         held.append(buf)
         return buf
     key = (dev.index, torch.cuda.current_stream(dev).cuda_stream, tag)
     buf = _WS.get(key)
     if buf is None or buf.numel() < nbytes:
-        buf = torch.empty(int(nbytes), dtype=torch.uint8, device=dev)
+        buf = _new_scratch(dev, nbytes, tag)
         _WS[key] = buf
     return buf
 
 
 def score_workspace(B, H, W, dev):
-    return torch.empty(int(_lib.lib().halo_score_workspace_bytes(int(B), int(H), int(W))), dtype=torch.uint8, device=dev)
+    return _new_scratch(dev, _lib.lib().halo_score_workspace_bytes(int(B), int(H), int(W)), "score")
+
+
+def score_stats(workspace, B, H, W):
+    off = int(_lib.lib().halo_score_stats_offset(int(B), int(H), int(W)))
+    return workspace[off:off + int(B) * 32].view(torch.float64).view(int(B), 4)
 
 
 def score_dtype(pur_type, decoder_out):
@@ -126,14 +143,14 @@
             "tail_stream needs events, a workspace of the call's own and preallocated maps"
         rc = L.halo_score_maps_split(_lib.ptr(logit), logit.stride(0), _lib.ptr(feat), fdt, fbs, _lib.ptr(gt),
                                      _lib.ptr(act), B, O, Cc, H, W, _lib.UNC.get(unc_type, _lib.UNC_ZEROS),
-                                     _lib.PUR[pur_type], _lib.score_flags(normalize, padding_mode), int(size), int(psize), int(K), float(c),
+                                     _lib.PUR[pur_type], _lib.score_flags(normalize, padding_mode, _ws_ready(ws)), int(size), int(psize), int(K), float(c),
                                      _lib.ptr(score), _lib.ptr(imp), _lib.ptr(unc), _lib.ptr(ws), ws.numel(),
                                      _lib.stream_ptr(dev), _lib.C.c_void_p(tail_stream.cuda_stream), ev0, ev1, _lib.ptr(score_range))
         _lib.check(rc, "halo_score_maps_split")
         return score, imp, unc
     rc = L.halo_score_maps_timed(_lib.ptr(logit), logit.stride(0), _lib.ptr(feat), fdt, fbs, _lib.ptr(gt),
                                  _lib.ptr(act), B, O, Cc, H, W, _lib.UNC.get(unc_type, _lib.UNC_ZEROS),
-                                 _lib.PUR[pur_type], _lib.score_flags(normalize, padding_mode), int(size), int(psize), int(K), float(c),
+                                 _lib.PUR[pur_type], _lib.score_flags(normalize, padding_mode, _ws_ready(ws)), int(size), int(psize), int(K), float(c),
                                  _lib.ptr(score), _lib.ptr(imp), _lib.ptr(unc), _lib.ptr(ws), ws.numel(),
                                  _lib.stream_ptr(dev), ev0, ev1, _lib.ptr(score_range))
     _lib.check(rc, "halo_score_maps")
@@ -190,7 +207,7 @@
     fn, name = (L.halo_score_maps_lr_gram, "halo_score_maps_lr_gram") if gram else (L.halo_score_maps_lr, "halo_score_maps_lr")
     args = (_lib.ptr(logit_lr), logit_lr.stride(0), hl, wl, _lib.ptr(feat), fdt, fbs, hf, wf,
             _lib.ptr(gt), _lib.ptr(act), B, O, Cc, H, W, _lib.UNC.get(unc_type, _lib.UNC_ZEROS),
-            _lib.PUR[pur_type], _lib.score_flags(normalize, padding_mode), int(ksize), int(psize), int(K), float(c),
+            _lib.PUR[pur_type], _lib.score_flags(normalize, padding_mode, _ws_ready(ws)), int(ksize), int(psize), int(K), float(c),
             _lib.ptr(score), _lib.ptr(imp), _lib.ptr(unc), _lib.ptr(ws), ws.numel(),
             _lib.stream_ptr(dev))
     if events is not None or score_range is not None:
diff --git a/halo_amd/csrc/halo_score.hip b/halo_amd/csrc/halo_score.hip
--- a/halo_amd/csrc/halo_score.hip
+++ b/halo_amd/csrc/halo_score.hip
@@ -237,6 +237,196 @@
     if (pred) pred[(size_t)b * hw + i] = (short)pr;
 }
 
+__device__ __forceinline__ float lane_prev(float v)
+{
+    return __int_as_float(__builtin_amdgcn_update_dpp(0, __float_as_int(v), 0x138 , 0xf, 0xf, false));
+}
+__device__ __forceinline__ float lane_next(float v)
+{
+    return __int_as_float(__builtin_amdgcn_update_dpp(0, __float_as_int(v), 0x130 , 0xf, 0xf, false));
+}
+
+__device__ __forceinline__ float box3_over_count(float a, int H, int W, int y, int xx, int pk)
+{
+    if (pk <= 0) return a;
+    const int rr = pk / 2;
+    const int y0 = y - rr < 0 ? 0 : y - rr, y1 = y + rr >= H ? H - 1 : y + rr;
+    const int x0 = xx - rr < 0 ? 0 : xx - rr, x1 = xx + rr >= W ? W - 1 : xx + rr;
+    return a / (float)((y1 - y0 + 1) * (x1 - x0 + 1));
+}
+
+constexpr int BM_RPT = 4, BM_TW = 256, BM_TH = BM_RPT * (TPB / 64);
+
+__device__ __forceinline__ float nan_minf(float a, float b) { return (a != a) ? a : ((b != b) ? b : (b < a ? b : a)); }
+__device__ __forceinline__ float nan_maxf(float a, float b) { return (a != a) ? a : ((b != b) ? b : (b > a ? b : a)); }
+
+__device__ __forceinline__ void box3_strip_minmax(const float *__restrict__ ep, int H, int W, int pk, int x, int y0, int ylim,
+                                                  float &mn, float &mx, bool &have)
+{
+    const int lane = threadIdx.x & 63;
+    const bool xin = x < W;
+    auto load_row = [&](int yy, float (&r)[6]) {
+        const bool in = xin && yy >= 0 && yy < H;
+        const float *row = ep + (size_t)(in ? yy : 0) * W;
+        float4 q = make_float4(0.0f, 0.0f, 0.0f, 0.0f);
+        if (in) q = *reinterpret_cast<const float4 *>(row + x);
+        float left = lane_prev(q.w), right = lane_next(q.x);
+        if (lane == 0) left = (in && x > 0) ? row[x - 1] : 0.0f;
+        if (lane == 63) right = (in && x + 4 < W) ? row[x + 4] : 0.0f;
+        r[0] = (in && x > 0) ? left : 0.0f;
+        r[1] = q.x; r[2] = q.y; r[3] = q.z; r[4] = q.w;
+        r[5] = (in && x + 4 < W) ? right : 0.0f;
+    };
+    float r0[6], r1[6], r2[6];
+    load_row(y0 - 1, r0);
+    load_row(y0, r1);
+#pragma unroll
+    for (int k = 0; k < BM_RPT; ++k) {
+        const int y = y0 + k;
+        load_row(y + 1, r2);
+        if (xin && y < ylim) {
+#pragma unroll
+            for (int j = 0; j < 4; ++j) {
+                float a = 0.0f;
+#pragma unroll
+                for (int dx = 0; dx < 3; ++dx) a = a + r0[j + dx];
+#pragma unroll
+                for (int dx = 0; dx < 3; ++dx) a = a + r1[j + dx];
+#pragma unroll
+                for (int dx = 0; dx < 3; ++dx) a = a + r2[j + dx];
+                const float o = box3_over_count(a, H, W, y, x + j, pk);
+                if (!have) { mn = mx = o; have = true; }
+                else { mn = nan_minf(mn, o); mx = nan_maxf(mx, o); }
+            }
+        }
+#pragma unroll
+        for (int q = 0; q < 6; ++q) { r0[q] = r1[q]; r1[q] = r2[q]; }
+    }
+}
+
+template <int NT>
+__device__ __forceinline__ bool block_minmaxf(float mn, float mx, bool have, float2 &out)
+{
+    __shared__ float seedf[2];
+    __shared__ float smn[NT / 64], smx[NT / 64];
+    __syncthreads();
+    if (threadIdx.x == 0) { seedf[0] = mn; seedf[1] = mx; }
+    __syncthreads();
+    if (!have) { mn = seedf[0]; mx = seedf[1]; }
+#pragma unroll
+    for (int off = 32; off > 0; off >>= 1) {
+        mn = nan_minf(mn, __shfl_xor(mn, off));
+        mx = nan_maxf(mx, __shfl_xor(mx, off));
+    }
+    if ((threadIdx.x & 63) == 0) { smn[threadIdx.x >> 6] = mn; smx[threadIdx.x >> 6] = mx; }
+    __syncthreads();
+    if (threadIdx.x != 0) return false;
+#pragma unroll
+    for (int i = 1; i < NT / 64; ++i) { mn = nan_minf(mn, smn[i]); mx = nan_maxf(mx, smx[i]); }
+    out = make_float2(mn, mx);
+    return true;
+}
+
+constexpr int FS_BR = 16;
+constexpr size_t FS_CNT_BYTES = 65536;
+struct FusedStats {
+    unsigned *cnt;
+    double *band_part;
+    double *stats;
+    unsigned *hist_zero;
+    int H, W, pk, nbands;
+};
+
+#define HALO_RLX_AGENT __ATOMIC_RELAXED, __HIP_MEMORY_SCOPE_AGENT
+__device__ __forceinline__ void fs_store(double *p, double v) { __hip_atomic_store(p, v, HALO_RLX_AGENT); }
+__device__ __forceinline__ void fs_wait_stores() { asm volatile("s_waitcnt vmcnt(0)" ::: "memory"); }
+__device__ __forceinline__ void fs_acquire()
+{
+    __builtin_amdgcn_fence(__ATOMIC_ACQUIRE, "agent");
+    asm volatile("s_waitcnt vmcnt(0)" ::: "memory");
+}
+
+template <int NT>
+__device__ __forceinline__ void fs_finalize(const FusedStats &fs, int b, const double *__restrict__ part_imp, int nblk_imp)
+{
+    if (threadIdx.x == 0) fs_acquire();
+    __syncthreads();
+#pragma unroll 1
+    for (int slot = 0; slot < 2; ++slot) {
+        const int n = slot ? fs.nbands : nblk_imp;
+        const double2 *p = reinterpret_cast<const double2 *>((slot ? fs.band_part + (size_t)b * fs.nbands * 2 : part_imp + (size_t)b * nblk_imp * 2));
+        const double2 p0 = p[0];
+        double mn = p0.x, mx = p0.y;
+        for (int i = threadIdx.x; i < n; i += NT) { const double2 q = p[i]; mn = nan_min(mn, q.x); mx = nan_max(mx, q.y); }
+        __syncthreads();
+        block_minmax<NT>(mn, mx, fs.stats + b * 4 + slot * 2);
+    }
+    if (fs.hist_zero)
+        for (int j = threadIdx.x; j < NB1; j += NT) fs.hist_zero[(size_t)b * NB1 + j] = 0u;
+    unsigned *c = fs.cnt + (size_t)b * (2 * fs.nbands + 1);
+    for (int j = threadIdx.x; j < 2 * fs.nbands + 1; j += NT) c[j] = 0u;
+}
+
+template <int NT>
+__device__ __forceinline__ void fs_reduce_band(const FusedStats &fs, const float *__restrict__ ep, int b, int k,
+                                               const double *__restrict__ part_imp, int nblk_imp, unsigned *s_flag)
+{
+    const int lane = threadIdx.x & 63, wv = threadIdx.x >> 6;
+    const int ybeg = k * FS_BR, yend = ybeg + FS_BR < fs.H ? ybeg + FS_BR : fs.H;
+    const int nsx = (fs.W + BM_TW - 1) / BM_TW, ns = nsx * ((yend - ybeg + BM_RPT - 1) / BM_RPT);
+    float mn = 0.0f, mx = 0.0f;
+    bool have = false;
+#pragma unroll 1
+    for (int s_ = wv; s_ < ns; s_ += NT / 64)
+        box3_strip_minmax(ep, fs.H, fs.W, fs.pk, (s_ % nsx) * BM_TW + lane * 4, ybeg + (s_ / nsx) * BM_RPT, yend, mn, mx, have);
+    float2 r;
+    if (block_minmaxf<NT>(mn, mx, have, r)) {
+        double *out2 = fs.band_part + ((size_t)b * fs.nbands + k) * 2;
+        fs_store(out2, (double)r.x);
+        fs_store(out2 + 1, (double)r.y);
+        fs_wait_stores();
+        const unsigned t = __hip_atomic_fetch_add(fs.cnt + (size_t)b * (2 * fs.nbands + 1) + 2 * fs.nbands, 1u, HALO_RLX_AGENT);
+        *s_flag = t == (unsigned)fs.nbands - 1u;
+    }
+    __syncthreads();
+    const bool last = *s_flag != 0u;
+    __syncthreads();
+    if (last) fs_finalize<NT>(fs, b, part_imp, nblk_imp);
+}
+
+template <int NT, unsigned CH>
+__device__ __forceinline__ void fs_chunk_done(const FusedStats &fs, const float *__restrict__ ep, int b, unsigned blk0, unsigned hw,
+                                              const double *__restrict__ part_imp, int nblk_imp)
+{
+    __shared__ unsigned s_fs[3];
+    if (threadIdx.x == 0) {
+        const unsigned W = (unsigned)fs.W, nb = (unsigned)fs.nbands;
+        const unsigned last = (blk0 + CH < hw ? blk0 + CH : hw) - 1u;
+        const unsigned k0 = (blk0 / W) / FS_BR, k1 = (last / W) / FS_BR;
+        unsigned *c = fs.cnt + (size_t)b * (2 * nb + 1);
+        unsigned todo = 0u;
+        for (unsigned k = k0; k <= k1; ++k) {
+            const unsigned p0 = k * FS_BR * W, p1 = (k + 1 < nb ? (k + 1) * FS_BR * W : hw) - 1u;
+            const unsigned need = p1 / CH - p0 / CH + 1u;
+            if (__hip_atomic_fetch_add(c + k, 1u, HALO_RLX_AGENT) != need - 1u) continue;
+            for (unsigned j = k > 0 ? k - 1 : 0; j <= k + 1 && j < nb; ++j) {
+                const unsigned want = 1u + (j > 0) + (j + 1 < nb);
+                if (__hip_atomic_fetch_add(c + nb + j, 1u, HALO_RLX_AGENT) == want - 1u) todo |= 1u << (j + 1 - k0);
+            }
+        }
+        if (todo) fs_acquire();
+        s_fs[0] = todo;
+        s_fs[1] = k0;
+    }
+    __syncthreads();
+    const unsigned todo = s_fs[0];
+    if (__builtin_expect(todo == 0u, 1)) return;
+    const int kbase = (int)s_fs[1] - 1;
+#pragma unroll 1
+    for (int i = 0; i < 4; ++i)
+        if ((todo >> i) & 1u) fs_reduce_band<NT>(fs, ep, b, kbase + i, part_imp, nblk_imp, &s_fs[2]);
+}
+
 __device__ __forceinline__ double fma_t(double a, double b, double c) { return __builtin_fma(a, b, c); }
 __device__ __forceinline__ float fma_t(float a, float b, float c) { return __builtin_fmaf(a, b, c); }
 
@@ -265,9 +455,11 @@
 __global__ void __launch_bounds__(FTPB) __attribute__((amdgpu_waves_per_eu(1, HALO_FEAT_WAVES))) k_feat_reduce(const T *__restrict__ feat, long long bstride, int C,
                                                      long long hw, double ks, double rks, T *__restrict__ out,
                                                      double *__restrict__ partials, const float *__restrict__ logit,
-                                                     long long lbstride, int unc_type, float *__restrict__ ent, unsigned xcd_g)
+                                                     long long lbstride, int unc_type, float *__restrict__ ent, unsigned xcd_g,
+                                                     const FusedStats fs)
 {
     const int b = blockIdx.y;
+    const bool fs_on = FO > 0 && VEC > 1 && fs.cnt != nullptr;
     unsigned bx = blockIdx.x;
     const unsigned xj = blockIdx.x >> 3;
     if (xcd_g != 0 && blockIdx.x < (gridDim.x / (8 * xcd_g)) * (8 * xcd_g))
@@ -317,8 +509,11 @@
 #pragma unroll 1
                         for (int j = 0; j < NP; ++j) px_general(lp + off + j, FO, hw, 0, unc_type, HALO_PUR_NONE, 0, e[j], pr[j]);
                     }
-                    if constexpr (NP == 2) *reinterpret_cast<float2 *>(eb + off) = make_float2(e[0], e[1]);
-                    else eb[off] = e[0];
+                    if constexpr (NP == 2) {
+                        if (fs_on) __hip_atomic_store(reinterpret_cast<unsigned long long *>(eb + off),
+                                                      ((unsigned long long)__float_as_uint(e[1]) << 32) | __float_as_uint(e[0]), HALO_RLX_AGENT);
+                        else *reinterpret_cast<float2 *>(eb + off) = make_float2(e[0], e[1]);
+                    } else eb[off] = e[0];
                 }
                 __builtin_amdgcn_sched_barrier(0);
             }
@@ -371,6 +566,21 @@
     if (threadIdx.x == 0) { seed[0] = mn; seed[1] = mx; }
     __syncthreads();
     if (!live) { mn = seed[0]; mx = seed[1]; }
+    if constexpr (FO > 0 && VEC > 1) {
+        if (fs_on) {
+            __shared__ double s_part[2];
+            block_minmax<FTPB>(mn, mx, s_part);
+            if (threadIdx.x == 0) {
+                double *out2 = partials + ((size_t)b * gridDim.x + bx) * 2;
+                fs_store(out2, s_part[0]);
+                fs_store(out2 + 1, s_part[1]);
+            }
+            fs_wait_stores();
+            __syncthreads();
+            fs_chunk_done<FTPB, FTPB * VEC>(fs, ent + (size_t)b * hw, b, (unsigned)blk0, (unsigned)hw, partials, (int)gridDim.x);
+            return;
+        }
+    }
     block_minmax<FTPB>(mn, mx, partials + ((size_t)b * gridDim.x + bx) * 2);
 }
 
@@ -579,23 +789,6 @@
     block_minmax<TPB>(mn, mx, partials + ((size_t)b * gridDim.x + blockIdx.x) * 2);
 }
 
-__device__ __forceinline__ float lane_prev(float v)
-{
-    return __int_as_float(__builtin_amdgcn_update_dpp(0, __float_as_int(v), 0x138 , 0xf, 0xf, false));
-}
-__device__ __forceinline__ float lane_next(float v)
-{
-    return __int_as_float(__builtin_amdgcn_update_dpp(0, __float_as_int(v), 0x130 , 0xf, 0xf, false));
-}
-
-__device__ __forceinline__ float box3_over_count(float a, int H, int W, int y, int xx, int pk)
-{
-    if (pk <= 0) return a;
-    const int rr = pk / 2;
-    const int y0 = y - rr < 0 ? 0 : y - rr, y1 = y + rr >= H ? H - 1 : y + rr;
-    const int x0 = xx - rr < 0 ? 0 : xx - rr, x1 = xx + rr >= W ? W - 1 : xx + rr;
-    return a / (float)((y1 - y0 + 1) * (x1 - x0 + 1));
-}
 
 __device__ __forceinline__ void box3_row4(const float *__restrict__ ep, int H, int W, int y, int x, bool live, int pk, float (&o)[4])
 {
@@ -651,11 +844,6 @@
     block_minmax<TPB>(mn, mx, partials + ((size_t)b * gridDim.x + blockIdx.x) * 2);
 }
 
-constexpr int BM_RPT = 4, BM_TW = 256, BM_TH = BM_RPT * (TPB / 64);
-
-__device__ __forceinline__ float nan_minf(float a, float b) { return (a != a) ? a : ((b != b) ? b : (b < a ? b : a)); }
-__device__ __forceinline__ float nan_maxf(float a, float b) { return (a != a) ? a : ((b != b) ? b : (b > a ? b : a)); }
-
 __global__ void __launch_bounds__(TPB) k_box3_minmax(const float *__restrict__ ent, int H, int W, int pk, double *__restrict__ partials,
                                                      unsigned *__restrict__ hist_zero)
 {
@@ -664,66 +852,14 @@
         const unsigned nb = gridDim.x * gridDim.y;
         for (unsigned l = blockIdx.y * gridDim.x + blockIdx.x; l < NB1 / TPB; l += nb) hist_zero[(size_t)b * NB1 + l * TPB + threadIdx.x] = 0u;
     }
-    const int x = blockIdx.x * BM_TW + lane * 4, y0 = blockIdx.y * BM_TH + wv * BM_RPT;
-    const float *ep = ent + (size_t)b * H * W;
-    const bool xin = x < W;
-    auto load_row = [&](int yy, float (&r)[6]) {
-        const bool in = xin && yy >= 0 && yy < H;
-        const float *row = ep + (size_t)(in ? yy : 0) * W;
-        float4 q = make_float4(0.0f, 0.0f, 0.0f, 0.0f);
-        if (in) q = *reinterpret_cast<const float4 *>(row + x);
-        float left = lane_prev(q.w), right = lane_next(q.x);
-        if (lane == 0) left = (in && x > 0) ? row[x - 1] : 0.0f;
-        if (lane == 63) right = (in && x + 4 < W) ? row[x + 4] : 0.0f;
-        r[0] = (in && x > 0) ? left : 0.0f;
-        r[1] = q.x; r[2] = q.y; r[3] = q.z; r[4] = q.w;
-        r[5] = (in && x + 4 < W) ? right : 0.0f;
-    };
-    float r0[6], r1[6], r2[6];
-    load_row(y0 - 1, r0);
-    load_row(y0, r1);
     float mn = 0.0f, mx = 0.0f;
     bool have = false;
-#pragma unroll
-    for (int k = 0; k < BM_RPT; ++k) {
-        const int y = y0 + k;
-        load_row(y + 1, r2);
-        if (xin && y < H) {
-#pragma unroll
-            for (int j = 0; j < 4; ++j) {
-                float a = 0.0f;
-#pragma unroll
-                for (int dx = 0; dx < 3; ++dx) a = a + r0[j + dx];
-#pragma unroll
-                for (int dx = 0; dx < 3; ++dx) a = a + r1[j + dx];
-#pragma unroll
-                for (int dx = 0; dx < 3; ++dx) a = a + r2[j + dx];
-                const float o = box3_over_count(a, H, W, y, x + j, pk);
-                if (!have) { mn = mx = o; have = true; }
-                else { mn = nan_minf(mn, o); mx = nan_maxf(mx, o); }
-            }
-        }
-#pragma unroll
-        for (int q = 0; q < 6; ++q) { r0[q] = r1[q]; r1[q] = r2[q]; }
-    }
-    __shared__ float seedf[2];
-    __shared__ float smn[TPB / 64], smx[TPB / 64];
-    if (threadIdx.x == 0) { seedf[0] = mn; seedf[1] = mx; }
-    __syncthreads();
-    if (!have) { mn = seedf[0]; mx = seedf[1]; }
-#pragma unroll
-    for (int off = 32; off > 0; off >>= 1) {
-        mn = nan_minf(mn, __shfl_xor(mn, off));
-        mx = nan_maxf(mx, __shfl_xor(mx, off));
-    }
-    if (lane == 0) { smn[wv] = mn; smx[wv] = mx; }
-    __syncthreads();
-    if (threadIdx.x == 0) {
-#pragma unroll
-        for (int i = 1; i < TPB / 64; ++i) { mn = nan_minf(mn, smn[i]); mx = nan_maxf(mx, smx[i]); }
+    box3_strip_minmax(ent + (size_t)b * H * W, H, W, pk, blockIdx.x * BM_TW + lane * 4, blockIdx.y * BM_TH + wv * BM_RPT, H, mn, mx, have);
+    float2 r;
+    if (block_minmaxf<TPB>(mn, mx, have, r)) {
         double *out2 = partials + (((size_t)b * gridDim.y + blockIdx.y) * gridDim.x + blockIdx.x) * 2;
-        out2[0] = (double)mn;
-        out2[1] = (double)mx;
+        out2[0] = (double)r.x;
+        out2[1] = (double)r.y;
     }
 }
 
@@ -740,6 +876,12 @@
     __syncthreads();
     if (!live) { mn = seed[0]; mx = seed[1]; }
     block_minmax<TPB>(mn, mx, partials + ((size_t)b * gridDim.x + blockIdx.x) * 2);
+}
+
+__global__ void __launch_bounds__(TPB) k_fill_u32(unsigned *__restrict__ x, long long n, unsigned v)
+{
+    const long long i = (long long)blockIdx.x * TPB + threadIdx.x;
+    if (i < n) x[i] = v;
 }
 
 __global__ void __launch_bounds__(TPB) k_fill_f32(float *__restrict__ x, long long n, float v)
@@ -1834,8 +1976,11 @@
 
 template <typename T, int VEC>
 static void launch_feat(const T *feat, long long bstride, int C, long long hw, int B, int mode, double ks, double rks,
-                        T *out, double *partials, int nblk, hipStream_t st, const FusedLogit *fl = nullptr)
-{
+                        T *out, double *partials, int nblk, hipStream_t st, const FusedLogit *fl = nullptr,
+                        const FusedStats *fsp = nullptr)
+{
+    FusedStats fs{nullptr, nullptr, nullptr, nullptr, 0, 0, 0, 0};
+    if (fsp && fl && VEC > 1) fs = *fsp;
     dim3 grid(nblk, B), block(FTPB);
     constexpr int UNROLL = HALO_FEAT_UNROLL;
     unsigned xcd_g = 256;
@@ -1844,7 +1989,7 @@
 #define HALO_FEAT(M, FO_)                                                                                               \
     hipLaunchKernelGGL((k_feat_reduce<T, VEC, M, UNROLL, FO_>), grid, block, 0, st, feat, bstride, C, hw, ks, rks, out, \
                        partials, fl ? fl->logit : nullptr, fl ? fl->bstride : 0ll, fl ? fl->unc_type : 0, fl ? fl->ent : nullptr, \
-                       xcd_g)
+                       xcd_g, fs)
     const int fo = fl ? fl->O : 0;
     if (mode == 0) {
         if (fo == 19) HALO_FEAT(0, 19); else if (fo == 16) HALO_FEAT(0, 16); else HALO_FEAT(0, 0);
@@ -1870,7 +2015,7 @@
     if (B <= 0 || H <= 0 || W <= 0) return 0;
     const size_t n = (size_t)B * H * W;
     const size_t nblk = partial_slots(H, W);
-    size_t s = 0;
+    size_t s = FS_CNT_BYTES;
     s += align_up(n * 4, 256);
     s += align_up(n * 4, 256);
     s += align_up(n * 8, 256);
@@ -1878,6 +2023,14 @@
     s += 2 * align_up((size_t)B * nblk * 2 * 8, 256);
     s += align_up((size_t)B * 4 * 8, 256);
     return s + 1024;
+}
+
+extern "C" size_t halo_score_stats_offset(int64_t B, int64_t H, int64_t W)
+{
+    if (B <= 0 || H <= 0 || W <= 0) return 0;
+    const size_t n = (size_t)B * H * W;
+    return FS_CNT_BYTES + 2 * align_up(n * 4, 256) + align_up(n * 8, 256) + align_up(n * 2, 256) +
+           2 * align_up((size_t)B * partial_slots(H, W) * 2 * 8, 256);
 }
 
 extern "C" int halo_score_maps(const float *logit, int64_t logit_bstride, const void *feat, int feat_dtype,
@@ -2002,7 +2155,8 @@
 {
     hipStream_t st = (hipStream_t)stream;
     const int pad = (normalize >> 8) & 3;
-    if (normalize & ~(HALO_FLAG_NORMALIZE | (3 << 8))) return fail(HALO_E_ARG, "halo_score_maps: unknown flag bits 0x%x", normalize);
+    const bool ws_ready = (normalize & HALO_FLAG_WORKSPACE_READY) != 0;
+    if (normalize & ~(HALO_FLAG_NORMALIZE | HALO_FLAG_WORKSPACE_READY | (3 << 8))) return fail(HALO_E_ARG, "halo_score_maps: unknown flag bits 0x%x", normalize);
     normalize &= HALO_FLAG_NORMALIZE;
     if (!logit || !score || B <= 0 || O <= 0 || H <= 0 || W <= 0) return fail(HALO_E_ARG, "halo_score_maps: null/empty argument");
     if (unc_type < 0 || unc_type > HALO_UNC_ZEROS) return fail(HALO_E_ARG, "halo_score_maps: bad unc_type %d", unc_type);
@@ -2027,6 +2181,7 @@
     const long long hw = (long long)H * W;
     const int nblk1 = (int)cdiv(hw, TPB);
     Arena ar(workspace, workspace_bytes);
+    unsigned *fs_cnt = ar.take<unsigned>(FS_CNT_BYTES / sizeof(unsigned));
     float *ent = ar.take<float>((size_t)B * hw);
     float *unc_raw = ar.take<float>((size_t)B * hw);
     double *imp_raw = ar.take<double>((size_t)B * hw);
@@ -2086,6 +2241,22 @@
 
     if (ev_logit_stop) (void)hipEventRecord((hipEvent_t)ev_logit_stop, st);
 
+    const int do_box = (unc_type == HALO_UNC_ENTROPY || unc_type == HALO_UNC_ORACLE_ACC) ? 1 : 0;
+    const bool box3 = do_box && pad == HALO_PAD_ZEROS && ksize == 3 && W % 4 == 0 && aligned16(ent) && aligned16(unc_raw);
+    const bool fuse_tail = box3 && B <= 65535 && H <= 65535 && aligned16(imp_raw) && aligned16(score) && (!impurity || aligned16(impurity)) &&
+                           (!uncertainty || aligned16(uncertainty)) && (!active || ((uintptr_t)active & 3) == 0);
+    unsigned *rng_hist = (score_range && normalize && fuse_tail)
+                             ? (unsigned *)((char *)score_range + range_hist_offset(B)) : nullptr;
+    const int fs_nbands = (int)cdiv(H, FS_BR);
+    const bool fstats = fuse && fuse_tail && normalize && !hist && pur_type != HALO_PUR_HYPER && H >= FS_BR &&
+                        hw >= (long long)FTPB * fvec && (long long)W * FS_BR >= (long long)FTPB * fvec && hw < (1ll << 31) &&
+                        (size_t)B * (2 * (size_t)fs_nbands + 1) * sizeof(unsigned) <= FS_CNT_BYTES;
+    FusedStats fsv{fs_cnt, part_unc, stats, rng_hist, (int)H, (int)W, hist ? pksize : 0, fs_nbands};
+    const FusedStats *fsp = fstats ? &fsv : nullptr;
+    if (fstats && !ws_ready)
+        hipLaunchKernelGGL(k_fill_u32, dim3((unsigned)cdiv(B * (2 * fs_nbands + 1), TPB)), block, 0, st, fs_cnt,
+                           (long long)(B * (2 * fs_nbands + 1)), 0u);
+
     int nblk_imp = nblk1;
     if (need_feat) {
         if (ev_feat_start) (void)hipEventRecord((hipEvent_t)ev_feat_start, st);
@@ -2121,11 +2292,11 @@
             if (rc != HALO_OK) return rc;
         } else if (feat_dtype == HALO_F64) {
             const bool v2 = (hw % 2 == 0) && (feat_bstride % 2 == 0) && aligned16(feat) && aligned16(imp_raw);
-            if (v2) { nblk_imp = (int)cdiv(hw, FTPB * 2); launch_feat<double, 2>((const double *)feat, feat_bstride, (int)C, hw, (int)B, mode, ks, rks, imp_raw, part_imp, nblk_imp, st, flp); }
+            if (v2) { nblk_imp = (int)cdiv(hw, FTPB * 2); launch_feat<double, 2>((const double *)feat, feat_bstride, (int)C, hw, (int)B, mode, ks, rks, imp_raw, part_imp, nblk_imp, st, flp, fsp); }
             else { nblk_imp = (int)cdiv(hw, FTPB); launch_feat<double, 1>((const double *)feat, feat_bstride, (int)C, hw, (int)B, mode, ks, rks, imp_raw, part_imp, nblk_imp, st); }
         } else {
             const bool v4 = (hw % 4 == 0) && (feat_bstride % 4 == 0) && aligned16(feat) && aligned16(imp_raw);
-            if (v4) { nblk_imp = (int)cdiv(hw, FTPB * 4); launch_feat<float, 4>((const float *)feat, feat_bstride, (int)C, hw, (int)B, mode, ks, rks, (float *)imp_raw, part_imp, nblk_imp, st, flp); }
+            if (v4) { nblk_imp = (int)cdiv(hw, FTPB * 4); launch_feat<float, 4>((const float *)feat, feat_bstride, (int)C, hw, (int)B, mode, ks, rks, (float *)imp_raw, part_imp, nblk_imp, st, flp, fsp); }
             else { nblk_imp = (int)cdiv(hw, FTPB); launch_feat<float, 1>((const float *)feat, feat_bstride, (int)C, hw, (int)B, mode, ks, rks, (float *)imp_raw, part_imp, nblk_imp, st); }
         }
         if (ev_feat_stop) (void)hipEventRecord((hipEvent_t)ev_feat_stop, st);
@@ -2154,16 +2325,12 @@
         nblk_imp = nblk1;
     }
 
-    const int do_box = (unc_type == HALO_UNC_ENTROPY || unc_type == HALO_UNC_ORACLE_ACC) ? 1 : 0;
     int nblk_unc = nblk1;
-    const bool box3 = do_box && pad == HALO_PAD_ZEROS && ksize == 3 && W % 4 == 0 && aligned16(ent) && aligned16(unc_raw);
-    const bool fuse_tail = box3 && B <= 65535 && H <= 65535 && aligned16(imp_raw) && aligned16(score) && (!impurity || aligned16(impurity)) &&
-                           (!uncertainty || aligned16(uncertainty)) && (!active || ((uintptr_t)active & 3) == 0);
     const int nblk_c3 = (int)cdiv(hw, TPB * 4);
-    unsigned *rng_hist = (score_range && normalize && fuse_tail)
-                             ? (unsigned *)((char *)score_range + range_hist_offset(B)) : nullptr;
     if (fuse_tail) {
-        if (normalize) {
+        if (fstats) {
+            nblk_unc = 0;
+        } else if (normalize) {
             const dim3 gridm((unsigned)cdiv(W, BM_TW), (unsigned)cdiv(H, BM_TH), (unsigned)B);
             nblk_unc = (int)(gridm.x * gridm.y);
             hipLaunchKernelGGL(k_box3_minmax, gridm, block, 0, st, (const float *)ent, (int)H, (int)W, hist ? pksize : 0, part_unc, rng_hist);
@@ -2178,7 +2345,7 @@
     }
 
     SelHdr *rng_free = (score_range && normalize && fuse_tail) ? (SelHdr *)score_range : nullptr;
-    if (normalize)
+    if (normalize && !fstats)
         hipLaunchKernelGGL(k_minmax_finalize2, dim3((unsigned)B, 2u), dim3(FIN_TPB), 0, st, (const double *)part_imp, nblk_imp,
                            (const double *)part_unc, nblk_unc, stats);
     if (fuse_tail) {
@@ -2248,6 +2415,7 @@
     const long long hw = (long long)H * W;
     const int nblk1 = (int)cdiv(hw, TPB), nblkf = (int)cdiv(hw, FTPB);
     Arena ar(workspace, workspace_bytes);
+    (void)ar.take<unsigned>(FS_CNT_BYTES / sizeof(unsigned));
     double *imp_raw = ar.take<double>((size_t)B * hw);
     double *part = ar.take<double>((size_t)B * nblkf * 2);
     double *stats = ar.take<double>((size_t)B * 4);
diff --git a/include/halo_hip.h b/include/halo_hip.h
--- a/include/halo_hip.h
+++ b/include/halo_hip.h
@@ -17,7 +17,8 @@
 enum { HALO_UNC_ENTROPY = 0, HALO_UNC_PIXEL_ENTROPY = 1, HALO_UNC_ORACLE_ACC = 2, HALO_UNC_ZEROS = 3 };
 
 enum { HALO_PAD_ZEROS = 0, HALO_PAD_REFLECT = 1, HALO_PAD_REPLICATE = 2, HALO_PAD_CIRCULAR = 3 };
-enum { HALO_FLAG_NORMALIZE = 1 };
+enum { HALO_FLAG_NORMALIZE = 1,
+       HALO_FLAG_WORKSPACE_READY = 2 };
 #define HALO_FLAG_PAD(mode) ((mode) << 8)
 
 enum { HALO_PUR_RIPU = 0, HALO_PUR_ORACLE_RIPU = 1, HALO_PUR_HYPER = 2, HALO_PUR_NONE = 3,
@@ -64,6 +65,7 @@
                                int64_t H, int64_t W, void *stream);
 
 size_t halo_score_workspace_bytes(int64_t B, int64_t H, int64_t W);
+size_t halo_score_stats_offset(int64_t B, int64_t H, int64_t W);
 int halo_score_maps(const float *logit, int64_t logit_bstride, const void *feat, int feat_dtype,
                     int64_t feat_bstride, const int64_t *gt, const uint8_t *active, int64_t B, int64_t O,
                     int64_t C, int64_t H, int64_t W, int unc_type, int pur_type, int normalize, int ksize,
```

Result: slower. 1331 (-2.6%).
